# Xharlie/pointnerf

Measured on AMD Instinct MI355X. Metric: rays/sec (render+bwd) NeRF-synth lego 800^2, K=8, 128 samp/ray, higher is better.
Workload: dtype f32 in / out / accumulate; forward GEMM operands as 2 x f16 planes (22-bit) on the f16 MFMA, 3 products per multiply-add; input-gradient GEMMs: f16 leading product + e4m3 cross terms (csrc/mixq.h), 2 product equivalents; weight-gradient GEMM operands as one f16 plane each

## Files before the change

include/pnerf.h:

```cpp
#ifndef PNERF_H
#define PNERF_H
#include <stddef.h>
#include <stdint.h>

#ifdef __cplusplus
extern "C" {
#endif

#define PNERF_E_INVAL   (-1)
#define PNERF_E_WS      (-2)
#define PNERF_E_LAUNCH  (-3)
#define PNERF_E_UNSUP   (-4)

#define PNERF_MAX_K 16

typedef struct pnerf_grid_params {
    float ranges[6];
    float vsize[3];
    int32_t vdim[3];
    int32_t kernel_size[3];
    int32_t query_size[3];
    int32_t P;
    int32_t max_o;
    float radius;
} pnerf_grid_params;

enum { PNERF_GI_N_IN_GRID = 0, PNERF_GI_N_OCC = 1, PNERF_GI_MAX_CNT = 2, PNERF_GI_CELL0 = 3,
       PNERF_GI_FIRST_IDX = 4, PNERF_GI_OSTART_OFF = 5 , PNERF_GI_LEN = 8 };

int pnerf_version(void);
const char *pnerf_arch(void);

size_t pnerf_grid_workspace_bytes(const pnerf_grid_params *gp, int n_points);
int pnerf_grid_build(const pnerf_grid_params *gp, const float *d_xyz, int n_points,
                     void *d_grid_ws, size_t ws_bytes, void *stream);
int pnerf_grid_info(const void *d_grid_ws, int32_t *host_info, void *stream);
int pnerf_points_minmax(const float *d_xyz, int64_t n_points, float *d_out6, void *stream);

size_t pnerf_query_workspace_bytes(int R, int SR);
int pnerf_query(const pnerf_grid_params *gp, const void *d_grid_ws,
                const float *d_raypos,
                const float *campos3_host, const float *d_raydir, const float *d_mid,
                float near_depth, float far_depth, float jitter, uint64_t seed,
                int R, int D, int SR, int K,
                float *d_sample_loc, int32_t *d_sample_pidx, int32_t *d_sample_nn,
                int32_t *d_ray_hit, int32_t *d_valid_list, int32_t *d_counters,
                void *d_query_ws, size_t ws_bytes, void *stream);

int pnerf_gather_rows(const float *d_src, int n_src, int width, const int32_t *d_idx, int64_t n_idx,
                      float *d_dst, void *stream);
int pnerf_scatter_add_rows(const float *d_grad_rows, const int32_t *d_idx, int64_t n_idx, int width,
                           float *d_grad_src, int n_src, void *stream);

int pnerf_zero_one_blocks(int64_t n_idx);
int pnerf_zero_one_forward(const float *d_conf, int n_points, const int32_t *d_idx, int64_t n_idx, float eps,
                           float *d_partial, void *stream);
int pnerf_zero_one_backward(const float *d_conf, int n_points, const int32_t *d_idx, int64_t n_idx, float eps,
                            const float *d_gscale, float *d_grad_conf, void *stream);
int pnerf_zero_one_forward_rays(const float *d_conf, int n_points, const int32_t *d_idx, const int32_t *d_ray_hit, int R, int slots_per_ray, float eps,
                                float *d_partial, void *stream);
int pnerf_zero_one_backward_rays(const float *d_conf, int n_points, const int32_t *d_idx, const int32_t *d_ray_hit, int R, int slots_per_ray, float eps,
                                 const float *d_gscale, float *d_grad_conf, void *stream);
int pnerf_color_loss_blocks(int R);
int pnerf_color_loss_forward_rays(const float *d_ray_color, const float *d_gt, const int32_t *d_ray_hit, int R, float *d_partial, void *stream);
int pnerf_color_loss_backward_rays(const float *d_ray_color, const float *d_gt, const int32_t *d_ray_hit, int R, const float *d_gscale,
                                   float *d_grad_ray_color, void *stream);

int pnerf_geometry_loss_forward_rays(const float *d_depth_sum, const float *d_acc, const float *d_bg_trans, const int32_t *d_ray_hit,
                                     const float *d_gt_depth, const float *d_gt_mask, int R, float *d_partial, void *stream);
int pnerf_geometry_loss_backward_rays(const float *d_depth_sum, const float *d_acc, const float *d_bg_trans, const int32_t *d_ray_hit,
                                      const float *d_gt_depth, const float *d_gt_mask, int R, const float *d_gscale2, float *d_grad_geom, void *stream);


#define PNERF_MLP_NTENSORS 18
int pnerf_mlp_layout(int feat_dim, int64_t *offsets );
size_t pnerf_mlp_packed_bytes(void);
int pnerf_mlp_pack(const float *d_params, void *d_packed, void *stream);

typedef struct pnerf_camera {
    float campos[3];
    float camrot[9];
    float rw2c[9];
    float vsize_z;
    int32_t raydist_mode_unit;
    float bg[3];
    int32_t has_bg;
} pnerf_camera;

typedef struct pnerf_points {
    const float *xyz;
    const float *embedding;
    const float *conf;
    const float *dir;
    const float *color;
    int32_t n, feat_dim;
    const float *frames;
} pnerf_points;

typedef struct pnerf_point_grads {
    float *embedding, *conf, *dir, *color;
    void *ready_event;
    const float *zero_one_gscale;
    float zero_one_eps;
    float *xyz;
} pnerf_point_grads;

typedef struct pnerf_step {
    const float *raydir;
    const float *sample_loc;
    const int32_t *sample_pidx;
    const int32_t *sample_nn;
    const int32_t *valid_list;
    const int32_t *counters;
    const float *xyz_pers;
    const float *loc_pers;
    const float *params;
    const void *packed_mlp;
    int32_t R, SR, K;
    int64_t n_valid_max;
} pnerf_step;

size_t pnerf_agg_saved_bytes(int64_t n_valid_samples, int K);
size_t pnerf_agg_workspace_bytes(int64_t n_valid_max, int K);
size_t pnerf_render_backward_workspace_bytes(int R, int SR);

int pnerf_render_forward(const pnerf_camera *cam, const pnerf_points *pts, const pnerf_step *step,
                         float *d_decoded, float *d_weight, float *d_ray_color, float *d_opacity,
                         float *d_bg_trans, float *d_blend_w,
                         void *d_saved, void *d_ws, size_t ws_bytes, void *stream);

size_t pnerf_render_cut_workspace_bytes(int R, int SR);
int pnerf_render_forward_cut(const pnerf_camera *cam, const pnerf_points *pts, const pnerf_step *step, float cutoff, int stage_samples,
                             float *d_decoded, float *d_weight, float *d_ray_color, float *d_opacity, float *d_bg_trans, float *d_blend_w,
                             int32_t *d_cut_counters, void *d_ws, size_t ws_bytes, void *d_cut_ws, size_t cut_ws_bytes, void *stream);
int pnerf_cut_stage(const pnerf_camera *cam, const float *d_sample_loc, const int32_t *d_sample_nn, const int32_t *d_ray_hit,
                    const float *d_decoded, int R, int SR, float cutoff, int stage_samples, int stage,
                    float *d_trans, float *d_depth_max, int32_t *d_alive, int32_t *d_flags, int32_t *d_list, int32_t *d_counters,
                    void *d_ws, size_t ws_bytes, void *stream);

int pnerf_set_inference_products(int n);

int pnerf_set_wgrad_planes(int n);
int pnerf_set_cross_terms(int bits);
int pnerf_set_cross_terms_where(int mask);
int pnerf_get_arithmetic(int32_t out[4]);
int pnerf_debug_set_tile_grid(int max_workgroups);

int pnerf_render_backward(const pnerf_camera *cam, const pnerf_points *pts, const pnerf_step *step,
                          const float *d_decoded, const float *d_weight, const float *d_grad_ray_color,
                          void *d_saved, float *d_grad_params, const pnerf_point_grads *pg,
                          void *d_ws, size_t ws_bytes, void *stream);
int pnerf_render_backward_geom(const pnerf_camera *cam, const pnerf_points *pts, const pnerf_step *step,
                               const float *d_decoded, const float *d_weight, const float *d_grad_ray_color, const float *d_grad_geom,
                               void *d_saved, float *d_grad_params, const pnerf_point_grads *pg,
                               void *d_ws, size_t ws_bytes, void *stream);


size_t pnerf_compact_workspace_bytes(int64_t n);
int pnerf_touched_flags(const int32_t *d_pidx, int64_t n, int32_t n_points, int32_t *d_flags, void *stream);
int pnerf_compact_valid(const int32_t *d_nn, int64_t n, int32_t *d_list, int32_t *d_counters, void *d_ws, size_t ws_bytes, void *stream);

int pnerf_agg_forward(const pnerf_camera *cam, const pnerf_points *pts, const pnerf_step *step, float *d_decoded, float *d_weight,
                      void *d_saved, void *d_ws, size_t ws_bytes, void *stream);
int pnerf_agg_backward(const pnerf_camera *cam, const pnerf_points *pts, const pnerf_step *step,
                       const float *d_decoded, const float *d_weight, const float *d_grad_decoded,
                       void *d_saved, float *d_grad_params, const pnerf_point_grads *pg, void *d_ws, size_t ws_bytes, void *stream);

int pnerf_raymarch_forward(const float *d_ray_dist, const uint8_t *d_ray_valid, const float *d_features, const float *bg3_host,
                           int R, int SR, float *d_ray_color, float *d_opacity, float *d_acc_trans, float *d_blend_w,
                           float *d_bg_trans, void *stream);
int pnerf_raymarch_backward(const float *d_ray_dist, const uint8_t *d_ray_valid, const float *d_features, const float *bg3_host,
                            int R, int SR, const float *d_grad_ray_color, float *d_grad_features, void *stream);
int pnerf_raymarch_backward_geom(const float *d_ray_dist, const uint8_t *d_ray_valid, const float *d_features, const float *d_z, const float *bg3_host,
                                 int R, int SR, const float *d_grad_ray_color, const float *d_grad_geom, float *d_grad_features, void *stream);

int pnerf_adam_step(float *d_param, const float *d_grad, float *d_exp_avg, float *d_exp_avg_sq, int64_t n,
                    double lr, double beta1, double beta2, double eps, int64_t step, void *stream);
typedef struct pnerf_adam_tensor {
    float *param; const float *grad; float *exp_avg; float *exp_avg_sq;
    int64_t n; double lr; int64_t step;
} pnerf_adam_tensor;
int pnerf_adam_step_multi(const pnerf_adam_tensor *tensors, int count, double beta1, double beta2, double eps, void *stream);

size_t pnerf_voxel_downsample_workspace_bytes(int64_t n_points, int rx, int ry, int rz);
int pnerf_voxel_downsample(const float *d_xyz, int64_t n_points, const float *space_min3_host, const float *vox_size3_host,
                           int rx, int ry, int rz, float *d_centroid, int32_t *d_grid_idx, int64_t *d_min_idx, int32_t *d_counts,
                           void *d_ws, size_t ws_bytes, void *stream);

#define PNERF_EX2D_MAX_VIEWS 8
#define PNERF_EX2D_MAX_MAPS 32
typedef struct pnerf_view_desc {
    float c2w[16];
    float w2c[16];
    float intrinsic[9];
    int32_t has_w2c;
} pnerf_view_desc;
typedef struct pnerf_map_desc {
    const float *d_map;
    int32_t view;
    int32_t C, H, W;
    int32_t out_col;
    int32_t is_color;
    int32_t first_of_view;
} pnerf_map_desc;
size_t pnerf_extract_2d_workspace_bytes(int64_t n_points, int n_views, int HD, int WD, int depth_occ);
int pnerf_extract_2d(const float *d_cam_xyz, int64_t n_points, const pnerf_view_desc *views, int n_views, const pnerf_map_desc *maps,
                     int n_maps, int HD, int WD, int depth_occ, float tolerate, float *d_feats, int feat_cols, float *d_colors,
                     int color_cols, uint8_t *d_mask, void *d_ws, size_t ws_bytes, void *stream);
int pnerf_point_dirs(const float *d_cam_xyz, int64_t n_points, const float *cam_pos_cam_host, int n_views, const float *rot1_host9,
                     const float *rot2_host9, float *d_dirs, void *stream);

#define PNERF_DF_PAIR_FLOATS 32
int pnerf_depth_consistency(const float *d_depth, const int32_t *view_hw_host, int V, const float *d_pairs, int32_t *d_geo_mask_sum,
                            float *d_depth_avg, void *stream);
size_t pnerf_depth_fuse_select_workspace_bytes(int V, int H, int W);
int pnerf_depth_fuse_select(const int32_t *d_geo_mask_sum, const float *d_depth_avg, const float *d_cam_xyz, const float *d_confidence,
                            const uint8_t *d_points_mask, const float *d_inv_ext, int V, int H, int W, float depth_conf_thresh,
                            int geo_cnsst_num, const float *conf_factor10_host, const float *ranges6_host, float *d_xyz_cam,
                            float *d_xyz_world, float *d_conf_out, int32_t *d_view_id, int32_t *d_count, void *d_ws, size_t ws_bytes,
                            void *stream);
int pnerf_alpha_hull(const float *d_points, int64_t n_points, const float *d_alphas, const float *d_w2c, const float *d_intrinsics, int V,
                     int H, int W, int use_range_mask, const float *near_far2_host, uint8_t *d_mask, void *stream);

int pnerf_nearest_view(const float *d_xyz, int64_t n, const float *d_campos, const float *d_camdir, int M, int32_t *d_cam_ind, void *stream);
size_t pnerf_occupancy_merge_workspace_bytes(int64_t nb, int res);
int pnerf_occupancy_merge(const float *d_a_xyz, int64_t na, const float *d_b_xyz, int64_t nb, const float *space_min3_host,
                          const float *vox_size_a3_host, const float *vox_size_b3_host, int res, float *d_kept_xyz, int32_t *d_count,
                          uint8_t *d_mask, void *d_ws, size_t ws_bytes, void *stream);
size_t pnerf_crop_ranges_workspace_bytes(int64_t n);
int pnerf_crop_ranges(const float *d_xyz, int64_t n, const float *ranges6_host, float *d_kept_xyz, int32_t *d_count, uint8_t *d_mask, void *d_ws,
                      size_t ws_bytes, void *stream);
size_t pnerf_group_by_view_workspace_bytes(int64_t n, int M);
int pnerf_group_by_view(const int32_t *d_cam_ind, int64_t n, int M, int64_t *d_order, int64_t *d_offsets, void *d_ws, size_t ws_bytes,
                        void *stream);

size_t pnerf_mvs_cost_volume_workspace_bytes(int n_feat_sets, int V, int h, int w);
int pnerf_mvs_cost_volume(const float *d_feats, int n_feat_sets, const float *d_proj, const float *d_depth_values, int B, int V, int C, int D,
                          int h, int w, int align_corners, float *d_volume, void *d_ws, size_t ws_bytes, void *stream);
int pnerf_mvs_depth_regress(const float *d_cost_reg, const float *d_depth_values, int B, int D, int h, int w, float *d_depth,
                            float *d_confidence, float *d_prob_volume, void *stream);
int pnerf_depth_to_cam_points(const float *d_depth_lr, const float *d_conf_lr, int h, int w, int H, int W, float near, float far,
                              const float *inv_kt9_host, float *d_cam_xyz, float *d_confidence, uint8_t *d_mask, void *stream);

size_t pnerf_image_metrics_workspace_bytes(int H, int W, int win);
int pnerf_image_metrics(const float *d_img, const float *d_gt, int H, int W, int win, double data_range, int quantize8, double *d_out4,
                        void *d_ws, size_t ws_bytes, void *stream);

int pnerf_probe_rays(const pnerf_points *pts, const float *d_opacity, const float *d_weight, const float *d_sample_loc,
                     const int32_t *d_sample_pidx, const int32_t *d_ray_hit, int R, int SR, int K, float *d_max_opacity, float *d_loc3,
                     float *d_far_dist, float *d_avg_color3, float *d_avg_dir3, float *d_avg_conf, float *d_avg_emb32, void *stream);
int pnerf_probe_hole_mask(const int8_t *d_ray_mask, const float *d_max_opacity, const float *d_far_dist, const float *d_raycolor,
                          const float *d_gt, const uint8_t *d_edge, const float *bg3_host, int H, int W, float opacity_thresh,
                          float far_thresh, int32_t *d_flags, void *stream);

int pnerf_ray_geometry(const pnerf_camera *cam, const float *d_sample_loc, const int32_t *d_sample_nn, const int32_t *d_ray_hit,
                       const float *d_opacity, const float *d_blend_w, int R, int SR, float *d_acc, float *d_depth_sum, float *d_depth,
                       float *d_median_depth, int32_t *d_median_slot, void *stream);
int pnerf_geometry_canvas(const int32_t *d_pixel_idx, const int8_t *d_ray_mask, const float *d_depth, const float *d_median_depth,
                          const float *d_acc, int n_rays, int H, int W, float *d_depth_canvas, float *d_median_canvas, float *d_acc_canvas,
                          int32_t *d_flag, void *stream);

int pnerf_ray_attributes(const float *d_attr, int32_t n_points, int C,
        const float *d_blend_w, const float *d_weight, const int32_t *d_sample_pidx, const int32_t *d_ray_hit,
        int R, int SR, int K,
        float *d_attr_sum , int32_t *d_top_point, int32_t *d_top_flat, float *d_top_contrib ,
        void *stream);
int pnerf_lift_to_points(const float *d_values , int C, const float *d_ray_factor ,
        const float *d_blend_w, const float *d_weight, const int32_t *d_sample_pidx, const int32_t *d_ray_hit,
        int R, int SR, int K, int32_t n_points,
        float *d_point_sum , float *d_point_mass , void *stream);

int pnerf_debug_mfma_f16(const void *d_a, const void *d_b, float *d_out, void *stream);
int pnerf_debug_mix_gemm(const float *d_w, int K, const float *d_x, void *d_img, float *d_out, void *stream);
int pnerf_debug_mfma_rate(int mode, int iters, float *d_scratch, double *flop_out, void *stream);
int pnerf_debug_uniform(uint64_t seed, uint64_t first, int64_t n, float *d_out, void *stream);
int pnerf_debug_split(const float *d_x, int64_t n, void *d_h, void *d_m, int sat, void *stream);
int pnerf_debug_pe(const float *d_x, int64_t n, int nfreq, float *d_out, void *stream);

int pnerf_prof_enable(int on);
int pnerf_prof_kernel_count(void);
const char *pnerf_prof_kernel_name(int id);
int pnerf_prof_collect(double *total_ms, int64_t *launches);

#ifdef __cplusplus
}
#endif
#endif
```

pointnerf_amd/_lib.py:

```python
import ctypes
import os

import torch

_HERE = os.path.dirname(os.path.abspath(__file__))
LIB_PATH = os.path.join(_HERE, "libpnerf_hip.so")

c_int, c_i64, c_f32, c_void_p, c_size_t = ctypes.c_int, ctypes.c_int64, ctypes.c_float, ctypes.c_void_p, ctypes.c_size_t

ABI_VERSION = 1009
PNERF_MAX_K = 16
DF_PAIR_FLOATS = 32
GI_N_IN_GRID, GI_N_OCC, GI_MAX_CNT, GI_CELL0, GI_FIRST_IDX, GI_LEN = 0, 1, 2, 3, 4, 8
MLP_NTENSORS = 18

ERRORS = {-1: "PNERF_E_INVAL (bad argument)", -2: "PNERF_E_WS (workspace too small)",
          -3: "PNERF_E_LAUNCH (HIP launch/runtime error)", -4: "PNERF_E_UNSUP (unsupported configuration)"}


class GridParams(ctypes.Structure):
    _fields_ = [("ranges", c_f32 * 6), ("vsize", c_f32 * 3), ("vdim", ctypes.c_int32 * 3),
                ("kernel_size", ctypes.c_int32 * 3), ("query_size", ctypes.c_int32 * 3),
                ("P", ctypes.c_int32), ("max_o", ctypes.c_int32), ("radius", c_f32)]


class Camera(ctypes.Structure):
    _fields_ = [("campos", c_f32 * 3), ("camrot", c_f32 * 9), ("rw2c", c_f32 * 9), ("vsize_z", c_f32),
                ("raydist_mode_unit", ctypes.c_int32), ("bg", c_f32 * 3), ("has_bg", ctypes.c_int32)]


class Points(ctypes.Structure):
    _fields_ = [("xyz", c_void_p), ("embedding", c_void_p), ("conf", c_void_p), ("dir", c_void_p),
                ("color", c_void_p), ("n", ctypes.c_int32), ("feat_dim", ctypes.c_int32), ("frames", c_void_p)]


class AdamTensor(ctypes.Structure):
    _fields_ = [("param", c_void_p), ("grad", c_void_p), ("exp_avg", c_void_p), ("exp_avg_sq", c_void_p),
                ("n", ctypes.c_int64), ("lr", ctypes.c_double), ("step", ctypes.c_int64)]


class ViewDesc(ctypes.Structure):
    _fields_ = [("c2w", c_f32 * 16), ("w2c", c_f32 * 16), ("intrinsic", c_f32 * 9), ("has_w2c", ctypes.c_int32)]


class MapDesc(ctypes.Structure):
    _fields_ = [("d_map", c_void_p), ("view", ctypes.c_int32), ("C", ctypes.c_int32), ("H", ctypes.c_int32), ("W", ctypes.c_int32),
                ("out_col", ctypes.c_int32), ("is_color", ctypes.c_int32), ("first_of_view", ctypes.c_int32)]


class PointGrads(ctypes.Structure):
    _fields_ = [("embedding", c_void_p), ("conf", c_void_p), ("dir", c_void_p), ("color", c_void_p), ("ready_event", c_void_p),
                ("zero_one_gscale", c_void_p), ("zero_one_eps", c_f32), ("xyz", c_void_p)]


class Step(ctypes.Structure):
    _fields_ = [("raydir", c_void_p), ("sample_loc", c_void_p), ("sample_pidx", c_void_p), ("sample_nn", c_void_p), ("valid_list", c_void_p),
                ("counters", c_void_p), ("xyz_pers", c_void_p), ("loc_pers", c_void_p), ("params", c_void_p), ("packed_mlp", c_void_p),
                ("R", ctypes.c_int32), ("SR", ctypes.c_int32), ("K", ctypes.c_int32), ("n_valid_max", ctypes.c_int64)]


_STEP_ARGS = [ctypes.POINTER(Camera), ctypes.POINTER(Points), ctypes.POINTER(Step)]
PROTOTYPES = {
    "pnerf_version": (c_int, []),
    "pnerf_arch": (ctypes.c_char_p, []),
    "pnerf_grid_workspace_bytes": (c_size_t, [ctypes.POINTER(GridParams), c_int]),
    "pnerf_grid_build": (c_int, [ctypes.POINTER(GridParams), c_void_p, c_int, c_void_p, c_size_t, c_void_p]),
    "pnerf_grid_info": (c_int, [c_void_p, ctypes.POINTER(ctypes.c_int32), c_void_p]),
    "pnerf_points_minmax": (c_int, [c_void_p, c_i64, c_void_p, c_void_p]),
    "pnerf_query_workspace_bytes": (c_size_t, [c_int, c_int]),
    "pnerf_query": (c_int, [ctypes.POINTER(GridParams), c_void_p, c_void_p, ctypes.POINTER(c_f32), c_void_p, c_void_p,
                            c_f32, c_f32, c_f32, ctypes.c_uint64, c_int, c_int, c_int, c_int,
                            c_void_p, c_void_p, c_void_p, c_void_p, c_void_p, c_void_p, c_void_p, c_size_t, c_void_p]),
    "pnerf_gather_rows": (c_int, [c_void_p, c_int, c_int, c_void_p, c_i64, c_void_p, c_void_p]),
    "pnerf_scatter_add_rows": (c_int, [c_void_p, c_void_p, c_i64, c_int, c_void_p, c_int, c_void_p]),
    "pnerf_zero_one_blocks": (c_int, [c_i64]),
    "pnerf_zero_one_forward": (c_int, [c_void_p, c_int, c_void_p, c_i64, c_f32, c_void_p, c_void_p]),
    "pnerf_zero_one_backward": (c_int, [c_void_p, c_int, c_void_p, c_i64, c_f32, c_void_p, c_void_p, c_void_p]),
    "pnerf_color_loss_blocks": (c_int, [c_int]),
    "pnerf_color_loss_forward_rays": (c_int, [c_void_p, c_void_p, c_void_p, c_int, c_void_p, c_void_p]),
    "pnerf_color_loss_backward_rays": (c_int, [c_void_p, c_void_p, c_void_p, c_int, c_void_p, c_void_p, c_void_p]),
    "pnerf_zero_one_forward_rays": (c_int, [c_void_p, c_int, c_void_p, c_void_p, c_int, c_int, c_f32, c_void_p, c_void_p]),
    "pnerf_zero_one_backward_rays": (c_int, [c_void_p, c_int, c_void_p, c_void_p, c_int, c_int, c_f32, c_void_p, c_void_p, c_void_p]),
    "pnerf_voxel_downsample_workspace_bytes": (c_size_t, [c_i64, c_int, c_int, c_int]),
    "pnerf_voxel_downsample": (c_int, [c_void_p, c_i64, c_void_p, c_void_p, c_int, c_int, c_int, c_void_p, c_void_p, c_void_p, c_void_p, c_void_p, c_size_t, c_void_p]),
    "pnerf_extract_2d_workspace_bytes": (c_size_t, [c_i64, c_int, c_int, c_int, c_int]),
    "pnerf_extract_2d": (c_int, [c_void_p, c_i64, ctypes.POINTER(ViewDesc), c_int, ctypes.POINTER(MapDesc), c_int, c_int, c_int, c_int, c_f32,
                                 c_void_p, c_int, c_void_p, c_int, c_void_p, c_void_p, c_size_t, c_void_p]),
    "pnerf_point_dirs": (c_int, [c_void_p, c_i64, ctypes.POINTER(c_f32), c_int, ctypes.POINTER(c_f32), ctypes.POINTER(c_f32), c_void_p, c_void_p]),
    "pnerf_depth_consistency": (c_int, [c_void_p, ctypes.POINTER(ctypes.c_int32), c_int, c_void_p, c_void_p, c_void_p, c_void_p]),
    "pnerf_depth_fuse_select_workspace_bytes": (c_size_t, [c_int, c_int, c_int]),
    "pnerf_depth_fuse_select": (c_int, [c_void_p, c_void_p, c_void_p, c_void_p, c_void_p, c_void_p, c_int, c_int, c_int, c_f32, c_int,
                                        ctypes.POINTER(c_f32), ctypes.POINTER(c_f32), c_void_p, c_void_p, c_void_p, c_void_p, c_void_p,
                                        c_void_p, c_size_t, c_void_p]),
    "pnerf_alpha_hull": (c_int, [c_void_p, c_i64, c_void_p, c_void_p, c_void_p, c_int, c_int, c_int, c_int, ctypes.POINTER(c_f32), c_void_p, c_void_p]),
    "pnerf_nearest_view": (c_int, [c_void_p, c_i64, c_void_p, c_void_p, c_int, c_void_p, c_void_p]),
    "pnerf_occupancy_merge_workspace_bytes": (c_size_t, [c_i64, c_int]),
    "pnerf_occupancy_merge": (c_int, [c_void_p, c_i64, c_void_p, c_i64, ctypes.POINTER(c_f32), ctypes.POINTER(c_f32), ctypes.POINTER(c_f32), c_int,
                                      c_void_p, c_void_p, c_void_p, c_void_p, c_size_t, c_void_p]),
    "pnerf_crop_ranges_workspace_bytes": (c_size_t, [c_i64]),
    "pnerf_crop_ranges": (c_int, [c_void_p, c_i64, ctypes.POINTER(c_f32), c_void_p, c_void_p, c_void_p, c_void_p, c_size_t, c_void_p]),
    "pnerf_group_by_view_workspace_bytes": (c_size_t, [c_i64, c_int]),
    "pnerf_group_by_view": (c_int, [c_void_p, c_i64, c_int, c_void_p, c_void_p, c_void_p, c_size_t, c_void_p]),
    "pnerf_mvs_cost_volume_workspace_bytes": (c_size_t, [c_int, c_int, c_int, c_int]),
    "pnerf_mvs_cost_volume": (c_int, [c_void_p, c_int, c_void_p, c_void_p, c_int, c_int, c_int, c_int, c_int, c_int, c_int, c_void_p, c_void_p,
                                      c_size_t, c_void_p]),
    "pnerf_mvs_depth_regress": (c_int, [c_void_p, c_void_p, c_int, c_int, c_int, c_int, c_void_p, c_void_p, c_void_p, c_void_p]),
    "pnerf_depth_to_cam_points": (c_int, [c_void_p, c_void_p, c_int, c_int, c_int, c_int, c_f32, c_f32, ctypes.POINTER(c_f32), c_void_p, c_void_p,
                                          c_void_p, c_void_p]),
    "pnerf_adam_step": (c_int, [c_void_p, c_void_p, c_void_p, c_void_p, c_i64, ctypes.c_double, ctypes.c_double, ctypes.c_double, ctypes.c_double, c_i64, c_void_p]),
    "pnerf_adam_step_multi": (c_int, [ctypes.POINTER(AdamTensor), c_int, ctypes.c_double, ctypes.c_double, ctypes.c_double, c_void_p]),
    "pnerf_mlp_layout": (c_int, [c_int, ctypes.POINTER(c_i64)]),
    "pnerf_mlp_packed_bytes": (c_size_t, []),
    "pnerf_mlp_pack": (c_int, [c_void_p, c_void_p, c_void_p]),
    "pnerf_agg_saved_bytes": (c_size_t, [c_i64, c_int]),
    "pnerf_agg_workspace_bytes": (c_size_t, [c_i64, c_int]),
    "pnerf_render_backward_workspace_bytes": (c_size_t, [c_int, c_int]),
    "pnerf_render_forward": (c_int, _STEP_ARGS + [c_void_p, c_void_p, c_void_p, c_void_p, c_void_p, c_void_p, c_void_p, c_void_p, c_size_t, c_void_p]),
    "pnerf_render_cut_workspace_bytes": (c_size_t, [c_int, c_int]),
    "pnerf_render_forward_cut": (c_int, _STEP_ARGS + [c_f32, c_int, c_void_p, c_void_p, c_void_p, c_void_p, c_void_p, c_void_p, c_void_p,
                                                      c_void_p, c_size_t, c_void_p, c_size_t, c_void_p]),
    "pnerf_cut_stage": (c_int, [ctypes.POINTER(Camera), c_void_p, c_void_p, c_void_p, c_void_p, c_int, c_int, c_f32, c_int, c_int,
                                c_void_p, c_void_p, c_void_p, c_void_p, c_void_p, c_void_p, c_void_p, c_size_t, c_void_p]),
    "pnerf_set_inference_products": (c_int, [c_int]),
    "pnerf_set_wgrad_planes": (c_int, [c_int]),
    "pnerf_set_cross_terms": (c_int, [c_int]),
    "pnerf_set_cross_terms_where": (c_int, [c_int]),
    "pnerf_get_arithmetic": (c_int, [ctypes.POINTER(ctypes.c_int32)]),
    "pnerf_debug_set_tile_grid": (c_int, [c_int]),
    "pnerf_compact_workspace_bytes": (c_size_t, [c_i64]),
    "pnerf_touched_flags": (c_int, [c_void_p, c_i64, c_int, c_void_p, c_void_p]),
    "pnerf_compact_valid": (c_int, [c_void_p, c_i64, c_void_p, c_void_p, c_void_p, c_size_t, c_void_p]),
    "pnerf_agg_forward": (c_int, _STEP_ARGS + [c_void_p, c_void_p, c_void_p, c_void_p, c_size_t, c_void_p]),
    "pnerf_agg_backward": (c_int, _STEP_ARGS + [c_void_p, c_void_p, c_void_p, c_void_p, c_void_p, ctypes.POINTER(PointGrads), c_void_p, c_size_t, c_void_p]),
    "pnerf_raymarch_forward": (c_int, [c_void_p, c_void_p, c_void_p, ctypes.POINTER(c_f32), c_int, c_int,
                                       c_void_p, c_void_p, c_void_p, c_void_p, c_void_p, c_void_p]),
    "pnerf_raymarch_backward": (c_int, [c_void_p, c_void_p, c_void_p, ctypes.POINTER(c_f32), c_int, c_int,
                                        c_void_p, c_void_p, c_void_p]),
    "pnerf_image_metrics_workspace_bytes": (c_size_t, [c_int, c_int, c_int]),
    "pnerf_image_metrics": (c_int, [c_void_p, c_void_p, c_int, c_int, c_int, ctypes.c_double, c_int, c_void_p, c_void_p, c_size_t, c_void_p]),
    "pnerf_probe_rays": (c_int, [ctypes.POINTER(Points), c_void_p, c_void_p, c_void_p, c_void_p, c_void_p, c_int, c_int, c_int,
                                 c_void_p, c_void_p, c_void_p, c_void_p, c_void_p, c_void_p, c_void_p, c_void_p]),
    "pnerf_probe_hole_mask": (c_int, [c_void_p, c_void_p, c_void_p, c_void_p, c_void_p, c_void_p, ctypes.POINTER(c_f32), c_int, c_int,
                                      c_f32, c_f32, c_void_p, c_void_p]),
    "pnerf_ray_geometry": (c_int, [ctypes.POINTER(Camera), c_void_p, c_void_p, c_void_p, c_void_p, c_void_p, c_int, c_int,
                                   c_void_p, c_void_p, c_void_p, c_void_p, c_void_p, c_void_p]),
    "pnerf_geometry_canvas": (c_int, [c_void_p, c_void_p, c_void_p, c_void_p, c_void_p, c_int, c_int, c_int,
                                      c_void_p, c_void_p, c_void_p, c_void_p, c_void_p]),
    "pnerf_ray_attributes": (c_int, [c_void_p, ctypes.c_int32, c_int, c_void_p, c_void_p, c_void_p, c_void_p, c_int, c_int, c_int,
                                     c_void_p, c_void_p, c_void_p, c_void_p, c_void_p]),
    "pnerf_lift_to_points": (c_int, [c_void_p, c_int, c_void_p, c_void_p, c_void_p, c_void_p, c_void_p, c_int, c_int, c_int, ctypes.c_int32,
                                     c_void_p, c_void_p, c_void_p]),
    "pnerf_debug_mfma_f16": (c_int, [c_void_p, c_void_p, c_void_p, c_void_p]),
    "pnerf_debug_mix_gemm": (c_int, [c_void_p, c_int, c_void_p, c_void_p, c_void_p, c_void_p]),
    "pnerf_debug_mfma_rate": (c_int, [c_int, c_int, c_void_p, ctypes.POINTER(ctypes.c_double), c_void_p]),
    "pnerf_debug_uniform": (c_int, [ctypes.c_uint64, ctypes.c_uint64, c_i64, c_void_p, c_void_p]),
    "pnerf_debug_split": (c_int, [c_void_p, c_i64, c_void_p, c_void_p, c_int, c_void_p]),
    "pnerf_debug_pe": (c_int, [c_void_p, c_i64, c_int, c_void_p, c_void_p]),
    "pnerf_prof_enable": (c_int, [c_int]),
    "pnerf_prof_kernel_count": (c_int, []),
    "pnerf_prof_kernel_name": (ctypes.c_char_p, [c_int]),
    "pnerf_prof_collect": (c_int, [ctypes.POINTER(ctypes.c_double), ctypes.POINTER(c_i64)]),
    "pnerf_render_backward": (c_int, _STEP_ARGS + [c_void_p, c_void_p, c_void_p, c_void_p, c_void_p, ctypes.POINTER(PointGrads), c_void_p, c_size_t, c_void_p]),
    "pnerf_render_backward_geom": (c_int, _STEP_ARGS + [c_void_p, c_void_p, c_void_p, c_void_p, c_void_p, c_void_p, ctypes.POINTER(PointGrads), c_void_p, c_size_t,
                                                        c_void_p]),
    "pnerf_raymarch_backward_geom": (c_int, [c_void_p, c_void_p, c_void_p, c_void_p, ctypes.POINTER(c_f32), c_int, c_int, c_void_p, c_void_p, c_void_p, c_void_p]),
    "pnerf_geometry_loss_forward_rays": (c_int, [c_void_p, c_void_p, c_void_p, c_void_p, c_void_p, c_void_p, c_int, c_void_p, c_void_p]),
    "pnerf_geometry_loss_backward_rays": (c_int, [c_void_p, c_void_p, c_void_p, c_void_p, c_void_p, c_void_p, c_int, c_void_p, c_void_p, c_void_p]),
}

_lib = None


def bind(handle, path):
    for name, (res, args) in PROTOTYPES.items():
        try:
            fn = getattr(handle, name)
        except AttributeError as e:
            raise RuntimeError("pointnerf_amd: %s lacks symbol %s (stale build?)" % (os.path.basename(path), name)) from e
        fn.restype, fn.argtypes = res, args
    got = handle.pnerf_version()
    if got != ABI_VERSION:
        raise RuntimeError("pointnerf_amd: %s reports pnerf_version() %d, this binding is written for %d (stale build?)"
                           % (os.path.basename(path), got, ABI_VERSION))
    return handle


def lib():
    global _lib
    if _lib is None:
        if not os.path.exists(LIB_PATH):
            raise RuntimeError(
                "pointnerf_amd: %s not found. Build it with `python -c 'import __graft_entry__ as g; g.build()'` "
                "(hipcc --offload-arch=gfx950). There is no CPU/PyTorch fallback for this path." % LIB_PATH)
        _lib = bind(ctypes.CDLL(LIB_PATH), LIB_PATH)
    return _lib


def check(rc, what):
    if rc != 0:
        raise RuntimeError("pointnerf_amd: %s failed: %s" % (what, ERRORS.get(rc, rc)))
```

pointnerf_amd/csrc/aggregate.hip:

```cpp
#include "mixq.h"
#include <stdlib.h>

extern "C" int pnerf_mlp_layout(int feat_dim, int64_t *offsets) {
    if (feat_dim != PN_F || !offsets) return PNERF_E_UNSUP;
    const int64_t o[PNERF_MLP_NTENSORS + 1] = {PO_W1, PO_B1, PO_W2, PO_B2, PO_W3, PO_B3, PO_W4, PO_B4, PO_W5, PO_B5,
                                               PO_WC1, PO_BC1, PO_WC2, PO_BC2, PO_WC3, PO_BC3, PO_WC4, PO_BC4, PO_TOTAL};
    for (int i = 0; i <= PNERF_MLP_NTENSORS; ++i) offsets[i] = o[i];
    return 0;
}
extern "C" size_t pnerf_mlp_packed_bytes(void) { return (size_t)PKC_END; }

namespace {
struct PackHDesc { int src, ld, trans, Mreal, Kreal, NCH, MB, dst, cm1, ck1; };
__device__ __forceinline__ float pn_pack_scale(const char *packed, int cm1, int ck1, int m, int k) {
    float f = 1.f;
    if (cm1 && m < (cm1 - 1 < PN_CS_C1 ? PN_H : PN_HC)) f = pn_col_scale(packed, cm1 - 1)[m];
    if (ck1) f *= pn_col_scale_inv(packed, ck1 - 1)[k];
    return f;
}
struct ColScaleDesc { int first, units, n_cons; struct { int src, ld, rows; } cons[2]; };
struct ColScaleTable { ColScaleDesc d[7]; };
__global__ __launch_bounds__(256) void k_pack_colscale(ColScaleTable t, const float *__restrict__ params, char *__restrict__ packed) {
    __shared__ unsigned red[256];
    const ColScaleDesc d = t.d[blockIdx.x];
// ... 163 lines not shown
        {PO_W3, PN_IN3, 0, PN_H, PN_IN3, 1, 8, PKM_F3},
        {PO_W4, PN_H, 0, PN_H, PN_H, 0, 8, PKM_F4},
        {PO_W4, PN_H, 1, PN_H, PN_H, 0, 8, PKM_D4, PN_CS_L3 + 1, PN_CS_L4 + 1},
        {PO_W3, PN_IN3, 1, PN_IN3, PN_H, 0, 9, PKM_D3, PN_CS_L2 + 1, PN_CS_L3 + 1},
        {PO_W2, PN_H, 1, PN_H, PN_H, 0, 8, PKM_D2, PN_CS_L1 + 1, PN_CS_L2 + 1},
        {PO_W1, PN_IN1, 1, 32 * PN_MB_D1, PN_H, 0, PN_MB_D1, PKM_D1, 0, PN_CS_L1 + 1},
        {PO_W1 + 32 * PN_MB_D1, PN_IN1, 1, PN_IN1 - 32 * PN_MB_D1, PN_H, 0, 2, PKM_D1T, 0, PN_CS_L1 + 1},
    }};
    hipLaunchKernelGGL(k_pack_mix, dim3(12, 9), dim3(256), 0, (hipStream_t)stream, tm, d_params, (char *)d_packed);
    PN_CHECK_LAUNCH();
    return 0;
}

namespace {
template <int NT>
__global__ __launch_bounds__(256) void k_debug_mix_gemm(const float *__restrict__ x, const char *__restrict__ img, float *__restrict__ out) {
    extern __shared__ __attribute__((aligned(16))) char smem_d[];
    pn_mode_saturate();
    constexpr int K = 256 + 16 * NT;
    char *X = smem_d;
    const int tid = threadIdx.x, lane = tid & 63, wave = __builtin_amdgcn_readfirstlane(tid >> 6);
    for (int e = tid; e < PN_TILE * (K / 4); e += 256) {
        const int row = e / (K / 4), col = 4 * (e % (K / 4));
        const float4 v = *reinterpret_cast<const float4 *>(x + row * K + col);
        if (col < 256) pn_xq_store4(X, row, col, v.x, v.y, v.z, v.w);
        else pn_xt_store4(X, row, col, v.x, v.y, v.z, v.w);
    }
    __syncthreads();
    f32x16 acc[2][2];
    pn_acc_zero(acc);
    pn_gemm_mix<PN_MIX_NS, NT, 8, 2>(X, img, 2 * wave, lane, acc);
#pragma unroll
    for (int fb = 0; fb < 2; ++fb)
#pragma unroll
        for (int rb = 0; rb < 2; ++rb)
#pragma unroll
            for (int g = 0; g < 4; ++g)
#pragma unroll
                for (int i = 0; i < 4; ++i) out[(32 * rb + (lane & 31)) * PN_H + pn_d_feat(2 * wave + fb, g, lane) + i] = acc[fb][rb][4 * g + i];
}
}

extern "C" int pnerf_debug_mix_gemm(const float *d_w, int K, const float *d_x, void *d_img, float *d_out, void *stream) {
    if (!d_w || !d_x || !d_img || !d_out || (K != 256 && K != 272 && K != 288)) return PNERF_E_INVAL;
    hipStream_t s = (hipStream_t)stream;
    const int NT = (K - 256) / 16;
    PackMTable tm = {{{0, K, 0, PN_H, K, NT, 8, 0}}};
    hipLaunchKernelGGL(k_pack_mix, dim3(12, 1), dim3(256), 0, s, tm, d_w, (char *)d_img);
    const void *fn = NT == 0 ? (const void *)k_debug_mix_gemm<0> : NT == 1 ? (const void *)k_debug_mix_gemm<1> : (const void *)k_debug_mix_gemm<2>;
    if (hipFuncSetAttribute(fn, hipFuncAttributeMaxDynamicSharedMemorySize, PN_XBYTES) != hipSuccess) return PNERF_E_LAUNCH;
    if (NT == 0) hipLaunchKernelGGL(k_debug_mix_gemm<0>, dim3(1), dim3(256), PN_XBYTES, s, d_x, (const char *)d_img, d_out);
    else if (NT == 1) hipLaunchKernelGGL(k_debug_mix_gemm<1>, dim3(1), dim3(256), PN_XBYTES, s, d_x, (const char *)d_img, d_out);
    else hipLaunchKernelGGL(k_debug_mix_gemm<2>, dim3(1), dim3(256), PN_XBYTES, s, d_x, (const char *)d_img, d_out);
    PN_CHECK_LAUNCH();
    return 0;
}

namespace {
__global__ __launch_bounds__(64) void k_debug_mfma_f16(const uint4 *__restrict__ a, const uint4 *__restrict__ b, float *__restrict__ d) {
    f32x16 acc;
#pragma unroll
    for (int r = 0; r < 16; ++r) acc[r] = 0.f;
    acc = __builtin_amdgcn_mfma_f32_32x32x16_f16(__builtin_bit_cast(pn_h8, a[threadIdx.x]), __builtin_bit_cast(pn_h8, b[threadIdx.x]), acc, 0, 0, 0);
#pragma unroll
    for (int r = 0; r < 16; ++r) d[threadIdx.x * 16 + r] = acc[r];
}
}
namespace {
__global__ __launch_bounds__(256) void k_debug_split(const float *__restrict__ x, long long n, unsigned *__restrict__ h, unsigned *__restrict__ m, int sat) {
    for (long long i = (long long)blockIdx.x * 256 + threadIdx.x; 2 * i < n; i += (long long)gridDim.x * 256) {
        unsigned hh, mm;
        if (sat) pn_split2_sat(x[2 * i], x[2 * i + 1], hh, mm);
        else pn_split2(x[2 * i], x[2 * i + 1], hh, mm);
        h[i] = hh; m[i] = mm;
    }
}
}
extern "C" int pnerf_debug_split(const float *d_x, int64_t n, void *d_h, void *d_m, int sat, void *stream) {
    if (!d_x || !d_h || !d_m || n < 0 || (n & 1)) return PNERF_E_INVAL;
    if (n == 0) return 0;
    hipLaunchKernelGGL(k_debug_split, dim3(64), dim3(256), 0, (hipStream_t)stream, d_x, (long long)n, (unsigned *)d_h, (unsigned *)d_m, sat);
    PN_CHECK_LAUNCH();
    return 0;
}

namespace {
template <int NF> __global__ __launch_bounds__(256) void k_debug_pe(const float *__restrict__ x, long long n, float *__restrict__ out) {
    for (long long i = (long long)blockIdx.x * 256 + threadIdx.x; i < n; i += (long long)gridDim.x * 256) {
        float s[NF], c[NF];
        pn_pe_octaves<NF>(x[i], s, c);
#pragma unroll
        for (int f = 0; f < NF; ++f) { out[(i * NF + f) * 2] = s[f]; out[(i * NF + f) * 2 + 1] = c[f]; }
    }
}
}
extern "C" int pnerf_debug_pe(const float *d_x, int64_t n, int nfreq, float *d_out, void *stream) {
    if (!d_x || !d_out || n < 0 || nfreq < 1 || nfreq > 5) return PNERF_E_INVAL;
    if (n == 0) return 0;
    hipStream_t s = (hipStream_t)stream;
    switch (nfreq) {
        case 1: hipLaunchKernelGGL(k_debug_pe<1>, dim3(64), dim3(256), 0, s, d_x, (long long)n, d_out); break;
        case 2: hipLaunchKernelGGL(k_debug_pe<2>, dim3(64), dim3(256), 0, s, d_x, (long long)n, d_out); break;
        case 3: hipLaunchKernelGGL(k_debug_pe<3>, dim3(64), dim3(256), 0, s, d_x, (long long)n, d_out); break;
        case 4: hipLaunchKernelGGL(k_debug_pe<4>, dim3(64), dim3(256), 0, s, d_x, (long long)n, d_out); break;
        default: hipLaunchKernelGGL(k_debug_pe<5>, dim3(64), dim3(256), 0, s, d_x, (long long)n, d_out); break;
    }
    PN_CHECK_LAUNCH();
    return 0;
}

extern "C" int pnerf_debug_mfma_f16(const void *d_a, const void *d_b, float *d_out, void *stream) {
    if (!d_a || !d_b || !d_out) return PNERF_E_INVAL;
    hipLaunchKernelGGL(k_debug_mfma_f16, dim3(1), dim3(64), 0, (hipStream_t)stream, (const uint4 *)d_a, (const uint4 *)d_b, d_out);
    PN_CHECK_LAUNCH();
    return 0;
}

size_t pn_saved_walk(void *base, long long n_valid, int K, PnSaved &s) {
    const int TS = pn_tile_samples(K);
    const long long tiles = (n_valid + TS - 1) / TS + 2 * PN_NCLS + 1;
    s.rows = tiles * PN_TILE;
    s.samples = ((tiles * TS + PN_CTILE - 1) / PN_CTILE + 1) * PN_CTILE;
    PnCarver cv(base);
    const size_t rg = (size_t)s.rows / 8, rgc = (size_t)s.samples / 8;
    auto planes = [&](uint4 *&x0, uint4 *&h2, uint4 *&h1, uint4 *&h3, uint4 *&dy1, uint4 *&dy2, uint4 *&dy3, uint4 *&dy4) {
        x0 = cv.take<uint4>(rg * PN_NF1); h2 = cv.take<uint4>(rg * PN_NF1);
        h1 = cv.take<uint4>(rg * PN_H); h3 = cv.take<uint4>(rg * PN_H);
        dy1 = cv.take<uint4>(rg * PN_H); dy2 = cv.take<uint4>(rg * PN_H);
        dy3 = cv.take<uint4>(rg * PN_H); dy4 = cv.take<uint4>(rg * PN_H);
    };
    auto cplanes = [&](uint4 *&xc, uint4 *&c1, uint4 *&c2, uint4 *&dc1, uint4 *&dc2, uint4 *&dc3) {
        xc = cv.take<uint4>(rgc * PN_NF1); c1 = cv.take<uint4>(rgc * PN_HC); c2 = cv.take<uint4>(rgc * PN_HC);
        dc1 = cv.take<uint4>(rgc * PN_HC); dc2 = cv.take<uint4>(rgc * PN_HC); dc3 = cv.take<uint4>(rgc * PN_HC);
    };
    planes(s.x0k, s.h2k, s.h1k, s.h3k, s.dy1k, s.dy2k, s.dy3k, s.dy4k);
    s.h4r = cv.take<uint4>((size_t)s.rows * 32 * 2);
    s.arow = cv.take<float>((size_t)s.rows); s.rmeta = cv.take<int4>((size_t)s.rows);
    s.lmask = cv.take<unsigned>((size_t)tiles * 3 * 512);
    s.gscale = cv.take<unsigned>(PN_GS_WORDS);
    s.fs = cv.take<float>((size_t)s.samples * PN_H); s.dfs = cv.take<float>((size_t)s.samples * PN_H);
    s.c3 = cv.take<float>((size_t)s.samples * PN_HC);
    cplanes(s.xck, s.c1k, s.c2k, s.dc1k, s.dc2k, s.dc3k);
    s.cmask = cv.take<unsigned>((size_t)s.samples / PN_CTILE * 2 * 256);
    s.wg2 = pn_arith().wgrad_planes == 2 ? 1 : 0;
    s.x0m = s.h1m = s.h2m = s.h3m = s.dy1m = s.dy2m = s.dy3m = s.dy4m = nullptr;
    s.xcm = s.c1m = s.c2m = s.dc1m = s.dc2m = s.dc3m = nullptr;
    if (s.wg2) {
        planes(s.x0m, s.h2m, s.h1m, s.h3m, s.dy1m, s.dy2m, s.dy3m, s.dy4m);
        cplanes(s.xcm, s.c1m, s.c2m, s.dc1m, s.dc2m, s.dc3m);
    }
    pn_cls_walk(cv, s);
    return cv.off;
}
void pn_cls_walk(PnCarver &cv, PnSaved &s) {
    s.cls_list = cv.take<int>((size_t)s.samples);
    s.cls_info = cv.take<int>(PN_CI_WORDS);
    s.cls_tmp = cv.take<int>((size_t)2 * s.samples + pn_scan_scratch_ints(s.samples) + 8);
}
size_t pn_saved_bytes(long long n_valid, int K) { PnSaved s; return pn_saved_walk(nullptr, n_valid, K, s); }
PnSaved pn_saved_carve(void *base, long long n_valid, int K) { PnSaved s; pn_saved_walk(base, n_valid, K, s); return s; }

extern "C" size_t pnerf_agg_saved_bytes(int64_t n_valid_samples, int K) {
    if (K <= 0 || K > PNERF_MAX_K || n_valid_samples < 0) return 0;
    return pn_saved_bytes(n_valid_samples, K);
}

namespace {
struct FwdArgs {
    pnerf_camera cam;
    const float *xyz, *emb, *conf, *dir, *color;
    const float *params;
    const float4 *packed;
    const float *raydir, *sample_loc;
    const float *xyz_pers, *loc_pers;
    const int *pidx, *valid_list, *counters;
    const int *cls_list, *cls_info;
    int cls, Kstride;
    int save_x0;
    int R, SR, K, TS;
    long long cap_samples;
    float *decoded, *weight;
    PnSaved sv;
};
struct FwdArgsF : FwdArgs { const float *frames; };
template <bool FRAMES> struct FwdArgsOf { using type = FwdArgs; };
template <> struct FwdArgsOf<true> { using type = FwdArgsF; };

namespace {
struct ClsArgs { const int *valid_list, *counters, *pidx; int K, n, ncls; int kc[PN_NCLS], ts[PN_NCLS]; };

__global__ void k_cls_flags(ClsArgs c, int which, int *__restrict__ flags) {
    const int vs = blockIdx.x * blockDim.x + threadIdx.x;
    if (vs >= c.n) return;
    const int Ns = c.counters[0] < c.n ? c.counters[0] : c.n;
    int f = 0;
    if (vs < Ns) {
        const long long si = c.valid_list[vs];
        int hv = 0;
        for (int k = 0; k < c.K; ++k)
            if (c.pidx[si * c.K + k] >= 0) hv = k + 1;
        int cl = 0;
        for (int j = 1; j < c.ncls; ++j)
            if (hv <= c.kc[j]) cl = j;
        f = cl == which;
    }
    flags[vs] = f;
}

__global__ void k_cls_gather(ClsArgs c, int which, const int *__restrict__ pos, const int *__restrict__ count, int *__restrict__ cls_list,
                             int *__restrict__ info) {
    const int n = *count, base = info[PN_CI_VBASE + which];
    for (int i = blockIdx.x * blockDim.x + threadIdx.x; i < n; i += gridDim.x * blockDim.x) cls_list[base + i] = c.valid_list[pos[i]];
    if (blockIdx.x == 0 && threadIdx.x == 0) {
        const int tiles = (n + c.ts[which] - 1) / c.ts[which], tb = info[PN_CI_TBASE + which];
        info[PN_CI_COUNT + which] = n;
        if (which + 1 < PN_NCLS) { info[PN_CI_VBASE + which + 1] = base + n; info[PN_CI_TBASE + which + 1] = tb + tiles + 1; }
        info[PN_CI_TILES] = tb + tiles + 1;
    }
}

__global__ void k_cls_zero_gaps(PnSaved sv, int ncls, int save_x0) {
    const int c = blockIdx.y;
    if (c >= ncls) return;
    if ((blockIdx.x == 0 && !save_x0) || (blockIdx.x == 8 && save_x0)) return;
    const long long gap = (c + 1 < PN_NCLS ? sv.cls_info[PN_CI_TBASE + c + 1] : sv.cls_info[PN_CI_TILES]) - 1;
    uint4 *arrs[9] = {sv.x0k, sv.h2k, sv.h1k, sv.h3k, sv.dy1k, sv.dy2k, sv.dy3k, sv.dy4k, sv.x0k};
    uint4 *arrm[9] = {sv.x0m, sv.h2m, sv.h1m, sv.h3m, sv.dy1m, sv.dy2m, sv.dy3m, sv.dy4m, nullptr};
    const int which = blockIdx.x;
    const int nf = which == 8 ? 64 : which < 2 ? PN_NF1 : PN_H;
    uint4 *p = arrs[which] + gap * 8 * nf;
    for (int i = threadIdx.x; i < 8 * nf; i += blockDim.x) p[i] = make_uint4(0u, 0u, 0u, 0u);
    if (sv.wg2 && arrm[which]) {
        uint4 *pm = arrm[which] + gap * 8 * nf;
        for (int i = threadIdx.x; i < 8 * nf; i += blockDim.x) pm[i] = make_uint4(0u, 0u, 0u, 0u);
    }
}
}

}

int pn_class_slots(int K, int kc[PN_NCLS]) {
    if (K % 4 == 0) { kc[0] = K; kc[1] = K / 2; kc[2] = K / 4; return 3; }
    kc[0] = K; kc[1] = kc[2] = 0;
    return 1;
}

int pn_classify(const PnSaved &sv, const int32_t *d_valid_list, const int32_t *d_counters, const int32_t *d_pidx, int K, long long n_valid,
                bool train, bool save_x0, hipStream_t s) {
    ClsArgs c;
    c.valid_list = d_valid_list; c.counters = d_counters; c.pidx = d_pidx; c.K = K; c.n = (int)n_valid;
    c.ncls = pn_class_slots(K, c.kc);
    for (int j = 0; j < PN_NCLS; ++j) c.ts[j] = c.kc[j] > 0 ? pn_tile_samples(c.kc[j]) : 1;
    if (hipMemsetAsync(sv.cls_info, 0, PN_CI_WORDS * sizeof(int), s) != hipSuccess) return PNERF_E_LAUNCH;
    if (n_valid <= 0) return 0;
    int *flags = sv.cls_tmp, *pos = flags + n_valid, *cnt = pos + n_valid, *scratch = cnt + 8;
    PnProfScope prof(PNK_COMPACT, s);
    for (int j = 0; j < c.ncls; ++j) {
        hipLaunchKernelGGL(k_cls_flags, dim3(pn_cdiv(n_valid, 256)), dim3(256), 0, s, c, j, flags);
        int rc = pn_compact_gt0_i32(flags, n_valid, pos, cnt, scratch, s);
        if (rc) return rc;
        hipLaunchKernelGGL(k_cls_gather, dim3(256), dim3(256), 0, s, c, j, pos, cnt, sv.cls_list, sv.cls_info);
    }
    if (train) hipLaunchKernelGGL(k_cls_zero_gaps, dim3(9, c.ncls), dim3(256), 0, s, sv, c.ncls, save_x0 ? 1 : 0);
    PN_CHECK_LAUNCH();
    return 0;
}


namespace {

constexpr int FL_EX = PN_XBYTES, FL_W5 = FL_EX + PN_TILE * 8 * 4, FL_ROW = FL_W5 + PN_H * 4, FL_CLAIM = FL_ROW + 4 * PN_TILE * 4 , FL_BYTES = FL_CLAIM + 16;
static_assert(2 * FL_BYTES <= 160 * 1024, "two forward workgroups must fit the 160 KB LDS");

struct FGather {
    float4 e0, e1;
    float px, py, pz, lx, ly, lz, cf;
    float ppx, ppy, ppz, lpx, lpy, lpz;
    float dxv, dyv, dzv, cx, cy, cz, rx, ry, rz;
    float fx, fy, fz, gx, gy, gz;
};

__device__ __forceinline__ int f_sample_of(const FwdArgs &a, long long tile, int row, int Ns, unsigned kinv) {
    const int ls = pn_row_div(row, kinv);
    const long long vs = tile * a.TS + ls;
    return (ls < a.TS && vs < Ns) ? a.valid_list[vs] : -1;
}

template <bool PERS, bool FRAMES = false>
__device__ __forceinline__ void f_gather(const FwdArgs &a, FGather &G, int si_, int p_, int q, const float *frames = nullptr) {
    const int p = p_ > 0 ? p_ : 0, si = si_ > 0 ? si_ : 0;
    const float *ep = a.emb + (long long)p * PN_F + PN_EPT * q;
    G.e0 = *reinterpret_cast<const float4 *>(ep); G.e1 = *reinterpret_cast<const float4 *>(ep + 4);
    G.px = a.xyz[3 * p]; G.py = a.xyz[3 * p + 1]; G.pz = a.xyz[3 * p + 2];
    G.lx = a.sample_loc[(long long)si * 3]; G.ly = a.sample_loc[(long long)si * 3 + 1]; G.lz = a.sample_loc[(long long)si * 3 + 2];
    if (PERS) {
        G.ppx = a.xyz_pers[3 * p]; G.ppy = a.xyz_pers[3 * p + 1]; G.ppz = a.xyz_pers[3 * p + 2];
        G.lpx = a.loc_pers[(long long)si * 3]; G.lpy = a.loc_pers[(long long)si * 3 + 1]; G.lpz = a.loc_pers[(long long)si * 3 + 2];
    }
    G.cf = a.conf[p];
    if (FRAMES) {
        const int r = si / a.SR, fr = q < 3 ? q : 2;
        const int ps_ = a.pidx[(long long)si * a.Kstride], ps = ps_ > 0 ? ps_ : 0;
        const float *fp = frames + (long long)p * 9 + 3 * fr, *gp = frames + (long long)ps * 9 + 3 * fr;
        G.fx = fp[0]; G.fy = fp[1]; G.fz = fp[2];
        G.gx = gp[0]; G.gy = gp[1]; G.gz = gp[2];
        G.dxv = a.dir[3 * p]; G.dyv = a.dir[3 * p + 1]; G.dzv = a.dir[3 * p + 2];
        G.rx = a.raydir[3 * r]; G.ry = a.raydir[3 * r + 1]; G.rz = a.raydir[3 * r + 2];
        if (q == 0) { G.cx = a.color[3 * p]; G.cy = a.color[3 * p + 1]; G.cz = a.color[3 * p + 2]; }
    } else if (q == 0) {
        const int r = si / a.SR;
        G.dxv = a.dir[3 * p]; G.dyv = a.dir[3 * p + 1]; G.dzv = a.dir[3 * p + 2];
        G.cx = a.color[3 * p]; G.cy = a.color[3 * p + 1]; G.cz = a.color[3 * p + 2];
        G.rx = a.raydir[3 * r]; G.ry = a.raydir[3 * r + 1]; G.rz = a.raydir[3 * r + 2];
    }
}

template <bool PERS, bool MIX = false, bool FRAMES = false>
__device__ __forceinline__ void f_build(const FwdArgs &a, const FGather &G, char *X, float *exb, float *wraw, int *sidx, int si, int p, int row, int q) {
    const float dwx = G.px - G.lx, dwy = G.py - G.ly, dwz = G.pz - G.lz;
    float ppx, ppy, pcz, spx, spy, scz;
    if (PERS) {
        ppx = G.ppx; ppy = G.ppy; pcz = G.ppz; spx = G.lpx; spy = G.lpy; scz = G.lpz;
    } else {
        float pcx, pcy, scx, scy;
        if (FRAMES) {
            const float *M = a.cam.camrot;
            const float x = G.px - a.cam.campos[0], y = G.py - a.cam.campos[1], z = G.pz - a.cam.campos[2];
            const float u = G.lx - a.cam.campos[0], v = G.ly - a.cam.campos[1], w = G.lz - a.cam.campos[2];
            pcx = __builtin_fmaf(z, M[6], __builtin_fmaf(y, M[3], x * M[0]));
            pcy = __builtin_fmaf(z, M[7], __builtin_fmaf(y, M[4], x * M[1]));
            pcz = __builtin_fmaf(z, M[8], __builtin_fmaf(y, M[5], x * M[2]));
            scx = __builtin_fmaf(w, M[6], __builtin_fmaf(u, M[0], v * M[3]));
            scy = __builtin_fmaf(w, M[7], __builtin_fmaf(u, M[1], v * M[4]));
            scz = __builtin_fmaf(w, M[8], __builtin_fmaf(u, M[2], v * M[5]));
        } else {
        rot3(a.cam.camrot, G.px - a.cam.campos[0], G.py - a.cam.campos[1], G.pz - a.cam.campos[2], false, pcx, pcy, pcz);
        rot3(a.cam.camrot, G.lx - a.cam.campos[0], G.ly - a.cam.campos[1], G.lz - a.cam.campos[2], false, scx, scy, scz);
        }
        ppx = pcx / pcz; ppy = pcy / pcz; spx = scx / scz; spy = scy / scz;
    }
    float d0, d1, d2;
    if (FRAMES) d0 = d1 = d2 = dwx * G.fx + dwy * G.fy + dwz * G.fz;
    else rot3(a.cam.rw2c, dwx, dwy, dwz, true, d0, d1, d2);
    const float d3 = ppx * pcz - spx * scz, d4 = ppy * pcz - spy * scz, d5 = pcz - scz;
    const float da = q == 0 ? d0 : q == 1 ? d1 : q == 2 ? d2 : d3;
    const float db = q == 0 ? d4 : d5;
    const float e[8] = {G.e0.x, G.e0.y, G.e0.z, G.e0.w, G.e1.x, G.e1.y, G.e1.z, G.e1.w};
    if (MIX) {
        pn_xq_store4(X, row, PN_EPT * q, e[0], e[1], e[2], e[3]);
        pn_xq_store4(X, row, PN_EPT * q + 4, e[4], e[5], e[6], e[7]);
#pragma unroll
        for (int i = 0; i < 8; i += 2) {
            const int col = PN_F + (PN_EPT * q + i) * 6;
            float s0[3], c0[3], s1[3], c1[3];
            pn_pe_octaves<3>(e[i], s0, c0);
            pn_pe_octaves<3>(e[i + 1], s1, c1);
            pn_xq_store4(X, row, col, s0[0], c0[0], s0[1], c0[1]);
            pn_xq_store4(X, row, col + 4, s0[2], c0[2], s1[0], c1[0]);
            pn_xq_store4(X, row, col + 8, s1[1], c1[1], s1[2], c1[2]);
        }
    } else {
    pn_xt_store4(X, row, PN_EPT * q, e[0], e[1], e[2], e[3]); pn_xt_store4(X, row, PN_EPT * q + 4, e[4], e[5], e[6], e[7]);
#pragma unroll
    for (int i = 0; i < 8; ++i) {
        const int dd = PN_EPT * q + i;
        float s[3], c[3];
        pn_pe_octaves<3>(e[i], s, c);
        pn_xt_store2(X, row, PN_F + dd * 6, s[0], c[0]);
        pn_xt_store2(X, row, PN_F + dd * 6 + 2, s[1], c[1]);
        pn_xt_store2(X, row, PN_F + dd * 6 + 4, s[2], c[2]);
    }
    }
#pragma unroll
    for (int j = 0; j < 2; ++j) {
        const int comp = q + 4 * j;
        if (comp < 6) {
            float s[5], c[5];
            pn_pe_octaves<5>(j == 0 ? da : db, s, c);
#pragma unroll
            for (int f = 0; f < 5; ++f) {
                if (MIX) pn_xa_store2(X, row, PN_F * 7 + (comp * 5 + f) * 2, s[f], c[f]);
                else pn_xt_store2(X, row, PN_F * 7 + (comp * 5 + f) * 2, s[f], c[f]);
            }
        }
    }
    if (q == 3) pn_xt_store4(X, row, PN_ONES1, 1.f, 0.f, 0.f, 0.f);
    float fvx = 0.f, fvy = 0.f, fvz = 0.f, fqx = 0.f, fqy = 0.f, fqz = 0.f;
    if (FRAMES) {
        fvx = G.rx * G.gx + G.ry * G.gy + G.rz * G.gz;
        fqx = G.dxv * G.fx + G.dyv * G.fy + G.dzv * G.fz;
        fvy = __shfl_down(fvx, 1, 64); fvz = __shfl_down(fvx, 2, 64);
        fqy = __shfl_down(fqx, 1, 64); fqz = __shfl_down(fqx, 2, 64);
    }
    if (q == 0) {
        float vx, vy, vz, qx, qy, qz;
        if (FRAMES) { vx = fvx; vy = fvy; vz = fvz; qx = fqx; qy = fqy; qz = fqz; }
        else {
        rot3(a.cam.rw2c, G.rx, G.ry, G.rz, true, vx, vy, vz);
        rot3(a.cam.rw2c, G.dxv, G.dyv, G.dzv, true, qx, qy, qz);
        }
        float *ex = exb + row * 8;
        *reinterpret_cast<float4 *>(ex) = make_float4(G.cx, G.cy, G.cz, qx - vx);
        if (FRAMES) {
            *reinterpret_cast<float4 *>(ex + 4) = make_float4(qy - vy, qz - vz, __builtin_fmaf(qz, vz, __builtin_fmaf(qx, vx, qy * vy)), 1.f);
            wraw[row] = p >= 0 ? 1.0f / fmaxf(sqrtf(__builtin_fmaf(dwz, dwz, __builtin_fmaf(dwx, dwx, dwy * dwy))), 1e-6f) : 0.f;
        } else {
        *reinterpret_cast<float4 *>(ex + 4) = make_float4(qy - vy, qz - vz, qx * vx + qy * vy + qz * vz, 1.f);
        wraw[row] = p >= 0 ? 1.0f / fmaxf(sqrtf(dwx * dwx + dwy * dwy + dwz * dwz), 1e-6f) : 0.f;
        }
        sidx[row] = si;
    }
}

__device__ __forceinline__ void f_acc_bias(const float *__restrict__ bias, int wave, int lane, f32x16 (&acc)[PN_NFB][2]) {
#pragma unroll
    for (int fb = 0; fb < PN_NFB; ++fb)
#pragma unroll
        for (int g = 0; g < 4; ++g) {
// ... 147 lines not shown
    }

    f32x16 acc[PN_NFB][2];
    PN_TR_ITER_DECL;
    for (bool first = true; t0 < tile_last; first = false) {
        PN_TR_ITER_NEXT;
        tile = t0;
        int tid = threadIdx.x;
        asm volatile("" : "+v"(tid));
        const int lane = tid & 63, wave = __builtin_amdgcn_readfirstlane(tid >> 6);
        const int row = tid / PN_TPR, q = tid % PN_TPR, k = row - pn_row_div(row, kinv) * K;
        const long long gtile = tb + tile;
        PN_LDS_BARRIER();
        PN_TR(pn_trace_fwd, 0); PN_TR_HWID(pn_trace_fwd); PN_TR_SPAN(pn_span_fwd, a.cls, 0);
        f_build<PERS, MIX, FRAMES>(a, G, X, exb, wraw, sidx, si0, p0, row, q);
        f_acc_bias(P + PO_B1, wave, lane, acc);
        PnTileW<MIX, 2, 8, NP> W1;
        W1.prefetch(img, PKH_F1, PKM_F1, PN_NFB * wave, lane);
        PN_LDS_BARRIER();
        if (q == 0) {
            const int ls = pn_row_div(row, kinv);
            float wn = 0.f, w = 0.f;
            if (si0 >= 0) {
                float sum = 0.f;
                for (int kk = 0; kk < K; ++kk) sum += wraw[ls * K + kk];
                wn = wraw[row] / fmaxf(sum, 1e-8f);
                w = wn * fminf(fmaxf(G.cf, 1e-4f), 1.0f);
                a.weight[(long long)si0 * a.Kstride + k] = wn;
            }
            wnrm[row] = wn; wrow[row] = w;
            if (TRAIN) a.sv.rmeta[gtile * PN_TILE + row] = make_int4(si0, si0 >= 0 ? p0 : -1, __float_as_int(wn), __float_as_int(w));
        }
        unsigned mask[PN_NFB];
        PN_TR(pn_trace_fwd, 1);
        PN_TR(pn_trace_fwd, 2);
        W1.run(X, lane, acc);
        if (TRAIN) {
            if (HC) {
                if (a.save_x0) pn_copy_out_kmajor_h<PN_NF1>(X, a.sv.x0k, gtile * 8, tid);
                else pn_copy_out_kmajor_cols64_h<224>(X, a.sv.x0k, gtile * 8, tid);
            } else if (WG2) pn_copy_out_kmajor<PN_NF1, true>(X, a.sv.x0k, gtile * 8, tid, a.sv.x0m);
            else if (a.save_x0) pn_copy_out_kmajor<PN_NF1, false>(X, a.sv.x0k, gtile * 8, tid);
            else pn_copy_out_kmajor_cols64<224>(X, a.sv.x0k, gtile * 8, tid);
        }
        PN_LDS_BARRIER();
        PN_TR(pn_trace_fwd, 3);
        f_epilogue<TRAIN, MIX, HR>(acc, X, wave, lane, mask);
        if (TRAIN) f_store_masks(a.sv.lmask, gtile, 0, wave, lane, mask);
        f_acc_bias(P + PO_B2, wave, lane, acc);
        PnTileW<MIX, 0, 8, NP> W2;
        W2.prefetch(img, PKH_F2, PKM_F2, PN_NFB * wave, lane);
        PN_LDS_BARRIER();
        PN_TR(pn_trace_fwd, 4);
        PN_TR(pn_trace_fwd, 5);
        W2.run(X, lane, acc);
        if (TRAIN) {
            if (HC) pn_copy_out_kmajor_h<PN_H>(X, a.sv.h1k, gtile * 8, tid);
            else pn_copy_out_kmajor<PN_H, WG2>(X, a.sv.h1k, gtile * 8, tid, a.sv.h1m);
        }
        PN_LDS_BARRIER();
        PN_TR(pn_trace_fwd, 6);
        f_epilogue<TRAIN, MIX, HR>(acc, X, wave, lane, mask);
        if (TRAIN) f_store_masks(a.sv.lmask, gtile, 1, wave, lane, mask);
        if (tid < PN_TILE) {
            const float4 u = *reinterpret_cast<const float4 *>(exb + tid * 8), v = *reinterpret_cast<const float4 *>(exb + tid * 8 + 4);
            pn_xt_store4(X, tid, PN_H, u.x, u.y, u.z, u.w);
            pn_xt_store4(X, tid, PN_H + 4, v.x, v.y, v.z, v.w);
            pn_xt_store4(X, tid, PN_H + 8, 0.f, 0.f, 0.f, 0.f);
            pn_xt_store4(X, tid, PN_H + 12, 0.f, 0.f, 0.f, 0.f);
        }
        f_acc_bias(P + PO_B3, wave, lane, acc);
        PnTileW<MIX, 1, 8, NP> W3;
        W3.prefetch(img, PKH_F3, PKM_F3, PN_NFB * wave, lane);
        PN_LDS_BARRIER();
        PN_TR(pn_trace_fwd, 7);
        PN_TR(pn_trace_fwd, 8);
        W3.run(X, lane, acc);
        if (TRAIN) {
            if (HC) pn_copy_out_kmajor_h<PN_NF1>(X, a.sv.h2k, gtile * 8, tid);
            else pn_copy_out_kmajor<PN_NF1, WG2>(X, a.sv.h2k, gtile * 8, tid, a.sv.h2m);
        }
        PN_LDS_BARRIER();
        PN_TR(pn_trace_fwd, 9);
        f_epilogue<TRAIN, MIX, HR>(acc, X, wave, lane, mask);
        if (TRAIN) f_store_masks(a.sv.lmask, gtile, 2, wave, lane, mask);
        f_acc_bias(P + PO_B4, wave, lane, acc);
        PnTileW<MIX, 0, 8, NP> W4;
        W4.prefetch(img, PKH_F4, PKM_F4, PN_NFB * wave, lane);
        PN_LDS_BARRIER();
        PN_TR(pn_trace_fwd, 10);
        PN_TR(pn_trace_fwd, 11);
        W4.run(X, lane, acc);
        if (TRAIN) {
            if (HC) pn_copy_out_kmajor_h<PN_H>(X, a.sv.h3k, gtile * 8, tid);
            else pn_copy_out_kmajor<PN_H, WG2>(X, a.sv.h3k, gtile * 8, tid, a.sv.h3m);
        }
        PN_TR(pn_trace_fwd, 12);
        const int t3 = first ? t2 + grid : pn_claim_tile(PN_CLAIM_STATIC_FWD, grid, __builtin_amdgcn_readfirstlane(*claim_w), nclaim - 1);
        const bool claims = nclaim % PN_CLAIM_TILES == 0;
        int claimed = 0;
        if (tid == 0 && claims) claimed = atomicAdd(claim_ctr, 1);
        const int si_next = si1, p_next = p1;
        if (t1 < tile_last) f_gather<PERS, FRAMES>(a, G, si1, p1, q, frames);
        const int p2 = si2 >= 0 ? a.pidx[(long long)si2 * a.Kstride + k] : -1;
        const int si3 = t3 < tile_last ? f_sample_of(a, t3, row, Ns, kinv) : -1;
        PN_LDS_BARRIER();
        PN_TR(pn_trace_fwd, 13);
        f_epilogue<false>(acc, X, wave, lane, mask);
        PN_LDS_BARRIER();
        PN_TR(pn_trace_fwd, 14);
        if (K == 8 || K == 4 || K == 2 || K == 1) {
            if (K == 8) f_tail<8, TRAIN>(a, X, w5s, wrow, sidx, b5, tile, gtile, tid);
            else if (K == 4) f_tail<4, TRAIN>(a, X, w5s, wrow, sidx, b5, tile, gtile, tid);
            else if (K == 2) f_tail<2, TRAIN>(a, X, w5s, wrow, sidx, b5, tile, gtile, tid);
            else f_tail<1, TRAIN>(a, X, w5s, wrow, sidx, b5, tile, gtile, tid);
            PN_TR(pn_trace_fwd, 15);
        } else {
        f_tail<0, TRAIN>(a, X, w5s, wrow, sidx, b5, tile, gtile, tid, wraw);
        PN_LDS_BARRIER();
        PN_TR(pn_trace_fwd, 15);
        for (int e = tid; e < TS * 32; e += PN_NTHR) {
            const int ls = e >> 5, cg = e & 31;
            float4 f0 = make_float4(0.f, 0.f, 0.f, 0.f), f1 = f0;
            for (int kk = 0; kk < K; ++kk) {
                const int r = ls * K + kk;
                const uint4 h = *reinterpret_cast<const uint4 *>(X + r * PN_XRS + cg * 16);
                const uint4 m = *reinterpret_cast<const uint4 *>(X + PN_XPLANE + r * PN_XRS + cg * 16);
                const float w = wrow[r];
                f0.x = pn_fma2_lo(h.x, m.x, w, f0.x); f0.y = pn_fma2_hi(h.x, m.x, w, f0.y); f0.z = pn_fma2_lo(h.y, m.y, w, f0.z); f0.w = pn_fma2_hi(h.y, m.y, w, f0.w);
                f1.x = pn_fma2_lo(h.z, m.z, w, f1.x); f1.y = pn_fma2_hi(h.z, m.z, w, f1.y); f1.z = pn_fma2_lo(h.w, m.w, w, f1.z); f1.w = pn_fma2_hi(h.w, m.w, w, f1.w);
            }
            const long long vs = tile * TS + ls;
            if (vs < a.cap_samples) {
                *reinterpret_cast<float4 *>(a.sv.fs + vs * PN_H + 8 * cg) = f0;
                *reinterpret_cast<float4 *>(a.sv.fs + vs * PN_H + 8 * cg + 4) = f1;
            }
        }
        if (tid < TS) {
            const int si = sidx[tid * K];
            if (si >= 0) {
                float sg = 0.f;
                for (int kk = 0; kk < K; ++kk) sg += wraw[tid * K + kk];
                a.decoded[(long long)si * 4] = sg;
            }
        }
        }
        si0 = si_next; p0 = p_next; si1 = si2; p1 = p2; si2 = si3;
        if (tid == 0 && claims) *claim_w = claimed;
        t0 = t1; t1 = t2; t2 = t3; ++nclaim;
        PN_TR(pn_trace_fwd, 16); PN_TR_SPAN(pn_span_fwd, a.cls, 1);
    }
}

constexpr int CL_W4 = PN_XBYTES, CL_BYTES = CL_W4 + 3 * PN_HC * 4;
static_assert(2 * CL_BYTES <= 160 * 1024, "two colour workgroups must fit the 160 KB LDS");

__device__ __forceinline__ void c_load_bias(const float *__restrict__ bias, int wave, int lane, float4 (&b)[4]) {
#pragma unroll
    for (int g = 0; g < 4; ++g) {
        const float *p = bias + pn_d_feat(wave, g, lane);
        b[g] = make_float4(p[0], p[1], p[2], p[3]);
    }
}
template <bool TRAIN, bool SAVE32>
__device__ __forceinline__ unsigned c_epilogue(const f32x16 (&acc)[2][2], const float4 (&bias)[4], char *X, int wave, int lane, float *__restrict__ save, long long grow0) {
    unsigned mw = 0u;
#pragma unroll
    for (int rb = 0; rb < 2; ++rb)
#pragma unroll
        for (int g = 0; g < 4; ++g) {
            const int f0 = pn_d_feat(wave, g, lane), row = 32 * rb + (lane & 31);
            const float4 b = bias[g];
            float v[4] = {acc[0][rb][4 * g] + b.x, acc[0][rb][4 * g + 1] + b.y, acc[0][rb][4 * g + 2] + b.z, acc[0][rb][4 * g + 3] + b.w};
            if (TRAIN && !SAVE32) {
#pragma unroll
                for (int i = 0; i < 4; ++i) mw = __builtin_amdgcn_alignbit(mw, __float_as_uint(v[i]), 31);
            }
#pragma unroll
            for (int i = 0; i < 4; ++i) v[i] = fmaxf(v[i], 0.01f * v[i]);
            if (TRAIN && SAVE32) {
                pn_f4 t = {v[0], v[1], v[2], v[3]};
                PN_REG_STORE(t, reinterpret_cast<pn_f4 *>(save + (grow0 + row) * PN_HC + f0));
            }
            pn_x_store4<false>(X, row, f0, v[0], v[1], v[2], v[3]);
        }
    return mw;
}

template <bool TRAIN, int NP, bool WG2 = false, bool FRAMES = false>
__global__ __launch_bounds__(256, 2) void k_color_forward(typename FwdArgsOf<FRAMES>::type a) {
    extern __shared__ __attribute__((aligned(16))) char smem_c[];
    char *X = smem_c;
    float *w4s = reinterpret_cast<float *>(smem_c + CL_W4);
    const int Ns = a.counters[0] < a.cap_samples ? a.counters[0] : (int)a.cap_samples;
    const float *P = a.params;
    const char *img = reinterpret_cast<const char *>(a.packed);
    for (int i = threadIdx.x; i < 3 * PN_HC; i += 256) w4s[i] = P[PO_WC4 + i];
    const float b40 = P[PO_BC4], b41 = P[PO_BC4 + 1], b42 = P[PO_BC4 + 2];

    f32x16 acc[2][2];
    for (long long tile = blockIdx.x; tile * PN_CTILE < Ns; tile += gridDim.x) {
        int tid = threadIdx.x;
        asm volatile("" : "+v"(tid));
        const int lane = tid & 63, wave = __builtin_amdgcn_readfirstlane(tid >> 6), row = tid >> 2, q = tid & 3;
        const long long grow0 = tile * PN_CTILE, vs = grow0 + row;
        const int si = vs < Ns ? a.valid_list[vs] : -1;
        PnGemmW<18, 4, 1, 7, NP> WC1;
        WC1.prefetch(reinterpret_cast<const uint4 *>(img + PKH_FC1), wave, lane);
        PN_LDS_BARRIER();
        if (si >= 0) {
            const float4 *f = reinterpret_cast<const float4 *>(a.sv.fs + vs * PN_H);
            float4 fv[16];
#pragma unroll
            for (int c = 0; c < 16; ++c) fv[c] = f[4 * c + q];
#pragma unroll
            for (int c = 0; c < 16; ++c) pn_x_store4<false>(X, row, 16 * c + 4 * q, fv[c].x, fv[c].y, fv[c].z, fv[c].w);
            {
                const int r = si / a.SR;
                float v[3], sn[4], cs[4];
                if constexpr (FRAMES) {
                    const int ps_ = a.pidx[(long long)si * a.Kstride], ps = ps_ > 0 ? ps_ : 0;
                    const float *fp = a.frames + (long long)ps * 9;
                    const float fm[9] = {fp[0], fp[1], fp[2], fp[3], fp[4], fp[5], fp[6], fp[7], fp[8]};
                    rot3(fm, a.raydir[3 * r], a.raydir[3 * r + 1], a.raydir[3 * r + 2], true, v[0], v[1], v[2]);
                } else
                rot3(a.cam.rw2c, a.raydir[3 * r], a.raydir[3 * r + 1], a.raydir[3 * r + 2], true, v[0], v[1], v[2]);
                const float vq = q == 0 ? v[0] : (q == 1 ? v[1] : v[2]);
                pn_pe_octaves<4>(vq, sn, cs);
                if (q < 3) {
                    pn_x_store4<false>(X, row, PN_H + 4 * q, sn[0], sn[1], sn[2], sn[3]);
                    pn_x_store4<false>(X, row, PN_H + 12 + 4 * q, cs[0], cs[1], cs[2], cs[3]);
                } else {
                    pn_x_store4<false>(X, row, PN_H + 24, 0.f, 0.f, 0.f, 0.f);
                    pn_x_store4<false>(X, row, PN_H + 28, 0.f, 0.f, 0.f, 0.f);
                }
            }
        } else {
#pragma unroll
            for (int c = 0; c < 18; ++c) pn_x_store4<false>(X, row, 16 * c + 4 * q, 0.f, 0.f, 0.f, 0.f);
        }
        PN_LDS_BARRIER();
        float4 bias[4];
        if (TRAIN) pn_copy_out_kmajor<PN_NF1, WG2>(X, a.sv.xck, tile * 8, tid, a.sv.xcm);
        pn_acc_zero(acc);
        pn_gemm_f16x3_run<18, 4, 1, 7, NP>(X, WC1, lane, acc);
        c_load_bias(P + PO_BC1, wave, lane, bias);
        PN_LDS_BARRIER();
        unsigned mw = c_epilogue<TRAIN, false>(acc, bias, X, wave, lane, nullptr, grow0);
        if (TRAIN) a.sv.cmask[(tile * 2 + 0) * 256 + tid] = mw;
        PnGemmW<8, 4, 1, 7, NP> WC2;
        WC2.prefetch(reinterpret_cast<const uint4 *>(img + PKH_FC2), wave, lane);
        PN_LDS_BARRIER();
        if (TRAIN) pn_copy_out_kmajor<PN_HC, WG2>(X, a.sv.c1k, tile * 8, tid, a.sv.c1m);
        pn_acc_zero(acc);
        pn_gemm_f16x3_run<8, 4, 1, 7, NP>(X, WC2, lane, acc);
        c_load_bias(P + PO_BC2, wave, lane, bias);
        PN_LDS_BARRIER();
        mw = c_epilogue<TRAIN, false>(acc, bias, X, wave, lane, nullptr, grow0);
        if (TRAIN) a.sv.cmask[(tile * 2 + 1) * 256 + tid] = mw;
        PnGemmW<8, 4, 1, 7, NP> WC3;
        WC3.prefetch(reinterpret_cast<const uint4 *>(img + PKH_FC3), wave, lane);
        PN_LDS_BARRIER();
        if (TRAIN) pn_copy_out_kmajor<PN_HC, WG2>(X, a.sv.c2k, tile * 8, tid, a.sv.c2m);
        pn_acc_zero(acc);
        pn_gemm_f16x3_run<8, 4, 1, 7, NP>(X, WC3, lane, acc);
        c_load_bias(P + PO_BC3, wave, lane, bias);
        PN_LDS_BARRIER();
        c_epilogue<TRAIN, true>(acc, bias, X, wave, lane, a.sv.c3, grow0);
        PN_LDS_BARRIER();
        {
            float o0 = 0.f, o1 = 0.f, o2 = 0.f;
#pragma unroll
            for (int j = 0; j < 4; ++j) {
                const int c0 = q * 32 + 8 * j;
                o0 = pn_x_dot8(X, row, c0, *reinterpret_cast<const float4 *>(w4s + c0), *reinterpret_cast<const float4 *>(w4s + c0 + 4), o0);
                o1 = pn_x_dot8(X, row, c0, *reinterpret_cast<const float4 *>(w4s + PN_HC + c0), *reinterpret_cast<const float4 *>(w4s + PN_HC + c0 + 4), o1);
                o2 = pn_x_dot8(X, row, c0, *reinterpret_cast<const float4 *>(w4s + 2 * PN_HC + c0), *reinterpret_cast<const float4 *>(w4s + 2 * PN_HC + c0 + 4), o2);
            }
            o0 = group_sum<4>(o0); o1 = group_sum<4>(o1); o2 = group_sum<4>(o2);
            if (q == 0 && si >= 0) {
                float *o = a.decoded + (long long)si * 4;
                o[1] = 1.0f / (1.0f + expf(-(o0 + b40))) * 1.002f - 0.001f;
                o[2] = 1.0f / (1.0f + expf(-(o1 + b41))) * 1.002f - 0.001f;
                o[3] = 1.0f / (1.0f + expf(-(o2 + b42))) * 1.002f - 0.001f;
            }
        }
    }
}
}

#ifndef PN_MIX_DEFAULT_MASK
#define PN_MIX_DEFAULT_MASK 4
#endif
static PnArith &pn_arith_record() {
    static PnArith a = [] {
        const char *e = getenv("PNERF_MIX_MASK");
        return PnArith{3, 1, 8, e ? atoi(e) & 7 : PN_MIX_DEFAULT_MASK};
    }();
    return a;
}
PnArith pn_arith() { return pn_arith_record(); }
static int pn_arith_set(int PnArith::*field, int v, bool valid) {
    if (!valid) return PNERF_E_INVAL;
    const int old = pn_arith_record().*field;
    pn_arith_record().*field = v;
    return old;
}
extern "C" int pnerf_set_inference_products(int n) { return pn_arith_set(&PnArith::products, n, n == 2 || n == 3); }
extern "C" int pnerf_set_wgrad_planes(int n) { return pn_arith_set(&PnArith::wgrad_planes, n, n == 1 || n == 2); }
extern "C" int pnerf_set_cross_terms(int bits) { return pn_arith_set(&PnArith::cross_terms, bits, bits == 8 || bits == 16); }
extern "C" int pnerf_set_cross_terms_where(int mask) { return pn_arith_set(&PnArith::mix_where, mask, mask >= 0 && mask <= 7); }
static int pn_tile_grid_cap = 0;
int pn_tile_grid(long long tiles, long long dflt) { return pn_capped_grid(tiles, pn_tile_grid_cap > 0 && pn_tile_grid_cap < dflt ? pn_tile_grid_cap : dflt); }
extern "C" int pnerf_debug_set_tile_grid(int max_workgroups) {
    if (max_workgroups < 0) return PNERF_E_INVAL;
    const int old = pn_tile_grid_cap;
    pn_tile_grid_cap = max_workgroups;
    return old;
}
extern "C" int pnerf_get_arithmetic(int32_t out[4]) {
    if (!out) return PNERF_E_INVAL;
    const PnArith a = pn_arith();
    out[0] = a.products; out[1] = a.wgrad_planes; out[2] = a.cross_terms; out[3] = a.mix_where;
    return 0;
}

int pn_agg_forward_launch(const pnerf_camera *cam, const pnerf_points *pts, const pnerf_step &st, float *d_decoded, float *d_weight,
                          const PnSaved &sv, bool train, bool save_x0, hipStream_t s) {
    const int K = st.K;
    const long long cap_samples = st.n_valid_max;
    const PnArith ar = pn_arith();
    FwdArgs a;
    const bool wg2 = train && sv.wg2;
    if (wg2) save_x0 = true;
    a.save_x0 = save_x0 ? 1 : 0;
    a.cam = *cam;
    a.xyz = pts->xyz; a.emb = pts->embedding; a.conf = pts->conf; a.dir = pts->dir; a.color = pts->color;
    a.params = st.params; a.packed = (const float4 *)st.packed_mlp;
    a.raydir = st.raydir; a.sample_loc = st.sample_loc; a.xyz_pers = st.xyz_pers; a.loc_pers = st.loc_pers; a.pidx = st.sample_pidx; a.valid_list = st.valid_list; a.counters = st.counters;
    a.R = st.R; a.SR = st.SR; a.K = K; a.TS = pn_tile_samples(K);
    a.cap_samples = cap_samples;
    a.decoded = d_decoded; a.weight = d_weight; a.sv = sv;
    const bool frames = pts->frames != nullptr;
    if (frames && train) return PNERF_E_INVAL;
    const int ncu = pn_cu_count();
    if (!ncu) return PNERF_E_LAUNCH;
    const int grid_c = pn_tile_grid((cap_samples + PN_CTILE - 1) / PN_CTILE, 2LL * ncu);
    const size_t lds_a = FL_BYTES, lds_c = CL_BYTES;
    const bool pers = st.xyz_pers != nullptr;
    const bool np2 = !train && ar.products == 2;
    const bool mix = !wg2 && !np2 && (ar.mix_mask() & (train ? 2 : 1));
    if (frames && (np2 || mix)) return PNERF_E_UNSUP;
    using FwdKernel = void (*)(FwdArgs);
    using FwdKernelF = void (*)(FwdArgsF);
    const FwdKernelF kfnf = pers ? k_agg_forward<false, true, 3, false, true> : k_agg_forward<false, false, 3, false, true>;
    const FwdKernelF cfnf = k_color_forward<false, 3, false, true>;
    const FwdKernel kfn = wg2   ? (pers ? k_agg_forward<true, true, 3, true> : k_agg_forward<true, false, 3, true>)
                        : mix   ? (train ? (pers ? k_agg_forward<true, true, 4> : k_agg_forward<true, false, 4>)
                                         : (pers ? k_agg_forward<false, true, 4> : k_agg_forward<false, false, 4>))
                        : train ? (pers ? k_agg_forward<true, true, 3> : k_agg_forward<true, false, 3>)
                        : np2   ? (pers ? k_agg_forward<false, true, 2> : k_agg_forward<false, false, 2>)
                                : (pers ? k_agg_forward<false, true, 3> : k_agg_forward<false, false, 3>);
    const FwdKernel cfn = wg2 ? k_color_forward<true, 3, true> : train ? k_color_forward<true, 3> : np2 ? k_color_forward<false, 2> : k_color_forward<false, 3>;
    if (hipFuncSetAttribute(frames ? reinterpret_cast<const void *>(kfnf) : reinterpret_cast<const void *>(kfn), hipFuncAttributeMaxDynamicSharedMemorySize, (int)lds_a) != hipSuccess) return PNERF_E_LAUNCH;
    if (hipFuncSetAttribute(frames ? reinterpret_cast<const void *>(cfnf) : reinterpret_cast<const void *>(cfn), hipFuncAttributeMaxDynamicSharedMemorySize, (int)lds_c) != hipSuccess) return PNERF_E_LAUNCH;
    int rc = pn_classify(sv, st.valid_list, st.counters, st.sample_pidx, K, cap_samples, train, save_x0, s);
    if (rc) return rc;
    a.cls_list = sv.cls_list; a.cls_info = sv.cls_info; a.Kstride = K;
    int kc[PN_NCLS];
    const int ncls = pn_class_slots(K, kc);
    {
        PnProfScope prof(PNK_AGG_FWD, s);
        for (int j = 0; j < ncls; ++j) {
            a.cls = j; a.K = kc[j]; a.TS = pn_tile_samples(kc[j]);
            const int grid_a = pn_tile_grid((cap_samples + a.TS - 1) / a.TS, 2LL * ncu);
            if (frames) { FwdArgsF af; static_cast<FwdArgs &>(af) = a; af.frames = pts->frames; hipLaunchKernelGGL(kfnf, dim3(grid_a), dim3(PN_NTHR), lds_a, s, af); }
            else hipLaunchKernelGGL(kfn, dim3(grid_a), dim3(PN_NTHR), lds_a, s, a);
        }
    }
    a.K = K; a.TS = pn_tile_samples(K); a.valid_list = sv.cls_list;
    {
        PnProfScope prof(PNK_COLOR_FWD, s);
        if (frames) { FwdArgsF af; static_cast<FwdArgs &>(af) = a; af.frames = pts->frames; hipLaunchKernelGGL(cfnf, dim3(grid_c), dim3(256), lds_c, s, af); }
        else hipLaunchKernelGGL(cfn, dim3(grid_c), dim3(256), lds_c, s, a);
    }
    PN_CHECK_LAUNCH();
    return 0;
}

#ifdef PN_PHASE_TRACE
extern "C" int pnerf_debug_trace_fwd(void *host, size_t bytes) {
    return hipMemcpyFromSymbol(host, HIP_SYMBOL(pn_trace_fwd), bytes < sizeof(pn_trace_fwd) ? bytes : sizeof(pn_trace_fwd)) == hipSuccess ? 0 : -1;
}
extern "C" int pnerf_debug_span_fwd(void *host, size_t bytes) {
    return hipMemcpyFromSymbol(host, HIP_SYMBOL(pn_span_fwd), bytes < sizeof(pn_span_fwd) ? bytes : sizeof(pn_span_fwd)) == hipSuccess ? 0 : -1;
}
#endif
```

pointnerf_amd/csrc/backward.hip:

```cpp
#include "mixq.h"

namespace {
constexpr int WG_CHUNKS = 256;
constexpr size_t PARTIAL_FLOATS = (size_t)WG_CHUNKS * PN_H * PN_IN1P;

struct BwdArgs {
    pnerf_camera cam;
    const float *params;
    const float4 *packed;
    const float *raydir;
    const int *pidx, *valid_list, *counters;
    const int *cls_list, *cls_info;
    int cls;
    int SR, K, TS;
    long long cap_samples;
    const float *decoded, *weight, *grad_decoded;
    PnSaved sv;
    const float *emb;
    float *gparams;
    float *g_emb, *g_conf, *g_dir, *g_color;
    const float *conf, *zo_gs;
    float zo_eps;
};
struct BwdXArgs : BwdArgs {
    const float *xyz, *sample_loc;
    float *g_xyz;
};
template <bool XYZG> struct BwdArgsOf { using T = BwdArgs; };
template <> struct BwdArgsOf<true> { using T = BwdXArgs; };

__global__ __launch_bounds__(256) void k_grad_max(const int *__restrict__ list, const int *__restrict__ counters, long long cap, const float *__restrict__ gd,
                                                  unsigned *__restrict__ gscale) {
    __shared__ unsigned red[4];
    const long long Ns = counters[0] < cap ? counters[0] : cap;
    float m = 0.f;
    for (long long vs = (long long)blockIdx.x * 256 + threadIdx.x; vs < Ns; vs += (long long)gridDim.x * 256) {
        const float4 g = *reinterpret_cast<const float4 *>(gd + (long long)list[vs] * 4);
        m = fmaxf(m, fmaxf(fmaxf(fabsf(g.x), fabsf(g.y)), fmaxf(fabsf(g.z), fabsf(g.w))));
    }
#pragma unroll
    for (int off = 32; off > 0; off >>= 1) m = fmaxf(m, __shfl_xor(m, off, 64));
    if ((threadIdx.x & 63) == 0) red[threadIdx.x >> 6] = __float_as_uint(m);
    __syncthreads();
    if (threadIdx.x == 0) {
        unsigned r = red[0];
        for (int i = 1; i < 4; ++i) r = red[i] > r ? red[i] : r;
        if (r != 0u && r < 0x7f800000u) atomicMax(gscale, r);
    }
}
__device__ __forceinline__ void pn_scale_from_bits(unsigned mb, float &S, float &invS) {
    const int e = (int)((mb >> 23) & 0xffu);
    int se = (e == 0 || e == 255) ? 127 : 127 + 4 - (e - 127);
    se = se < 2 ? 2 : (se > 252 ? 252 : se);
    S = __uint_as_float((unsigned)se << 23);
    invS = __uint_as_float((unsigned)(254 - se) << 23);
}
static_assert(PN_CTILE == PN_TILE, "one row-scale record layout for both tile kernels");
constexpr int PN_RSC_BYTES = PN_TILE * 16 + PN_TILE * 2;
__device__ __forceinline__ void pn_sample_scale(const float4 g, float S, float invS, float &Si, float &invSi) {
    const unsigned mb = __float_as_uint(fmaxf(fmaxf(fabsf(g.x), fabsf(g.y)), fmaxf(fabsf(g.z), fabsf(g.w))));
    Si = S; invSi = invS;
    if (mb >= 0x00800000u && mb < 0x7f800000u) {
        pn_scale_from_bits(mb, Si, invSi);
        if (Si < S) { Si = S; invSi = invS; }
    }
}
struct PnRowScale {
    float *p;
    __device__ __forceinline__ void set(int r, float Si, float invSi, float S, float w = 0.f) const {
        const float f = S * invSi;
        *reinterpret_cast<float4 *>(p + 4 * r) = make_float4(Si, invSi, f, w * Si);
        reinterpret_cast<_Float16 *>(p + 4 * PN_TILE)[r] = (_Float16)f;
    }
    __device__ __forceinline__ float S(int r) const { return p[4 * r]; }
    __device__ __forceinline__ float inv(int r) const { return p[4 * r + 1]; }
    __device__ __forceinline__ float to_call(int r) const { return p[4 * r + 2]; }
    __device__ __forceinline__ float wS(int r) const { return p[4 * r + 3]; }
    __device__ __forceinline__ const char *h8(int rg) const { return reinterpret_cast<const char *>(p + 4 * PN_TILE) + rg * 16; }
};
template <int NF, int XRS = PN_XRS>
__device__ __forceinline__ void pn_copy_out_kmajor_hs(const char *X, const PnRowScale &rs, uint4 *__restrict__ dst, long long rg0, int tid) {
    const int lane = tid & 63, wave = tid >> 6;
    const int blk = ((lane >> 2) & 3) * XRS + ((lane >> 4) * 16 + (lane & 3) * 4) * 2;
#pragma unroll
    for (int i = 0; i < 2; ++i) {
        const int rg = wave * 2 + i;
        const char *src = X + rg * 8 * XRS + blk;
        uint4 *d = dst + (rg0 + rg) * NF;
        const uint4 fq = *reinterpret_cast<const uint4 *>(rs.h8(rg));
        const pn_h4 flo = __builtin_bit_cast(pn_h4, make_uint2(fq.x, fq.y)), fhi = __builtin_bit_cast(pn_h4, make_uint2(fq.z, fq.w));
        uint2 lo[(NF + 63) / 64], hi[(NF + 63) / 64];
#pragma unroll
        for (int j = 0; j < (NF + 63) / 64; ++j) { lo[j] = pn_lds_read_tr16(src + j * 128); hi[j] = pn_lds_read_tr16(src + 4 * XRS + j * 128); }
#pragma unroll
        for (int j = 0; j < (NF + 63) / 64; ++j) {
            const int f = lane + 64 * j;
            if (f < NF) {
                const uint2 a = __builtin_bit_cast(uint2, __builtin_bit_cast(pn_h4, lo[j]) * flo), b = __builtin_bit_cast(uint2, __builtin_bit_cast(pn_h4, hi[j]) * fhi);
                pn_f4 t = {__uint_as_float(a.x), __uint_as_float(a.y), __uint_as_float(b.x), __uint_as_float(b.y)};
                PN_STREAM_STORE(t, reinterpret_cast<pn_f4 *>(d + f));
            }
        }
    }
}

constexpr int CB_XRS = 2 * PN_HC + 16, CB_XPL = PN_CTILE * CB_XRS, CB_XBYTES = 2 * CB_XPL;
constexpr int CB_GSUMS = 6 * PN_HC;
constexpr int CB_DRAW = CB_XBYTES, CB_GACC = CB_DRAW + PN_CTILE * 4 * 4, CB_W4 = CB_GACC + 4 * CB_GSUMS * 4, CB_RSC = CB_W4 + 3 * PN_HC * 4, CB_BYTES = CB_RSC + PN_RSC_BYTES;
static_assert(3 * CB_BYTES <= 160 * 1024, "three colour workgroups must fit the 160 KB LDS");

__device__ __forceinline__ void cb_epilogue(const f32x16 (&acc)[2][2], unsigned mw, char *X, int wave, int lane) {
#pragma unroll
    for (int rb = 0; rb < 2; ++rb)
#pragma unroll
        for (int g = 0; g < 4; ++g) {
            const int f0 = pn_d_feat(wave, g, lane), row = 32 * rb + (lane & 31), e = rb * 16 + g * 4;
            float v[4];
#pragma unroll
            for (int i = 0; i < 4; ++i) v[i] = acc[0][rb][4 * g + i] * ((int)(mw << (e + i)) < 0 ? 0.01f : 1.f);
            pn_x_store4<true, CB_XRS, CB_XPL>(X, row, f0, v[0], v[1], v[2], v[3]);
        }
}
__device__ __forceinline__ void cb_bias_sums(const char *X, const PnRowScale &rs, int tid, float *__restrict__ gsum) {
    const int cp = tid & 63, r0 = 16 * (tid >> 6);
    float g0 = 0.f, g1 = 0.f;
#pragma unroll
    for (int rr = 0; rr < 16; ++rr) {
        const unsigned h = *reinterpret_cast<const unsigned *>(X + (r0 + rr) * CB_XRS + cp * 4);
        const unsigned m = *reinterpret_cast<const unsigned *>(X + CB_XPL + (r0 + rr) * CB_XRS + cp * 4);
        const float f = rs.to_call(r0 + rr);
        g0 = pn_fma2_lo(h, m, f, g0); g1 = pn_fma2_hi(h, m, f, g1);
    }
    float2 *d = reinterpret_cast<float2 *>(gsum) + cp;
    const float2 t = *d;
    *d = make_float2(t.x + g0, t.y + g1);
}

__device__ __forceinline__ void cb_add4(float *__restrict__ d, const float (&v)[4]) {
    float4 *p = reinterpret_cast<float4 *>(d);
    const float4 t = *p;
    *p = make_float4(t.x + v[0], t.y + v[1], t.z + v[2], t.w + v[3]);
}

template <bool WG2>
__global__ __launch_bounds__(256, 3) void k_color_backward(BwdArgs a) {
    extern __shared__ __attribute__((aligned(16))) char smem_cb[];
    char *X = smem_cb;
    float *draw = reinterpret_cast<float *>(smem_cb + CB_DRAW);
    const PnRowScale rs{reinterpret_cast<float *>(smem_cb + CB_RSC)};
    const int Ns = a.counters[0] < a.cap_samples ? a.counters[0] : (int)a.cap_samples;
    const float *P = a.params;
    const char *img = reinterpret_cast<const char *>(a.packed);
    float S, invS;
    pn_scale_from_bits(a.sv.gscale[0], S, invS);
    if (blockIdx.x == 0 && threadIdx.x == 0) a.sv.cls_info[PN_CI_CTILES] = (Ns + PN_CTILE - 1) / PN_CTILE;
    float *gacc = reinterpret_cast<float *>(smem_cb + CB_GACC);
    for (int i = threadIdx.x; i < 4 * CB_GSUMS; i += 256) gacc[i] = 0.f;
    float *gaccw = gacc + (threadIdx.x >> 6) * CB_GSUMS;
    float gb4x = 0.f, gb4y = 0.f, gb4z = 0.f;
    auto row_sample = [&](long long t) -> long long {
        const long long vs = t * PN_CTILE + threadIdx.x;
        return (threadIdx.x < PN_CTILE && vs < Ns) ? (long long)a.valid_list[vs] : -1;
    };
    float po[3] = {0.f, 0.f, 0.f}, pg[3] = {0.f, 0.f, 0.f}, pgs = 0.f;
    auto row_values = [&](long long si) {
        if (si >= 0) {
            const float *o = a.decoded + si * 4, *g = a.grad_decoded + si * 4;
            po[0] = o[1]; po[1] = o[2]; po[2] = o[3]; pgs = g[0]; pg[0] = g[1]; pg[1] = g[2]; pg[2] = g[3];
        }
    };
    long long si_cur = row_sample(blockIdx.x);
    row_values(si_cur);
    float *w4s = reinterpret_cast<float *>(smem_cb + CB_W4);
    for (int i = threadIdx.x; i < 3 * PN_HC; i += 256) w4s[i] = P[PO_WC4 + i] * pn_col_scale(a.packed, PN_CS_C3)[i & (PN_HC - 1)];

    f32x16 acc[2][2];
    for (long long tile = blockIdx.x; tile * PN_CTILE < Ns; tile += gridDim.x) {
        int tid = threadIdx.x;
        asm volatile("" : "+v"(tid));
        const int lane = tid & 63, wave = __builtin_amdgcn_readfirstlane(tid >> 6);
        const long long grow0 = tile * PN_CTILE;
        float4 c3v[8];
#pragma unroll
        for (int rr = 0; rr < 8; ++rr) c3v[rr] = *reinterpret_cast<const float4 *>(a.sv.c3 + (grow0 + 8 * (tid >> 5) + rr) * PN_HC + 4 * (tid & 31));
        const unsigned mw2 = a.sv.cmask[(tile * 2 + 1) * 256 + tid], mw1 = a.sv.cmask[(tile * 2 + 0) * 256 + tid];
        PN_LDS_BARRIER();
        if (tid < PN_CTILE) {
            float d0 = 0.f, d1 = 0.f, d2 = 0.f, Si = S, invSi = invS;
            if (si_cur >= 0) {
                pn_sample_scale(make_float4(pgs, pg[0], pg[1], pg[2]), S, invS, Si, invSi);
                const float s0 = (po[0] + 0.001f) / 1.002f, s1 = (po[1] + 0.001f) / 1.002f, s2 = (po[2] + 0.001f) / 1.002f;
                d0 = pg[0] * 1.002f * s0 * (1.f - s0); d1 = pg[1] * 1.002f * s1 * (1.f - s1); d2 = pg[2] * 1.002f * s2 * (1.f - s2);
            }
            *reinterpret_cast<float4 *>(draw + tid * 4) = make_float4(d0, d1, d2, Si);
            rs.set(tid, Si, invSi, S);
            gb4x += d0; gb4y += d1; gb4z += d2;
        }
        const long long si_next = row_sample(tile + gridDim.x);
        PN_LDS_BARRIER();
        {
            const int c4 = tid & 31, rg = tid >> 5;
            float w4[3][4], gw4[3][4], gb3[4] = {0.f, 0.f, 0.f, 0.f};
#pragma unroll
            for (int k = 0; k < 3; ++k) {
                const float4 w = *reinterpret_cast<const float4 *>(w4s + k * PN_HC + 4 * c4);
                w4[k][0] = w.x; w4[k][1] = w.y; w4[k][2] = w.z; w4[k][3] = w.w;
#pragma unroll
                for (int i = 0; i < 4; ++i) gw4[k][i] = 0.f;
            }
#pragma unroll
            for (int rr = 0; rr < 8; ++rr) {
                const int row = 8 * rg + rr;
                const float4 d = *reinterpret_cast<const float4 *>(draw + row * 4);
                const float c[4] = {c3v[rr].x, c3v[rr].y, c3v[rr].z, c3v[rr].w};
                float u[4];
#pragma unroll
                for (int i = 0; i < 4; ++i) {
                    u[i] = (d.x * w4[0][i] + d.y * w4[1][i] + d.z * w4[2][i]) * pn_lrelu_grad(c[i]);
                    gw4[0][i] += d.x * c[i]; gw4[1][i] += d.y * c[i]; gw4[2][i] += d.z * c[i];
                    gb3[i] += u[i];
                }
                pn_x_store4<true, CB_XRS, CB_XPL>(X, row, 4 * c4, u[0] * d.w, u[1] * d.w, u[2] * d.w, u[3] * d.w);
            }
#pragma unroll
            for (int i = 0; i < 4; ++i) {
#pragma unroll
                for (int k = 0; k < 3; ++k) gw4[k][i] += __shfl_xor(gw4[k][i], 32, 64);
                gb3[i] += __shfl_xor(gb3[i], 32, 64);
            }
            if (lane < 32) {
#pragma unroll
                for (int k = 0; k < 3; ++k) cb_add4(gaccw + k * PN_HC + 4 * c4, gw4[k]);
                cb_add4(gaccw + 3 * PN_HC + 4 * c4, gb3);
            }
        }
        PnGemmW<8, 4, 1, 4, 3> WD3;
        WD3.prefetch(reinterpret_cast<const uint4 *>(img + PKH_DC3), wave, lane);
        PN_LDS_BARRIER();
        pn_copy_out_kmajor_hs<PN_HC, CB_XRS>(X, rs, a.sv.dc3k, tile * 8, tid);
        if (WG2) pn_copy_out_kmajor_hs<PN_HC, CB_XRS>(X + CB_XPL, rs, a.sv.dc3m, tile * 8, tid);
        pn_acc_zero(acc);
        pn_gemm_f16x3_run<8, 4, 1, 4, 3, CB_XRS, CB_XPL>(X, WD3, lane, acc);
        row_values(si_next);
        si_cur = si_next;
        PN_LDS_BARRIER();
        cb_epilogue(acc, mw2, X, wave, lane);
        PnGemmW<8, 4, 1, 4, 3> WD2;
        WD2.prefetch(reinterpret_cast<const uint4 *>(img + PKH_DC2), wave, lane);
        PN_LDS_BARRIER();
        cb_bias_sums(X, rs, tid, gaccw + 4 * PN_HC);
        pn_copy_out_kmajor_hs<PN_HC, CB_XRS>(X, rs, a.sv.dc2k, tile * 8, tid);
        if (WG2) pn_copy_out_kmajor_hs<PN_HC, CB_XRS>(X + CB_XPL, rs, a.sv.dc2m, tile * 8, tid);
        pn_acc_zero(acc);
        pn_gemm_f16x3_run<8, 4, 1, 4, 3, CB_XRS, CB_XPL>(X, WD2, lane, acc);
        PN_LDS_BARRIER();
        cb_epilogue(acc, mw1, X, wave, lane);
        PnGemmW<8, 8, 2, 1, 3> WD1;
        WD1.prefetch(reinterpret_cast<const uint4 *>(img + PKH_DC1), 2 * wave, lane);
        PN_LDS_BARRIER();
        cb_bias_sums(X, rs, tid, gaccw + 5 * PN_HC);
        pn_copy_out_kmajor_hs<PN_HC, CB_XRS>(X, rs, a.sv.dc1k, tile * 8, tid);
        if (WG2) pn_copy_out_kmajor_hs<PN_HC, CB_XRS>(X + CB_XPL, rs, a.sv.dc1m, tile * 8, tid);
        pn_acc_zero(acc);
        pn_gemm_f16x3_run<8, 8, 2, 1, 3, CB_XRS, CB_XPL>(X, WD1, lane, acc);
#pragma unroll
        for (int fb = 0; fb < 2; ++fb)
#pragma unroll
            for (int rb = 0; rb < 2; ++rb) {
                const float ri = rs.inv(32 * rb + (lane & 31));
#pragma unroll
                for (int g = 0; g < 4; ++g) {
                    pn_f4 t = {acc[fb][rb][4 * g] * ri, acc[fb][rb][4 * g + 1] * ri, acc[fb][rb][4 * g + 2] * ri, acc[fb][rb][4 * g + 3] * ri};
                    PN_REG_STORE(t, reinterpret_cast<pn_f4 *>(a.sv.dfs + (grow0 + 32 * rb + (lane & 31)) * PN_H + pn_d_feat(2 * wave + fb, g, lane)));
                }
            }
    }
    PN_LDS_BARRIER();
    {
        const int tid = threadIdx.x;
        auto total = [&](int i) { return (gacc[i] + gacc[CB_GSUMS + i]) + (gacc[2 * CB_GSUMS + i] + gacc[3 * CB_GSUMS + i]); };
        for (int i = tid; i < 3 * PN_HC; i += 256) atomicAdd(&a.gparams[PO_WC4 + i], total(i));
        if (tid < PN_HC) {
            atomicAdd(&a.gparams[PO_BC3 + tid], total(3 * PN_HC + tid) * pn_col_scale_inv(a.packed, PN_CS_C3)[tid]);
            atomicAdd(&a.gparams[PO_BC2 + tid], total(4 * PN_HC + tid) * invS * pn_col_scale_inv(a.packed, PN_CS_C2)[tid]);
            atomicAdd(&a.gparams[PO_BC1 + tid], total(5 * PN_HC + tid) * invS * pn_col_scale_inv(a.packed, PN_CS_C1)[tid]);
        }
        if (tid < PN_CTILE) {
#pragma unroll
            for (int off = 32; off > 0; off >>= 1) { gb4x += __shfl_xor(gb4x, off, 64); gb4y += __shfl_xor(gb4y, off, 64); gb4z += __shfl_xor(gb4z, off, 64); }
            if (tid == 0) { atomicAdd(&a.gparams[PO_BC4], gb4x); atomicAdd(&a.gparams[PO_BC4 + 1], gb4y); atomicAdd(&a.gparams[PO_BC4 + 2], gb4z); }
        }
    }
}

constexpr int BL_ROW = PN_XBYTES, BL_RSC = BL_ROW + 10 * PN_TILE * 4, BL_W5 = BL_RSC + PN_RSC_BYTES, BL_CLAIM = BL_W5 + PN_H * 4 ,
              BL_C4 = BL_CLAIM + 16 , BL_BYTES = BL_C4 + PN_H * 4;
constexpr int LDDX = 228;
static_assert(2 * BL_BYTES <= 160 * 1024, "two backward workgroups must fit the 160 KB LDS");
static_assert(PN_TILE * LDDX * 4 <= PN_XBYTES, "d X0 tile");
constexpr int LDDX_X = 292, BL_GW = BL_BYTES, BL_BYTES_X = BL_GW + PN_TILE * 4;
static_assert(2 * BL_BYTES_X <= 160 * 1024, "two xyz_grad backward workgroups must fit the 160 KB LDS");
static_assert(PN_TILE * LDDX_X * 4 <= PN_XBYTES, "d X0 tile (xyz_grad)");

template <bool MIX = false>
__device__ __forceinline__ void b_epilogue(const f32x16 (&acc)[PN_NFB][2], const unsigned (&mask)[PN_NFB], char *X, int wave, int lane) {
#pragma unroll
    for (int fb = 0; fb < PN_NFB; ++fb) {
        const unsigned mw = mask[fb];
#pragma unroll
        for (int rb = 0; rb < 2; ++rb)
#pragma unroll
            for (int g = 0; g < 4; ++g) {
                float v[4];
#pragma unroll
                for (int i = 0; i < 4; ++i) {
                    const int e = (rb * 4 + g) * 4 + i;
                    v[i] = acc[fb][rb][4 * g + i] * ((int)(mw << e) < 0 ? 0.01f : 1.f);
                }
                if (MIX) pn_xq_store4(X, 32 * rb + (lane & 31), pn_d_feat(PN_NFB * wave + fb, g, lane), v[0], v[1], v[2], v[3]);
                else pn_x_store4<true>(X, 32 * rb + (lane & 31), pn_d_feat(PN_NFB * wave + fb, g, lane), v[0], v[1], v[2], v[3]);
            }
    }
}

#ifdef PN_EMU
#define PN_WAVE_LDS_SYNC() __syncthreads()
#else
#define PN_WAVE_LDS_SYNC() asm volatile("s_waitcnt lgkmcnt(0)" ::: "memory")
#endif

template <int KC, bool MIX = false, bool XG = false>
__device__ __forceinline__ void b_front(const BwdArgs &a, char *X, const float *w5s, const float *c4is, const float *wrow, const float *wnrm, const float *dsg, const float *xrow,
                                        float *draw, const int *sidx, const int *prow, const float4 (&dfr)[4], const float *dfb0, const PnRowScale &rs, int tid,
                                        float (&gw5)[8], float &gb5t, unsigned kinv = 0u, float *gwf = nullptr) {
    const int lane = tid & 63, cg = tid & 31, r0 = 8 * (tid >> 5);
    const int j0 = KC == 0 ? pn_row_div(r0, kinv) : 0;
    float zo_conf = 0.f;
    if (a.zo_gs && (lane & 3) == 0) {
        const int rz = prow[r0 + ((lane >> 4) & 1) * 4 + ((lane >> 3) & 1) * 2 + ((lane >> 2) & 1)];
        if (rz >= 0) zo_conf = a.conf[rz];
    }
    auto df_of = [&](int j, float4 &ga, float4 &gb) {
        if (KC >= 4) { ga = dfr[2 * j]; gb = dfr[2 * j + 1]; }
        else { ga = *reinterpret_cast<const float4 *>(dfb0 + j * PN_H); gb = *reinterpret_cast<const float4 *>(dfb0 + j * PN_H + 4); }
    };
    const float4 cia = *reinterpret_cast<const float4 *>(c4is + 8 * cg), cib = *reinterpret_cast<const float4 *>(c4is + 8 * cg + 4);
    float pd[8];
#pragma unroll
    for (int i = 0; i < 8; ++i) {
        const int r = r0 + i, j = KC == 0 ? pn_row_div(r, kinv) - j0 : i / (KC == 0 ? 1 : KC);
        const uint4 h = *reinterpret_cast<const uint4 *>(X + r * PN_XRS + cg * 16);
        const uint4 m = *reinterpret_cast<const uint4 *>(X + PN_XPLANE + r * PN_XRS + cg * 16);
        float4 ga, gb;
        df_of(j, ga, gb);
        ga.x *= cia.x; ga.y *= cia.y; ga.z *= cia.z; ga.w *= cia.w; gb.x *= cib.x; gb.y *= cib.y; gb.z *= cib.z; gb.w *= cib.w;
        float s = 0.f;
        s = pn_fma2_lo(h.x, m.x, ga.x, s); s = pn_fma2_hi(h.x, m.x, ga.y, s); s = pn_fma2_lo(h.y, m.y, ga.z, s); s = pn_fma2_hi(h.y, m.y, ga.w, s);
        s = pn_fma2_lo(h.z, m.z, gb.x, s); s = pn_fma2_hi(h.z, m.z, gb.y, s); s = pn_fma2_lo(h.w, m.w, gb.z, s); s = pn_fma2_hi(h.w, m.w, gb.w, s);
        pd[i] = s;
    }
    {
        const bool b4 = lane & 16, b3 = lane & 8, b2 = lane & 4;
#pragma unroll
        for (int j = 0; j < 4; ++j) { const float send = b4 ? pd[j] : pd[j + 4], keep = b4 ? pd[j + 4] : pd[j]; pd[j] = keep + __shfl_xor(send, 16, 64); }
#pragma unroll
        for (int j = 0; j < 2; ++j) { const float send = b3 ? pd[j] : pd[j + 2], keep = b3 ? pd[j + 2] : pd[j]; pd[j] = keep + __shfl_xor(send, 8, 64); }
        { const float send = b2 ? pd[0] : pd[1], keep = b2 ? pd[1] : pd[0]; pd[0] = keep + __shfl_xor(send, 4, 64); }
        pd[0] += __shfl_xor(pd[0], 2, 64);
        pd[0] += __shfl_xor(pd[0], 1, 64);
        const int r = r0 + ((lane >> 4) & 1) * 4 + ((lane >> 3) & 1) * 2 + ((lane >> 2) & 1);
        if ((lane & 3) == 0) {
            float dr = 0.f, gw = 0.f;
            if (sidx[r] >= 0) {
                const float x = xrow[r], dotf = pd[0] * rs.S(r);
                const float alpha = pn_softplus(x), sg = pn_sigmoid(x);
                const int rp = prow[r];
                float zo_eps = a.zo_eps;
                asm volatile("" : "+s"(zo_eps));
                if (rp >= 0) atomicAdd(&a.g_conf[rp], (dsg[r] * alpha + dotf) * wnrm[r] * rs.inv(r) + (a.zo_gs ? PnZeroOne(zo_conf, zo_eps).grad(a.zo_gs[0]) : 0.f));
                if (XG && rp >= 0) gw = dsg[r] * alpha + dotf;
                dr = dsg[r] * wrow[r] * sg;
            }
            draw[r] = dr;
            if (XG) gwf[r] = gw;
        }
    }
    PN_WAVE_LDS_SYNC();
    const float4 wa = *reinterpret_cast<const float4 *>(w5s + 8 * cg), wb = *reinterpret_cast<const float4 *>(w5s + 8 * cg + 4);
    const float w5[8] = {wa.x, wa.y, wa.z, wa.w, wb.x, wb.y, wb.z, wb.w};
    float drsum = 0.f;
#pragma unroll
    for (int i = 0; i < 8; ++i) {
        const int r = r0 + i, j = KC == 0 ? pn_row_div(r, kinv) - j0 : i / (KC == 0 ? 1 : KC);
        const uint4 h = *reinterpret_cast<const uint4 *>(X + r * PN_XRS + cg * 16);
        const uint4 m = *reinterpret_cast<const uint4 *>(X + PN_XPLANE + r * PN_XRS + cg * 16);
        const bool live = sidx[r] >= 0;
        const float dr = draw[r], w = rs.wS(r), drc = dr * rs.to_call(r);
        drsum += drc;
        const float hv[8] = {pn_h_lo(h.x) + pn_h_lo(m.x), pn_h_hi(h.x) + pn_h_hi(m.x), pn_h_lo(h.y) + pn_h_lo(m.y), pn_h_hi(h.y) + pn_h_hi(m.y),
                             pn_h_lo(h.z) + pn_h_lo(m.z), pn_h_hi(h.z) + pn_h_hi(m.z), pn_h_lo(h.w) + pn_h_lo(m.w), pn_h_hi(h.w) + pn_h_hi(m.w)};
        float4 ga, gb;
        df_of(j, ga, gb);
        const float g[8] = {ga.x, ga.y, ga.z, ga.w, gb.x, gb.y, gb.z, gb.w};
        float o[8];
#pragma unroll
        for (int c = 0; c < 8; ++c) {
            o[c] = live ? (w * g[c] + dr * w5[c]) * pn_lrelu_grad(hv[c]) : 0.f;
            gw5[c] += drc * hv[c];
        }
        unsigned oh[4], om[4];
#pragma unroll
        for (int c = 0; c < 4; ++c) pn_split2_sat(o[2 * c], o[2 * c + 1], oh[c], om[c]);
        *reinterpret_cast<uint4 *>(X + r * PN_XRS + cg * 16) = make_uint4(oh[0], oh[1], oh[2], oh[3]);
        if (MIX) *reinterpret_cast<uint4 *>(X + PN_XPLANE + r * PN_XRS + cg * 16) =
                     make_uint4(pn_q8x4(oh[0], oh[1], 1.0f), pn_q8x4(oh[2], oh[3], 1.0f), pn_q8x4(om[0], om[1], PN_MIX_MSC), pn_q8x4(om[2], om[3], PN_MIX_MSC));
        else *reinterpret_cast<uint4 *>(X + PN_XPLANE + r * PN_XRS + cg * 16) = make_uint4(om[0], om[1], om[2], om[3]);
    }
    if (cg == 0) gb5t += drsum;
}

__device__ __forceinline__ void b_xyz_row(const BwdXArgs &a, const float *dxr, const float *gwf, const float *wrow, const float *wnrm, const int *sidx,
                                          int rp, int row, int q, int K, unsigned kinv, float invS) {
    float u[6] = {0.f, 0.f, 0.f, 0.f, 0.f, 0.f}, t = 0.f;
    float dwx = 0.f, dwy = 0.f, dwz = 0.f;
    if (rp >= 0) {
        const long long si = sidx[row];
        const float px = a.xyz[3 * rp], py = a.xyz[3 * rp + 1], pz = a.xyz[3 * rp + 2];
        const float lx = a.sample_loc[si * 3], ly = a.sample_loc[si * 3 + 1], lz = a.sample_loc[si * 3 + 2];
// ... 735 lines not shown
                const uint4 *fa = smem_x + ra * WX_AU + (2 * kk + (lane >> 5)) * MF + (lane & 31);
                const uint4 *fb = smem_x + WX_OFF_B + (s & 1) * WX_BU + (2 * kk + (lane >> 5)) * WX_NB + (lane & 31);
                const uint4 *ft = smem_x + WX_OFF_T + ra * WX_TU + (2 * kk + (lane >> 5)) * 64 + (lane & 31);
                pn_h8 ah[MTW], bh[2];
#pragma unroll
                for (int i = 0; i < MTW; ++i) ah[i] = __builtin_bit_cast(pn_h8, fa[(MTW * wm + i) * 32]);
                const pn_h8 tah = __builtin_bit_cast(pn_h8, fa[(MTW * wm + wn) * 32]);
                bh[0] = __builtin_bit_cast(pn_h8, fb[(2 * wn) * 32]);
                bh[1] = __builtin_bit_cast(pn_h8, wn < 3 ? fb[(2 * wn + 1) * 32] : ft[0]);
#pragma unroll
                for (int i = 0; i < MTW; ++i)
#pragma unroll
                    for (int j = 0; j < 2; ++j)
                        acc[i][j] = __builtin_amdgcn_mfma_f32_32x32x16_f16(ah[i], bh[j], acc[i][j], 0, 0, 0);
                acct = __builtin_amdgcn_mfma_f32_32x32x16_f16(tah, __builtin_bit_cast(pn_h8, ft[32]), acct, 0, 0, 0);
            }
            build_into(lds + (size_t)(WX_OFF_B + ((s + 1) & 1) * WX_BU) * 16, lds + (size_t)(WX_OFF_G + rgs * WX_GU) * 16);
            if (wave >= 1 && wave <= WX_RG && s + 1 + WX_GD < nst) {
                const int p = reinterpret_cast<const int4 *>(smem_x + WX_OFF_RM + rrm * WX_RS)[8 * (wave - 1) + (lane & 7)].y;
                p_gather = p < 0 ? 0 : (p >= g.n_points ? g.n_points - 1 : p);
            }
            bump(ia, WX_NST); bump(ig, WX_G_SLOTS); bump(irm, WX_RM_SLOTS); bump(ra, WX_NST); bump(rgs, WX_G_SLOTS); bump(rrm, WX_RM_SLOTS);
        }
    }
    float *out = partial + (size_t)blockIdx.x * 256 * 288;
#pragma unroll
    for (int i = 0; i < MTW; ++i)
#pragma unroll
        for (int j = 0; j < 2; ++j)
#pragma unroll
            for (int r = 0; r < 16; ++r) {
                const int m = (MTW * wm + i) * 32 + (r & 3) + 8 * (r >> 2) + 4 * (lane >> 5);
                out[(size_t)m * 288 + (2 * wn + j) * 32 + (lane & 31)] = acc[i][j][r];
            }
#pragma unroll
    for (int r = 0; r < 16; ++r) {
        const int m = (MTW * wm + wn) * 32 + (r & 3) + 8 * (r >> 2) + 4 * (lane >> 5);
        out[(size_t)m * 288 + 256 + (lane & 31)] = acct[r];
    }
}

int launch_wgrad_x0(const uint4 *A, const WgX0Args &g, const int *d_tiles, long long rows_max, float *partial, const unsigned *gscale, const float *cinv,
                    float *grad, hipStream_t s) {
    int chunks = WG_CHUNKS;
    const long long tiles = rows_max / PN_TILE;
    if (tiles < chunks) chunks = (int)(tiles > 0 ? tiles : 1);
    if ((size_t)chunks * 256 * 288 > PARTIAL_FLOATS) return PNERF_E_WS;
    constexpr size_t lds = (size_t)WX_UNITS * 16;
    if (hipFuncSetAttribute((const void *)k_wgrad_x0, hipFuncAttributeMaxDynamicSharedMemorySize, (int)lds) != hipSuccess) return PNERF_E_LAUNCH;
    { PnProfScope prof(PNK_WGRAD, s);
    hipLaunchKernelGGL(k_wgrad_x0, dim3(chunks), dim3(512), lds, s, A, g, d_tiles, partial); }
    PnProfScope prof(PNK_WGRAD_REDUCE, s);
    hipLaunchKernelGGL(k_wgrad_reduce_f16, dim3(pn_cdiv((long long)PN_H * 288, 64)), dim3(256), 0, s, partial, chunks, PN_H, PN_IN1, PN_ONES1, gscale, cinv, grad, (int)PO_W1, (int)PN_IN1, (int)PO_B1);
    PN_CHECK_LAUNCH();
    return 0;
}
}

size_t pn_wgrad_partials_bytes() { return pn_align(PARTIAL_FLOATS * sizeof(float)); }

namespace {
__global__ void k_zero_one_empty(const float *__restrict__ conf, const int *__restrict__ counters, long long slots_per_ray, const float *__restrict__ gs, float eps,
                                 float *__restrict__ g_conf) {
    const long long n_empty = (long long)counters[1] * slots_per_ray - (long long)counters[3];
    if (n_empty <= 0) return;
    const float g = PnZeroOne(conf[0], eps).grad(gs[0]);
    if (g != 0.f) atomicAdd(&g_conf[0], g * (float)n_empty);
}
}

int pn_agg_backward_launch(const pnerf_camera *cam, const pnerf_points *pts, const pnerf_step &st, const float *d_decoded, const float *d_weight,
                           const float *d_grad_decoded, const PnSaved &sv, float *d_grad_params, const pnerf_point_grads *pg,
                           float *d_partials, bool x0_saved, hipStream_t s) {
    const int K = st.K;
    const long long n_valid = st.n_valid_max;
    const PnArith ar = pn_arith();
    BwdArgs a;
    a.cam = *cam; a.params = st.params; a.packed = (const float4 *)st.packed_mlp; a.raydir = st.raydir;
    a.pidx = st.sample_pidx; a.valid_list = st.valid_list; a.counters = st.counters;
    a.SR = st.SR; a.K = K; a.TS = pn_tile_samples(K); a.cap_samples = n_valid;
    a.decoded = d_decoded; a.weight = d_weight; a.grad_decoded = d_grad_decoded; a.sv = sv;
    a.emb = pts->embedding;
    a.gparams = d_grad_params; a.g_emb = pg->embedding; a.g_conf = pg->conf; a.g_dir = pg->dir; a.g_color = pg->color;
    a.conf = pts->conf; a.zo_gs = x0_saved ? nullptr : pg->zero_one_gscale; a.zo_eps = pg->zero_one_eps;
    if (a.zo_gs && !a.conf) return PNERF_E_INVAL;
    if (!a.g_emb || !a.g_conf || !a.g_dir || !a.g_color) return PNERF_E_INVAL;
    BwdXArgs ax;
    ax.xyz = pts->xyz; ax.sample_loc = st.sample_loc; ax.g_xyz = pg->xyz;
    const bool xg = ax.g_xyz != nullptr;
    if (xg && x0_saved) return PNERF_E_UNSUP;
    if (xg && (!ax.xyz || !ax.sample_loc)) return PNERF_E_INVAL;
    const int ncu = pn_cu_count();
    if (!ncu) return PNERF_E_LAUNCH;
    const int grid_c = pn_tile_grid((n_valid + PN_CTILE - 1) / PN_CTILE, 3LL * ncu);
    const size_t lds_c = CB_BYTES, lds_a = xg ? BL_BYTES_X : BL_BYTES;
    const bool wg2 = sv.wg2 != 0;
    if (wg2) x0_saved = true;
    const bool mix = !wg2 && (ar.mix_mask() & 4);
    void (*const kcb)(BwdArgs) = wg2 ? k_color_backward<true> : k_color_backward<false>;
    void (*const kab)(BwdArgs) = wg2 ? k_agg_backward<true> : mix ? k_agg_backward<false, true> : k_agg_backward<false>;
    void (*const kax)(BwdXArgs) = wg2 ? k_agg_backward<true, false, true> : mix ? k_agg_backward<false, true, true> : k_agg_backward<false, false, true>;
    if (hipFuncSetAttribute(reinterpret_cast<const void *>(kcb), hipFuncAttributeMaxDynamicSharedMemorySize, (int)lds_c) != hipSuccess) return PNERF_E_LAUNCH;
    if (hipFuncSetAttribute(xg ? reinterpret_cast<const void *>(kax) : reinterpret_cast<const void *>(kab), hipFuncAttributeMaxDynamicSharedMemorySize, (int)lds_a) != hipSuccess) return PNERF_E_LAUNCH;
    a.cls_list = sv.cls_list; a.cls_info = sv.cls_info; a.valid_list = sv.cls_list;
    if (hipMemsetAsync(sv.gscale, 0, PN_GS_WORDS * sizeof(unsigned), s) != hipSuccess) return PNERF_E_LAUNCH;
    hipLaunchKernelGGL(k_grad_max, dim3(pn_capped_grid((n_valid + 255) / 256, 1024)), dim3(256), 0, s, sv.cls_list, st.counters, n_valid, d_grad_decoded, sv.gscale);
    if (a.zo_gs) hipLaunchKernelGGL(k_zero_one_empty, dim3(1), dim3(1), 0, s, a.conf, st.counters, (long long)st.SR * K, a.zo_gs, a.zo_eps, a.g_conf);
    { PnProfScope prof(PNK_COLOR_BWD, s);
      hipLaunchKernelGGL(kcb, dim3(grid_c), dim3(256), lds_c, s, a); }
    int kc[PN_NCLS];
    const int ncls = pn_class_slots(K, kc);
    { PnProfScope prof(PNK_AGG_BWD, s);
      for (int j = 0; j < ncls; ++j) {
          a.cls = j; a.K = kc[j]; a.TS = pn_tile_samples(kc[j]);
          const int grid_a = pn_tile_grid((n_valid + a.TS - 1) / a.TS, 2LL * ncu);
          if (xg) { static_cast<BwdArgs &>(ax) = a; hipLaunchKernelGGL(kax, dim3(grid_a), dim3(PN_NTHR), lds_a, s, ax); }
          else hipLaunchKernelGGL(kab, dim3(grid_a), dim3(PN_NTHR), lds_a, s, a);
      } }
    PN_CHECK_LAUNCH();
    if (pg->ready_event && hipEventRecord((hipEvent_t)pg->ready_event, s) != hipSuccess) return PNERF_E_LAUNCH;
    const long long rows = sv.rows, smps = sv.samples;
    const int *dt = sv.cls_info + PN_CI_TILES, *ct = sv.cls_info + PN_CI_CTILES;
    const float *ci = reinterpret_cast<const float *>(reinterpret_cast<const char *>(st.packed_mlp) + PKC_SCALE) + PN_CS_UNITS;
    const WgLayer layers[7] = {
        {WG_288x256, sv.dy1k, sv.x0k, sv.dy1m, sv.x0m, dt, rows, PO_W1, PN_IN1, PN_IN1, PN_ONES1, PO_B1, ci + PN_CS_L1},
        {WG_256x256, sv.dy2k, sv.h1k, sv.dy2m, sv.h1m, dt, rows, PO_W2, PN_H, PN_H, PN_H, PO_B2, ci + PN_CS_L2},
        {WG_288x256, sv.dy3k, sv.h2k, sv.dy3m, sv.h2m, dt, rows, PO_W3, PN_IN3, PN_IN3, PN_ONES3, PO_B3, ci + PN_CS_L3},
        {WG_256x256, sv.dy4k, sv.h3k, sv.dy4m, sv.h3m, dt, rows, PO_W4, PN_H, PN_H, PN_H, PO_B4, ci + PN_CS_L4},
        {WG_288x128, sv.dc1k, sv.xck, sv.dc1m, sv.xcm, ct, smps, PO_WC1, PN_INC, PN_INC, -1, 0, ci + PN_CS_C1},
        {WG_128x128, sv.dc2k, sv.c1k, sv.dc2m, sv.c1m, ct, smps, PO_WC2, PN_HC, PN_HC, -1, 0, ci + PN_CS_C2},
        {WG_128x128, sv.dc3k, sv.c2k, sv.dc3m, sv.c2m, ct, smps, PO_WC3, PN_HC, PN_HC, -1, 0, ci + PN_CS_C3},
    };
    for (const WgLayer &L : layers) {
        int rc;
        if (&L == layers && !x0_saved) {
            WgX0Args wa;
            wa.rmeta = sv.rmeta; wa.emb = pts->embedding; wa.x0t = sv.x0k; wa.n_points = pts->n;
            rc = launch_wgrad_x0(L.dy, wa, dt, rows, d_partials, sv.gscale, L.cinv, d_grad_params, s);
        } else {
            rc = wg2 ? launch_wgrad_layer<true>(L, d_partials, sv.gscale, d_grad_params, s) : launch_wgrad_layer<false>(L, d_partials, sv.gscale, d_grad_params, s);
        }
        if (rc) return rc;
    }
    return 0;
}

#ifdef PN_PHASE_TRACE
extern "C" int pnerf_debug_trace_bwd(void *host, size_t bytes) {
    return hipMemcpyFromSymbol(host, HIP_SYMBOL(pn_trace_bwd), bytes < sizeof(pn_trace_bwd) ? bytes : sizeof(pn_trace_bwd)) == hipSuccess ? 0 : -1;
}
extern "C" int pnerf_debug_span_bwd(void *host, size_t bytes) {
    return hipMemcpyFromSymbol(host, HIP_SYMBOL(pn_span_bwd), bytes < sizeof(pn_span_bwd) ? bytes : sizeof(pn_span_bwd)) == hipSuccess ? 0 : -1;
}
#endif
```

pointnerf_amd/csrc/grid.hip:

```cpp
#include <limits.h>
#include "pn_ray.h"

PnGridLayout pn_grid_layout(const pnerf_grid_params *gp, int n) {
    PnGridLayout L;
    L.G = (long long)gp->vdim[0] * gp->vdim[1] * gp->vdim[2];
    L.NB = (long long)pn_cdiv(gp->vdim[0], 4) * pn_cdiv(gp->vdim[1], 4) * pn_cdiv(gp->vdim[2], 4);
    const size_t np = (size_t)(n > 0 ? n : 1);
    size_t off = 0;
    auto take = [&](size_t bytes) { size_t o = off; off += pn_align(bytes); return o; };
    L.info = take(PNERF_GI_LEN * sizeof(int));
    L.bricks = take((size_t)L.NB * sizeof(uint4));
    L.occ = take((size_t)((L.G + 31) / 32) * sizeof(uint32_t));
    L.pts = take(np * sizeof(float4));
    L.ostart = take((np + 2) * sizeof(int));
    L.keys = take(np * sizeof(int));
    L.cnt = take((size_t)L.NB * 64 * sizeof(int));
    L.tmp_idx = take(np * sizeof(int));
    L.ocell = take((np + 1) * sizeof(int));
    L.bocc = take((size_t)(L.NB + 1) * sizeof(int));
    L.bpts = take((size_t)(L.NB + 1) * sizeof(int));
    L.brank = take((size_t)(L.NB + 1) * sizeof(int));
    L.bbase = take((size_t)(L.NB + 1) * sizeof(int));
    L.scan = take(pn_scan_scratch_ints(L.NB) * sizeof(int));
    L.total = off;
// ... 91 lines not shown
    int pre = c;
#pragma unroll
    for (int d = 1; d < 64; d <<= 1) { const int v = __shfl_up(pre, d, 64); if (lane >= d) pre += v; }
    if (c > 0) {
        const int o = rank0 + __popcll(bits & ((1ull << lane) - 1ull));
        const int st = base0 + pre - c;
        ostart[o] = st;
        ocell[o] = key;
        cnt[key] = st;
    }
}

__global__ __launch_bounds__(TPB) void k_grid_scatter(const int *__restrict__ keys, int n, int *__restrict__ cursor, int *__restrict__ tmp_idx) {
    int i = blockIdx.x * TPB + threadIdx.x;
    if (i >= n) return;
    int key = keys[i];
    if (key < 0) return;
    tmp_idx[atomicAdd(&cursor[key], 1)] = i;
}

__global__ __launch_bounds__(TPB) void k_grid_finalize(GP g, int n, const float *__restrict__ xyz, const int *__restrict__ ostart,
                                                       const int *__restrict__ ocell, int *__restrict__ tmp_idx,
                                                       float4 *__restrict__ pts, uint32_t *__restrict__ occ, const int *info) {
    const int o = blockIdx.x * TPB + threadIdx.x;
    if (o >= n || o >= info[PNERF_GI_N_OCC]) return;
    const int s = ostart[o], m = ostart[o + 1] - s;
    for (int a = 1; a < m; ++a) {
        int v = tmp_idx[s + a];
        int b = a - 1;
        while (b >= 0 && tmp_idx[s + b] > v) { tmp_idx[s + b + 1] = tmp_idx[s + b]; --b; }
        tmp_idx[s + b + 1] = v;
    }
    for (int a = 0; a < m; ++a) {
        int idx = tmp_idx[s + a];
        pts[s + a] = make_float4(xyz[3 * idx], xyz[3 * idx + 1], xyz[3 * idx + 2], __int_as_float(idx));
    }
    const int key = ocell[o], brick = key >> 6, local = key & 63;
    const int bzi = brick % g.bz, byi = (brick / g.bz) % g.by, bxi = brick / (g.bz * g.by);
    const int cx = bxi * 4 + (local >> 4), cy = byi * 4 + ((local >> 2) & 3), cz = bzi * 4 + (local & 3);
    int x0 = max(0, cx - g.qx / 2), x1 = min(g.gx, cx + (g.qx + 1) / 2);
    int y0 = max(0, cy - g.qy / 2), y1 = min(g.gy, cy + (g.qy + 1) / 2);
    int z0 = max(0, cz - g.qz / 2), z1 = min(g.gz, cz + (g.qz + 1) / 2);
    for (int x = x0; x < x1; ++x)
        for (int y = y0; y < y1; ++y)
            for (int z = z0; z < z1; ++z) {
                long long lin = (long long)x * (g.gy * g.gz) + (long long)y * g.gz + z;
                atomicOr(&occ[lin >> 5], 1u << (lin & 31));
            }
}
}

extern "C" size_t pnerf_grid_workspace_bytes(const pnerf_grid_params *gp, int n_points) {
    if (!gp) return 0;
    return pn_grid_layout(gp, n_points).total;
}

extern "C" int pnerf_grid_build(const pnerf_grid_params *gp, const float *d_xyz, int n, void *ws, size_t ws_bytes,
                                void *stream) {
    if (!gp || !ws || (n > 0 && !d_xyz) || n < 0) return PNERF_E_INVAL;
    for (int a = 0; a < 3; ++a)
        if (gp->vdim[a] <= 0 || !(gp->vsize[a] > 0.f) || gp->query_size[a] <= 0 || gp->kernel_size[a] <= 0) return PNERF_E_INVAL;
    PnGridLayout L = pn_grid_layout(gp, n);
    if (L.G <= 0 || L.G >= (1LL << 31) - 64 || L.NB * 64 >= (1LL << 31) - 64) return PNERF_E_UNSUP;
    if (ws_bytes < L.total) return PNERF_E_WS;
    hipStream_t s = (hipStream_t)stream;
    char *b = (char *)ws;
    int *info = (int *)(b + L.info), *ostart = (int *)(b + L.ostart), *keys = (int *)(b + L.keys), *cnt = (int *)(b + L.cnt);
    int *tmp_idx = (int *)(b + L.tmp_idx), *ocell = (int *)(b + L.ocell), *scan = (int *)(b + L.scan);
    int *bocc = (int *)(b + L.bocc), *bpts = (int *)(b + L.bpts), *brank = (int *)(b + L.brank), *bbase = (int *)(b + L.bbase);
    uint4 *bricks = (uint4 *)(b + L.bricks);
    uint32_t *occ = (uint32_t *)(b + L.occ);
    float4 *pts = (float4 *)(b + L.pts);
    GP g = {gp->ranges[0], gp->ranges[1], gp->ranges[2], gp->vsize[0], gp->vsize[1], gp->vsize[2],
            gp->vdim[0], gp->vdim[1], gp->vdim[2], gp->query_size[0], gp->query_size[1], gp->query_size[2],
            pn_cdiv(gp->vdim[1], 4), pn_cdiv(gp->vdim[2], 4)};

    PnProfScope prof(PNK_GRID, s);
    hipLaunchKernelGGL(k_grid_init, dim3(1), dim3(TPB), 0, s, info, (int)(L.ostart / 256));
    if (hipMemsetAsync(cnt, 0, (size_t)L.NB * 64 * sizeof(int), s) != hipSuccess) return PNERF_E_LAUNCH;
    if (hipMemsetAsync(occ, 0, (size_t)((L.G + 31) / 32) * sizeof(uint32_t), s) != hipSuccess) return PNERF_E_LAUNCH;
    if (n > 0) hipLaunchKernelGGL(k_grid_count, dim3(pn_cdiv(n, TPB)), dim3(TPB), 0, s, g, d_xyz, n, keys, cnt, info);
    hipLaunchKernelGGL(k_grid_cell0, dim3(1), dim3(1), 0, s, keys, n, info);
    const int nbw = (int)pn_cdiv(L.NB, TPB / 64);
    hipLaunchKernelGGL(k_brick_bits, dim3(nbw), dim3(TPB), 0, s, L.NB, cnt, bocc, bpts, info);
    int rc = pn_exclusive_scan_i32(bocc, brank, L.NB, scan, s);
    if (rc) return rc;
    rc = pn_exclusive_scan_i32(bpts, bbase, L.NB, scan, s);
    if (rc) return rc;
    hipLaunchKernelGGL(k_brick_fill, dim3(nbw), dim3(TPB), 0, s, L.NB, cnt, brank, bbase, bricks, ostart, ocell, info);
    if (n > 0) {
        hipLaunchKernelGGL(k_grid_scatter, dim3(pn_cdiv(n, TPB)), dim3(TPB), 0, s, keys, n, cnt, tmp_idx);
        hipLaunchKernelGGL(k_grid_finalize, dim3(pn_cdiv(n, TPB)), dim3(TPB), 0, s, g, n, d_xyz, ostart, ocell, tmp_idx, pts, occ, info);
    }
    PN_CHECK_LAUNCH();
    return 0;
}

extern "C" int pnerf_grid_info(const void *ws, int32_t *host_info, void *stream) {
    if (!ws || !host_info) return PNERF_E_INVAL;
    hipStream_t s = (hipStream_t)stream;
    if (hipMemcpyAsync(host_info, ws, PNERF_GI_LEN * sizeof(int), hipMemcpyDeviceToHost, s) != hipSuccess) return PNERF_E_LAUNCH;
    if (hipStreamSynchronize(s) != hipSuccess) return PNERF_E_LAUNCH;
    return 0;
}

namespace {
__device__ __forceinline__ unsigned pn_fkey(float f) { const unsigned b = __float_as_uint(f); return (b & 0x80000000u) ? ~b : (b | 0x80000000u); }
__device__ __forceinline__ float pn_fkey_inv(unsigned k) { return __uint_as_float((k & 0x80000000u) ? (k & 0x7fffffffu) : ~k); }
__global__ void k_minmax_init(unsigned *__restrict__ key) { if (threadIdx.x < 6) key[threadIdx.x] = threadIdx.x < 3 ? 0xffffffffu : 0u; }
__global__ __launch_bounds__(256) void k_minmax(const float *__restrict__ xyz, long long n, unsigned *__restrict__ key) {
    unsigned mn[3] = {0xffffffffu, 0xffffffffu, 0xffffffffu}, mx[3] = {0u, 0u, 0u};
    for (long long i = (long long)blockIdx.x * 256 + threadIdx.x; i < n; i += (long long)gridDim.x * 256) {
#pragma unroll
        for (int c = 0; c < 3; ++c) {
            const unsigned k = pn_fkey(xyz[3 * i + c]);
            mn[c] = min(mn[c], k); mx[c] = max(mx[c], k);
        }
    }
#pragma unroll
    for (int c = 0; c < 3; ++c) {
#pragma unroll
        for (int off = 32; off > 0; off >>= 1) { mn[c] = min(mn[c], __shfl_xor(mn[c], off, 64)); mx[c] = max(mx[c], __shfl_xor(mx[c], off, 64)); }
    }
    __shared__ unsigned red[4][6];
    if ((threadIdx.x & 63) == 0) {
#pragma unroll
        for (int c = 0; c < 3; ++c) { red[threadIdx.x >> 6][c] = mn[c]; red[threadIdx.x >> 6][3 + c] = mx[c]; }
    }
    __syncthreads();
    if (threadIdx.x < 6) {
        unsigned v = red[0][threadIdx.x];
        for (int w = 1; w < 4; ++w) v = threadIdx.x < 3 ? min(v, red[w][threadIdx.x]) : max(v, red[w][threadIdx.x]);
        if (threadIdx.x < 3) atomicMin(&key[threadIdx.x], v); else atomicMax(&key[threadIdx.x], v);
    }
}
__global__ void k_minmax_decode(unsigned *__restrict__ key) {
    if (threadIdx.x < 6) { const float f = pn_fkey_inv(key[threadIdx.x]); key[threadIdx.x] = __float_as_uint(f); }
}
}

extern "C" int pnerf_points_minmax(const float *d_xyz, int64_t n, float *d_out6, void *stream) {
    if (!d_xyz || !d_out6 || n <= 0) return PNERF_E_INVAL;
    hipStream_t s = (hipStream_t)stream;
    unsigned *key = reinterpret_cast<unsigned *>(d_out6);
    PnProfScope prof(PNK_GRID, s);
    hipLaunchKernelGGL(k_minmax_init, dim3(1), dim3(64), 0, s, key);
    const int blocks = (int)(n / 256 < 512 ? (n + 255) / 256 : 512);
    hipLaunchKernelGGL(k_minmax, dim3(blocks), dim3(256), 0, s, d_xyz, (long long)n, key);
    hipLaunchKernelGGL(k_minmax_decode, dim3(1), dim3(64), 0, s, key);
    PN_CHECK_LAUNCH();
    return 0;
}

extern "C" int pnerf_version(void) { return 1009; }
extern "C" const char *pnerf_arch(void) { return "gfx950"; }
```

pointnerf_amd/csrc/mlp_common.h:

```cpp
#pragma once
#include "pn_common.h"
#include <type_traits>
#include <utility>

#define PN_F      32
#define PN_IN1    284
#define PN_IN1P   288
#define PN_H      256
#define PN_IN3    263
#define PN_INC    280
#define PN_HC     128
#define PN_TILE   64
#define PN_MT     (PN_TILE / 32)
#define PN_NTHR   256
#define PN_NW     4
#define PN_NFB    2
static_assert(PN_NTHR == 64 * PN_NW && PN_NW == 4 && PN_NW * PN_NFB == 8, "the tile kernels are written for 4 waves x 2 of the 8 feature blocks each");
#define PN_TPR    (PN_NTHR / PN_TILE)
#define PN_EPT    (PN_F / PN_TPR)
#define PN_CTILE  64

enum : int {
    PO_W1 = 0, PO_B1 = PO_W1 + PN_H * PN_IN1, PO_W2 = PO_B1 + PN_H, PO_B2 = PO_W2 + PN_H * PN_H,
    PO_W3 = PO_B2 + PN_H, PO_B3 = PO_W3 + PN_H * PN_IN3, PO_W4 = PO_B3 + PN_H, PO_B4 = PO_W4 + PN_H * PN_H,
    PO_W5 = PO_B4 + PN_H, PO_B5 = PO_W5 + PN_H, PO_WC1 = PO_B5 + 1, PO_BC1 = PO_WC1 + PN_HC * PN_INC,
    PO_WC2 = PO_BC1 + PN_HC, PO_BC2 = PO_WC2 + PN_HC * PN_HC, PO_WC3 = PO_BC2 + PN_HC, PO_BC3 = PO_WC3 + PN_HC * PN_HC,
    PO_WC4 = PO_BC3 + PN_HC, PO_BC4 = PO_WC4 + 3 * PN_HC, PO_TOTAL = PO_BC4 + 3
};
static_assert(PO_TOTAL == 341764, "parameter count of the lego-script aggregator");

typedef float f32x16 __attribute__((ext_vector_type(16)));

typedef float pn_f4 __attribute__((ext_vector_type(4)));
typedef float pn_f2 __attribute__((ext_vector_type(2)));

__device__ __forceinline__ float pn_lrelu_grad(float post) { return post > 0.f ? 1.f : 0.01f; }

template <int... I, class F> __device__ __forceinline__ void pn_static_for_impl(std::integer_sequence<int, I...>, F &&f) { (f(std::integral_constant<int, I>{}), ...); }
template <int N, class F> __device__ __forceinline__ void pn_static_for(F &&f) { pn_static_for_impl(std::make_integer_sequence<int, N>{}, f); }

__device__ __forceinline__ void rot3(const float *M, float x, float y, float z, bool transpose, float &ox, float &oy, float &oz) {
    if (!transpose) { ox = x * M[0] + y * M[3] + z * M[6]; oy = x * M[1] + y * M[4] + z * M[7]; oz = x * M[2] + y * M[5] + z * M[8]; }
    else { ox = x * M[0] + y * M[1] + z * M[2]; oy = x * M[3] + y * M[4] + z * M[5]; oz = x * M[6] + y * M[7] + z * M[8]; }
}
template <int N> __device__ __forceinline__ float group_sum(float v) {
#pragma unroll
    for (int off = 1; off < N; off <<= 1) v += __shfl_xor(v, off, 64);
    return v;
}
template <int AF> __device__ __forceinline__ void pn_acc_zero(f32x16 (&acc)[AF][2]) {
#pragma unroll
    for (int i = 0; i < AF; ++i)
#pragma unroll
        for (int j = 0; j < 2; ++j)
#pragma unroll
            for (int r = 0; r < 16; ++r) acc[i][j][r] = 0.f;
}
__device__ __forceinline__ float pn_softplus(float x) {
#ifdef PN_EMU
    return x > 20.f ? x : log1pf(expf(x));
#else
    return x > 20.f ? x : __logf(1.0f + __expf(x));
#endif
}
__device__ __forceinline__ float pn_sigmoid(float x) {
#ifdef PN_EMU
    return x > 20.f ? 1.f : 1.0f / (1.0f + expf(-x));
#else
    return x > 20.f ? 1.f : __builtin_amdgcn_rcpf(1.0f + __expf(-x));
#endif
}

struct PnSaved {
    uint4 *x0k, *h1k, *h2k, *h3k;
    uint4 *dy1k, *dy2k, *dy3k, *dy4k;
    uint4 *h4r;
    float *arow;
    int4 *rmeta;
    unsigned *lmask;
    unsigned *gscale;
    float *fs, *dfs, *c3;
    uint4 *xck, *c1k, *c2k;
    uint4 *dc1k, *dc2k, *dc3k;
    unsigned *cmask;
    uint4 *x0m, *h1m, *h2m, *h3m, *dy1m, *dy2m, *dy3m, *dy4m;
    uint4 *xcm, *c1m, *c2m, *dc1m, *dc2m, *dc3m;
    int wg2;
    int *cls_list;
    int *cls_info;
    int *cls_tmp;
    long long rows, samples;
};
enum : int { PN_NCLS = 3, PN_CI_COUNT = 0, PN_CI_VBASE = 4, PN_CI_TBASE = 8, PN_CI_TILES = 12, PN_CI_CTILES = 13 ,
              PN_CI_CLAIM = 16 , PN_CI_WORDS = 20 };
#ifndef PN_CLAIM_TILES
#define PN_CLAIM_TILES 1
#endif
enum : int { PN_CLAIM_STATIC_FWD = 4, PN_CLAIM_STATIC_BWD = 2, PN_GS_CLAIM = 4, PN_GS_WORDS = 8 };
__device__ __forceinline__ int pn_claim_tile(int nstatic, int grid, int v, int m) { return nstatic * grid + v * PN_CLAIM_TILES + m % PN_CLAIM_TILES; }
int pn_tile_grid(long long tiles, long long dflt);
int pn_class_slots(int K, int kc[3]);
int pn_classify(const PnSaved &sv, const int32_t *d_valid_list, const int32_t *d_counters, const int32_t *d_pidx, int K, long long n_valid, bool train, bool save_x0, hipStream_t s);
size_t pn_saved_walk(void *base, long long n_valid, int K, PnSaved &s);
void pn_cls_walk(PnCarver &cv, PnSaved &s);
size_t pn_saved_bytes(long long n_valid, int K);
PnSaved pn_saved_carve(void *base, long long n_valid, int K);
int pn_agg_forward_launch(const pnerf_camera *cam, const pnerf_points *pts, const pnerf_step &st, float *d_decoded, float *d_weight,
                          const PnSaved &sv, bool train, bool save_x0, hipStream_t s);
int pn_agg_backward_launch(const pnerf_camera *cam, const pnerf_points *pts, const pnerf_step &st, const float *d_decoded, const float *d_weight,
                           const float *d_grad_decoded, const PnSaved &sv, float *d_grad_params, const pnerf_point_grads *pg,
                           float *d_partials, bool x0_saved, hipStream_t s);
size_t pn_wgrad_partials_bytes();
struct PnArith {
    int products;
    int wgrad_planes;
    int cross_terms;
    int mix_where;
    int mix_mask() const { return cross_terms == 8 ? mix_where : 0; }
};
PnArith pn_arith();

__host__ __device__ inline int pn_tile_samples(int K) { return PN_TILE / K; }
__device__ __forceinline__ unsigned pn_kinv(int K) { return (65536u + (unsigned)K - 1u) / (unsigned)K; }
__device__ __forceinline__ int pn_row_div(int row, unsigned kinv) { return (int)(((unsigned)row * kinv) >> 16); }


#ifdef PN_PHASE_TRACE
#define PN_TR_WGS   512
#define PN_TR_IT0   20
#define PN_TR_ITERS 6
#define PN_TR_SLOTS 24
#define PN_TR_DECL(name) __device__ unsigned long long name[PN_TR_WGS * PN_TR_ITERS * PN_TR_SLOTS]
#define PN_TR(buf, ph)                                                                                              \
    do {                                                                                                            \
        if (tid == 0 && blockIdx.x < PN_TR_WGS && titer >= PN_TR_IT0 && titer < PN_TR_IT0 + PN_TR_ITERS)           \
            buf[((size_t)blockIdx.x * PN_TR_ITERS + (titer - PN_TR_IT0)) * PN_TR_SLOTS + (ph)] = wall_clock64();    \
    } while (0)
#define PN_TR_HWID(buf)                                                                                             \
    do {                                                                                                            \
        if (tid == 0 && blockIdx.x < PN_TR_WGS && titer >= PN_TR_IT0 && titer < PN_TR_IT0 + PN_TR_ITERS)           \
            buf[((size_t)blockIdx.x * PN_TR_ITERS + (titer - PN_TR_IT0)) * PN_TR_SLOTS + PN_TR_SLOTS - 1] =         \
                (unsigned long long)__builtin_amdgcn_s_getreg((31 << 11) | 4) |                                    \
                ((unsigned long long)__builtin_amdgcn_s_getreg((31 << 11) | 20) << 32);                             \
    } while (0)
#define PN_TR_ITER_DECL int titer = -1
#define PN_TR_ITER_NEXT ++titer
#define PN_TR_SPAN_DECL(name) __device__ unsigned long long name[PN_TR_WGS * 4]
#define PN_TR_SPAN(buf, cls, end)                                                                                   \
    do {                                                                                                            \
        if (tid == 0 && (cls) == 0 && blockIdx.x < PN_TR_WGS && ((end) || titer == 0)) {                            \
            buf[(size_t)blockIdx.x * 4 + (end)] = wall_clock64();                                                   \
            if (end) buf[(size_t)blockIdx.x * 4 + 2] = (unsigned long long)(titer + 1);                             \
        }                                                                                                           \
    } while (0)
#else
#define PN_TR(buf, ph)
#define PN_TR_HWID(buf)
#define PN_TR_ITER_DECL
#define PN_TR_ITER_NEXT
#define PN_TR_SPAN(buf, cls, end)
#endif
```

pointnerf_amd/ops.py:

```python
import ctypes
import math

import numpy as np
import torch

from . import _lib as L


def _stream():
    return ctypes.c_void_p(torch.cuda.current_stream().cuda_stream)


def _ptr(t):
    if t is None:
        return ctypes.c_void_p(0)
    assert t.is_cuda and t.is_contiguous(), "pointnerf_amd ops need contiguous device tensors"
    return ctypes.c_void_p(t.data_ptr())


def host_array(t):
    if not isinstance(t, torch.Tensor):
        return np.asarray(t)
    if not t.is_cuda:
        return t.detach().numpy()
# ... 453 lines not shown
        n_src = gs.numel() // w
        L.check(L.lib().pnerf_scatter_add_rows(_ptr(g2), _ptr(i2), i2.numel(), w, _ptr(gs), n_src, _stream()),
                "pnerf_scatter_add_rows")
        return gs, None


def gather_rows(src, idx):
    return GatherRows.apply(src, idx)


def zero_one_sum(conf_flat, pidx, ray_hit, eps):
    lib = L.lib()
    R = 0 if ray_hit is None else int(pidx.shape[0])
    part = torch.empty(lib.pnerf_zero_one_blocks(pidx.numel() if ray_hit is None else R * 256), dtype=torch.float32, device=conf_flat.device)
    if ray_hit is None:
        L.check(lib.pnerf_zero_one_forward(_ptr(conf_flat), conf_flat.numel(), _ptr(pidx), pidx.numel(), float(eps), _ptr(part), _stream()), "pnerf_zero_one_forward")
    else:
        L.check(lib.pnerf_zero_one_forward_rays(_ptr(conf_flat), conf_flat.numel(), _ptr(pidx), _ptr(ray_hit), R, int(pidx.numel() // max(R, 1)), float(eps),
                                                _ptr(part), _stream()), "pnerf_zero_one_forward_rays")
    return part.sum()


def zero_one_add_grad(conf_flat, pidx, ray_hit, eps, gscale, grad_conf_flat):
    if ray_hit is None:
        L.check(L.lib().pnerf_zero_one_backward(_ptr(conf_flat), conf_flat.numel(), _ptr(pidx), pidx.numel(), float(eps), _ptr(gscale), _ptr(grad_conf_flat),
                                                _stream()), "pnerf_zero_one_backward")
    else:
        R = int(pidx.shape[0])
        L.check(L.lib().pnerf_zero_one_backward_rays(_ptr(conf_flat), conf_flat.numel(), _ptr(pidx), _ptr(ray_hit), R, int(pidx.numel() // max(R, 1)), float(eps),
                                                     _ptr(gscale), _ptr(grad_conf_flat), _stream()), "pnerf_zero_one_backward_rays")


class ZeroOneConf(torch.autograd.Function):

    @staticmethod
    def forward(ctx, conf, pidx, ray_hit, eps):
        c = conf.detach().reshape(-1)
        _need_cuda(c, "points_conf")
        ctx.save_for_backward(c, pidx, ray_hit)
        ctx.eps, ctx.shape = float(eps), conf.shape
        return zero_one_sum(c, pidx, ray_hit, eps)

    @staticmethod
    def backward(ctx, g):
        c, pidx, ray_hit = ctx.saved_tensors
        grad = torch.zeros_like(c)
        zero_one_add_grad(c, pidx, ray_hit, ctx.eps, g.detach().reshape(1).to(torch.float32).contiguous(), grad)
        return grad.view(ctx.shape), None, None, None


def zero_one_conf_sum(conf, pidx, eps):
    return ZeroOneConf.apply(conf, pidx.contiguous().reshape(-1), None, eps)


def zero_one_conf_sum_rays(conf, pidx_dense, ray_hit, eps):
    return ZeroOneConf.apply(conf, pidx_dense.contiguous(), ray_hit.contiguous(), eps)


class ColorLossRays(torch.autograd.Function):

    @staticmethod
    def forward(ctx, ray_color, gt, ray_hit):
        _need_cuda(ray_color, "ray_color")
        lib = L.lib()
        c, g = ray_color.detach().reshape(-1, 3).contiguous().float(), gt.detach().reshape(-1, 3).contiguous().float()
        R = c.shape[0]
        part = torch.empty(lib.pnerf_color_loss_blocks(R), dtype=torch.float32, device=c.device)
        L.check(lib.pnerf_color_loss_forward_rays(_ptr(c), _ptr(g), _ptr(ray_hit), R, _ptr(part), _stream()), "pnerf_color_loss_forward_rays")
        ctx.save_for_backward(c, g, ray_hit)
        ctx.shape = ray_color.shape
        return part.sum()

    @staticmethod
    def backward(ctx, gout):
        c, g, ray_hit = ctx.saved_tensors
        grad = torch.empty_like(c)
        gs = gout.detach().reshape(1).to(torch.float32).contiguous()
        L.check(L.lib().pnerf_color_loss_backward_rays(_ptr(c), _ptr(g), _ptr(ray_hit), c.shape[0], _ptr(gs), _ptr(grad), _stream()),
                "pnerf_color_loss_backward_rays")
        return grad.view(ctx.shape), None, None


def color_loss_sum_rays(ray_color, gt, ray_hit):
    return ColorLossRays.apply(ray_color, gt, ray_hit.contiguous())


class GeometryLossRays(torch.autograd.Function):

    @staticmethod
    def forward(ctx, depth_sum, acc, bg_trans, ray_hit, gt_depth, gt_mask):
        _need_cuda(depth_sum, "depth_sum")
        lib = L.lib()
        R = int(ray_hit.numel())
        f32 = torch.float32
        flat = lambda t: t.detach().reshape(-1).contiguous().float()
        a = (flat(depth_sum), flat(acc), flat(bg_trans), ray_hit.reshape(-1).contiguous(), flat(gt_depth), flat(gt_mask))
        _dense_args("ray_hit", a[3], ("depth_sum", a[0], f32, R), ("acc", a[1], f32, R), ("bg_trans", a[2], f32, R), ("ray_hit", a[3], torch.int32, R),
                    ("gt_depth", a[4], f32, R), ("gt_mask", a[5], f32, R))
        nb = lib.pnerf_color_loss_blocks(R)
        part = torch.empty(2, nb, dtype=f32, device=a[0].device)
        L.check(lib.pnerf_geometry_loss_forward_rays(*[_ptr(t) for t in a], R, _ptr(part), _stream()), "pnerf_geometry_loss_forward_rays")
        ctx.save_for_backward(*a)
        ctx.shapes = (depth_sum.shape, acc.shape, bg_trans.shape)
        sums = part.sum(dim=1)
        return sums[0], sums[1]

    @staticmethod
    def backward(ctx, g_depth, g_bg):
        a = ctx.saved_tensors
        R = int(a[3].numel())
        dev = a[0].device
        gs = torch.stack([torch.zeros((), device=dev) if g is None else g.detach().reshape(()).to(torch.float32) for g in (g_depth, g_bg)]).contiguous()
        grad = torch.empty(R, 3, dtype=torch.float32, device=dev)
        L.check(L.lib().pnerf_geometry_loss_backward_rays(*[_ptr(t) for t in a], R, _ptr(gs), _ptr(grad), _stream()), "pnerf_geometry_loss_backward_rays")
        return grad[:, 0].reshape(ctx.shapes[0]), grad[:, 1].reshape(ctx.shapes[1]), grad[:, 2].reshape(ctx.shapes[2]), None, None, None


def geometry_loss_sums_rays(depth_sum, acc, bg_trans, ray_hit, gt_depth, gt_mask):
    return GeometryLossRays.apply(depth_sum, acc, bg_trans, ray_hit, gt_depth, gt_mask)


def set_inference_products(n):
    old = L.lib().pnerf_set_inference_products(int(n))
    if old < 0:
        raise ValueError("inference products must be 2 or 3")
    return old


def set_wgrad_planes(n):
    old = L.lib().pnerf_set_wgrad_planes(int(n))
    if old < 0:
        raise ValueError("weight-gradient planes must be 1 or 2")
    ARENA._cap_cache = {}
    return old


def set_cross_terms(bits, where=None):
    old = L.lib().pnerf_set_cross_terms(int(bits))
    if old < 0:
        raise ValueError("cross terms must be 8 or 16")
    oldw = L.lib().pnerf_set_cross_terms_where(int(where)) if where is not None else None
    if where is not None and oldw < 0:
        raise ValueError("cross-term mask must be 0..7")
    return old, oldw


def set_tile_grid(max_workgroups=0):
    old = L.lib().pnerf_debug_set_tile_grid(int(max_workgroups))
    if old < 0:
        raise ValueError("the grid cap must be >= 0")
    return old


def arithmetic():
    out = (ctypes.c_int32 * 4)()
    L.check(L.lib().pnerf_get_arithmetic(out), "pnerf_get_arithmetic")
    return tuple(int(v) for v in out)


def cross_terms_state():
    _, _, bits, mask = arithmetic()
    return bits, (mask if bits == 8 else 0)


def image_metrics_sums(img, gt, win=11, data_range=2.0, quantize8=True):
    for name, t in (("img", img), ("gt", gt)):
        _need_cuda(t, name)
        if t.dtype != torch.float32:
            raise TypeError("pointnerf_amd: image_metrics needs float32 images, %s is %s" % (name, t.dtype))
        if t.dim() != 3 or t.shape[2] != 3:
            raise ValueError("pointnerf_amd: image_metrics needs [H, W, 3] images, %s is %s" % (name, list(t.shape)))
        if not t.is_contiguous():
            raise ValueError("pointnerf_amd: image_metrics needs contiguous images, %s has strides %s" % (name, list(t.stride())))
    if img.shape != gt.shape or img.device != gt.device:
        raise ValueError("pointnerf_amd: image_metrics: img %s on %s and gt %s on %s differ" % (list(img.shape), img.device, list(gt.shape), gt.device))
    H, W = int(img.shape[0]), int(img.shape[1])
    lib = L.lib()
    nbytes = lib.pnerf_image_metrics_workspace_bytes(H, W, int(win))
    ws = torch.empty(max(nbytes, 8), dtype=torch.uint8, device=img.device)
    out4 = torch.empty(4, dtype=torch.float64, device=img.device)
    L.check(lib.pnerf_image_metrics(_ptr(img.detach()), _ptr(gt.detach()), H, W, int(win), float(data_range), 1 if quantize8 else 0,
                                    _ptr(out4), _ptr(ws), nbytes, _stream()), "pnerf_image_metrics")
    return out4


def image_metrics(img, gt, win=11, data_range=2.0, quantize8=True):
    out4 = image_metrics_sums(img, gt, win, data_range, quantize8)
    H, W = int(img.shape[0]), int(img.shape[1])
    n_win = (H - int(win) + 1) * (W - int(win) + 1)
    return torch.stack([out4[0] / float(H * W * 3), out4[1:].sum() / float(3 * n_win)])


def _f32(t, name, anchor=None):
    _need_cuda(t, name)
    if not t.is_floating_point():
        raise ValueError("pointnerf_amd: %s must be a floating-point tensor, got %s" % (name, t.dtype))
    if anchor is not None and t.device != anchor.device:
        raise ValueError("pointnerf_amd: %s is on %s, expected %s" % (name, t.device, anchor.device))
    return t.detach().float().contiguous()


def mvs_cost_volume(features, proj, depth_values, align_corners=False):
    f = _f32(features, "features")
    if f.dim() == 4:
        f = f[None]
    if f.dim() != 5:
        raise ValueError("pointnerf_amd: features must be [V,C,h,w] or [B,V,C,h,w], got %s" % list(features.shape))
    dv = _f32(depth_values, "depth_values", f)
    if dv.dim() != 2:
        raise ValueError("pointnerf_amd: depth_values must be [B,D], got %s" % list(depth_values.shape))
    B, D = dv.shape
    sets, V, C, h, w = f.shape
    _need_cuda(proj, "proj")
    if proj.dim() != 4 or proj.shape[0] != B or proj.shape[1] != V or proj.shape[2] not in (3, 4) or proj.shape[3] != 4:
        raise ValueError("pointnerf_amd: proj must be [%d,%d,3 or 4,4], got %s" % (B, V, list(proj.shape)))
    p = _f32(proj[:, :, :3, :], "proj", f)
    lib = L.lib()
    nws = lib.pnerf_mvs_cost_volume_workspace_bytes(sets, V, h, w)
    ws = torch.empty(max(nws, 8), dtype=torch.uint8, device=f.device)
    vol = torch.empty(B, C, D, h, w, dtype=torch.float32, device=f.device)
    L.check(lib.pnerf_mvs_cost_volume(_ptr(f), sets, _ptr(p), _ptr(dv), B, V, C, D, h, w, 1 if align_corners else 0, _ptr(vol), _ptr(ws), nws,
                                      _stream()), "pnerf_mvs_cost_volume")
    return vol


def mvs_depth_regress(cost_reg, depth_values, return_prob=False):
    c = _f32(cost_reg, "cost_reg")
    dv = _f32(depth_values, "depth_values", c)
    if c.dim() != 4 or dv.dim() != 2 or tuple(dv.shape) != tuple(c.shape[:2]):
        raise ValueError("pointnerf_amd: cost_reg [B,D,h,w] and depth_values [B,D] expected, got %s and %s" % (list(cost_reg.shape), list(depth_values.shape)))
    B, D, h, w = c.shape
    depth = torch.empty(B, h, w, dtype=torch.float32, device=c.device)
    conf = torch.empty(B, h, w, dtype=torch.float32, device=c.device)
    prob = torch.empty(B, D, h, w, dtype=torch.float32, device=c.device) if return_prob else None
    L.check(L.lib().pnerf_mvs_depth_regress(_ptr(c), _ptr(dv), B, D, h, w, _ptr(depth), _ptr(conf), _ptr(prob), _stream()), "pnerf_mvs_depth_regress")
    return (depth, conf, prob) if return_prob else (depth, conf)


def depth_to_cam_points(depth_lr, conf_lr, size, near_far, intrinsic):
    d = _f32(depth_lr, "depth_lr")
    c = _f32(conf_lr, "conf_lr", d)
    if d.dim() != 2 or c.shape != d.shape:
        raise ValueError("pointnerf_amd: depth_lr and conf_lr must be [h,w], got %s and %s" % (list(depth_lr.shape), list(conf_lr.shape)))
    h, w = d.shape
    H, W = int(size[0]), int(size[1])
    K = torch.tensor(np.asarray(host_array(intrinsic) if isinstance(intrinsic, torch.Tensor) else intrinsic), dtype=torch.float32).reshape(3, 3)
    M = (ctypes.c_float * 9)(*torch.inverse(K.t()).contiguous().reshape(-1).tolist())
    nf = [float(v) for v in (host_array(near_far) if isinstance(near_far, torch.Tensor) else np.asarray(near_far)).reshape(-1)[:2]]
    xyz = torch.empty(1, 1, 1, H, W, 3, dtype=torch.float32, device=d.device)
    conf = torch.empty(1, 1, H, W, dtype=torch.float32, device=d.device)
    mask = torch.empty(1, 1, H, W, dtype=torch.uint8, device=d.device)
    L.check(L.lib().pnerf_depth_to_cam_points(_ptr(d), _ptr(c), h, w, H, W, nf[0], nf[1], M, _ptr(xyz), _ptr(conf), _ptr(mask), _stream()),
            "pnerf_depth_to_cam_points")
    return xyz, conf, mask.bool()


PROBE_RAY_KEYS = (("ray_max_shading_opacity", 1), ("ray_max_sample_loc_w", 3), ("ray_max_far_dist", 1), ("shading_avg_color", 3),
                  ("shading_avg_dir", 3), ("shading_avg_conf", 1), ("shading_avg_embedding", 32))


def probe_rays(pts, opacity, weight, sample_loc, sample_pidx, ray_hit, R, SR, K):
    R, SR, K = int(R), int(SR), int(K)
    f32, i32 = torch.float32, torch.int32
    _dense_args(None, None, ("opacity", opacity, f32, R * SR), ("weight", weight, f32, R * SR * K), ("sample_loc", sample_loc, f32, R * SR * 3),
                ("sample_pidx", sample_pidx, i32, R * SR * K), ("ray_hit", ray_hit, i32, R))
    out = {k: torch.empty(R, c, dtype=f32, device=opacity.device) for k, c in PROBE_RAY_KEYS}
    L.check(L.lib().pnerf_probe_rays(ctypes.byref(pts), _ptr(opacity), _ptr(weight), _ptr(sample_loc), _ptr(sample_pidx), _ptr(ray_hit), R, SR, K,
                                     *[_ptr(out[k]) for k, _ in PROBE_RAY_KEYS], _stream()), "pnerf_probe_rays")
    return out


def probe_hole_flags(ray_mask, max_opacity, far_dist, raycolor, gt, edge, bg, opacity_thresh, far_thresh=-1.0):
    H, W = int(edge.shape[0]), int(edge.shape[1])
    n = H * W
    _need_cuda(edge, "edge")
    if edge.dtype != torch.bool or not edge.is_contiguous() or edge.dim() != 2:
        raise ValueError("pointnerf_amd: edge must be a contiguous [H, W] bool tensor")
    _dense_arg(ray_mask, "ray_mask", torch.int8, n); _dense_arg(max_opacity, "max_opacity", torch.float32, n); _dense_arg(far_dist, "far_dist", torch.float32, n)
    _dense_arg(raycolor, "raycolor", torch.float32, n * 3); _dense_arg(gt, "gt", torch.float32, n * 3)
    bg3 = (ctypes.c_float * 3)(*[float(x) for x in np.asarray(host_array(bg), dtype=np.float64).reshape(-1)[:3]])
    flags = torch.empty(H, W, dtype=torch.int32, device=edge.device)
    L.check(L.lib().pnerf_probe_hole_mask(_ptr(ray_mask), _ptr(max_opacity), _ptr(far_dist), _ptr(raycolor), _ptr(gt), _ptr(edge.view(torch.uint8)), bg3,
                                          H, W, float(opacity_thresh), float(far_thresh), _ptr(flags), _stream()), "pnerf_probe_hole_mask")
    return flags


RAY_GEOMETRY_KEYS = ("acc", "depth_sum", "depth", "median_depth", "median_slot")


def ray_geometry(cam, sample_loc, sample_nn, ray_hit, opacity, blend_w):
    _need_cuda(sample_nn, "sample_nn")
    if sample_nn.dim() != 2:
        raise ValueError("pointnerf_amd: sample_nn must be [R, SR], got %s" % (list(sample_nn.shape),))
    R, SR = int(sample_nn.shape[0]), int(sample_nn.shape[1])
    f32, i32 = torch.float32, torch.int32
    _dense_args("sample_nn", sample_nn, ("sample_loc", sample_loc, f32, R * SR * 3), ("sample_nn", sample_nn, i32, R * SR), ("ray_hit", ray_hit, i32, R),
                ("opacity", opacity, f32, R * SR), ("blend_w", blend_w, f32, R * SR))
    dev = sample_nn.device
    rows = torch.empty(4, R, dtype=f32, device=dev)
    out = {k: rows[i] for i, k in enumerate(RAY_GEOMETRY_KEYS[:4])}
    out["median_slot"] = torch.empty(R, dtype=i32, device=dev)
    L.check(L.lib().pnerf_ray_geometry(ctypes.byref(cam), _ptr(sample_loc), _ptr(sample_nn), _ptr(ray_hit), _ptr(opacity), _ptr(blend_w), R, SR,
                                       *[_ptr(out[k]) for k in RAY_GEOMETRY_KEYS], _stream()), "pnerf_ray_geometry")
    out["_rows"] = rows
    return out

# ... 132 lines not shown
```

Before: 2.158 million.

## Single-pass sample classification and atomic tile claiming for colour kernels

Replaces the per-class flag plus compaction plus gather loop (three launches per class) with a three-kernel count, offset-scan and scatter scheme that uses wave ballots to rank samples. It also switches the colour forward and backward persistent loops from a static grid stride to dynamic tile claiming through an atomic counter, with some tiles still assigned statically. The aim is to remove launch overhead in classification and load imbalance across workgroups in the colour MLP kernels. In exchange it adds atomics and extra LDS per workgroup, and it relies on the claim counters being zeroed beforehand.

After: 2.172 million (median of 6 runs). About the same (+0.6%).

```diff
diff --git a/include/pnerf.h b/include/pnerf.h
--- a/include/pnerf.h
+++ b/include/pnerf.h
@@ -145,6 +145,10 @@
 int pnerf_set_cross_terms_where(int mask);
 int pnerf_get_arithmetic(int32_t out[4]);
 int pnerf_debug_set_tile_grid(int max_workgroups);
+size_t pnerf_debug_classify_workspace_bytes(int64_t n);
+int pnerf_debug_classify_info_words(void);
+int pnerf_debug_classify(const int32_t *d_valid_list, const int32_t *d_counters, const int32_t *d_pidx, int K, int64_t n, int32_t *d_cls_list,
+                         int32_t *d_cls_info, void *d_ws, size_t ws_bytes, void *stream);
 
 int pnerf_render_backward(const pnerf_camera *cam, const pnerf_points *pts, const pnerf_step *step,
                           const float *d_decoded, const float *d_weight, const float *d_grad_ray_color,
diff --git a/pointnerf_amd/_lib.py b/pointnerf_amd/_lib.py
--- a/pointnerf_amd/_lib.py
+++ b/pointnerf_amd/_lib.py
@@ -8,7 +8,7 @@
 
 c_int, c_i64, c_f32, c_void_p, c_size_t = ctypes.c_int, ctypes.c_int64, ctypes.c_float, ctypes.c_void_p, ctypes.c_size_t
 
-ABI_VERSION = 1009
+ABI_VERSION = 1010
 PNERF_MAX_K = 16
 DF_PAIR_FLOATS = 32
 GI_N_IN_GRID, GI_N_OCC, GI_MAX_CNT, GI_CELL0, GI_FIRST_IDX, GI_LEN = 0, 1, 2, 3, 4, 8
@@ -127,6 +127,9 @@
     "pnerf_set_cross_terms_where": (c_int, [c_int]),
     "pnerf_get_arithmetic": (c_int, [ctypes.POINTER(ctypes.c_int32)]),
     "pnerf_debug_set_tile_grid": (c_int, [c_int]),
+    "pnerf_debug_classify_workspace_bytes": (c_size_t, [c_i64]),
+    "pnerf_debug_classify_info_words": (c_int, []),
+    "pnerf_debug_classify": (c_int, [c_void_p, c_void_p, c_void_p, c_int, c_i64, c_void_p, c_void_p, c_void_p, c_size_t, c_void_p]),
     "pnerf_compact_workspace_bytes": (c_size_t, [c_i64]),
     "pnerf_touched_flags": (c_int, [c_void_p, c_i64, c_int, c_void_p, c_void_p]),
     "pnerf_compact_valid": (c_int, [c_void_p, c_i64, c_void_p, c_void_p, c_void_p, c_size_t, c_void_p]),
diff --git a/pointnerf_amd/csrc/aggregate.hip b/pointnerf_amd/csrc/aggregate.hip
--- a/pointnerf_amd/csrc/aggregate.hip
+++ b/pointnerf_amd/csrc/aggregate.hip
@@ -339,10 +339,11 @@
     pn_cls_walk(cv, s);
     return cv.off;
 }
+static size_t pn_cls_tmp_ints(long long samples) { return (size_t)2 * samples + pn_scan_scratch_ints(samples) + 8; }
 void pn_cls_walk(PnCarver &cv, PnSaved &s) {
     s.cls_list = cv.take<int>((size_t)s.samples);
     s.cls_info = cv.take<int>(PN_CI_WORDS);
-    s.cls_tmp = cv.take<int>((size_t)2 * s.samples + pn_scan_scratch_ints(s.samples) + 8);
+    s.cls_tmp = cv.take<int>(pn_cls_tmp_ints(s.samples));
 }
 size_t pn_saved_bytes(long long n_valid, int K) { PnSaved s; return pn_saved_walk(nullptr, n_valid, K, s); }
 PnSaved pn_saved_carve(void *base, long long n_valid, int K) { PnSaved s; pn_saved_walk(base, n_valid, K, s); return s; }
@@ -376,33 +377,105 @@
 namespace {
 struct ClsArgs { const int *valid_list, *counters, *pidx; int K, n, ncls; int kc[PN_NCLS], ts[PN_NCLS]; };
 
-__global__ void k_cls_flags(ClsArgs c, int which, int *__restrict__ flags) {
-    const int vs = blockIdx.x * blockDim.x + threadIdx.x;
-    if (vs >= c.n) return;
+constexpr int CLS_TPB = 1024, CLS_NW = CLS_TPB / 64, CLS_NONE = PN_NCLS ;
+
+__device__ __forceinline__ int cls_wave_rank(int cl, int lane, int (&cnt)[PN_NCLS]) {
+    const unsigned long long below = (1ull << lane) - 1ull;
+    int rank = 0;
+#pragma unroll
+    for (int j = 0; j < PN_NCLS; ++j) {
+        const unsigned long long m = __ballot(cl == j);
+        cnt[j] = __popcll(m);
+        if (cl == j) rank = __popcll(m & below);
+    }
+    return rank;
+}
+
+__global__ __launch_bounds__(CLS_TPB) void k_cls_count(ClsArgs c, unsigned char *__restrict__ cls, int *__restrict__ bsum, int nb) {
+    __shared__ int wcnt[CLS_NW][PN_NCLS];
+    const int vs = blockIdx.x * CLS_TPB + threadIdx.x, lane = threadIdx.x & 63, wave = threadIdx.x >> 6;
     const int Ns = c.counters[0] < c.n ? c.counters[0] : c.n;
-    int f = 0;
+    int cl = CLS_NONE;
     if (vs < Ns) {
         const long long si = c.valid_list[vs];
         int hv = 0;
         for (int k = 0; k < c.K; ++k)
             if (c.pidx[si * c.K + k] >= 0) hv = k + 1;
-        int cl = 0;
+        cl = 0;
         for (int j = 1; j < c.ncls; ++j)
             if (hv <= c.kc[j]) cl = j;
-        f = cl == which;
-    }
-    flags[vs] = f;
-}
-
-__global__ void k_cls_gather(ClsArgs c, int which, const int *__restrict__ pos, const int *__restrict__ count, int *__restrict__ cls_list,
-                             int *__restrict__ info) {
-    const int n = *count, base = info[PN_CI_VBASE + which];
-    for (int i = blockIdx.x * blockDim.x + threadIdx.x; i < n; i += gridDim.x * blockDim.x) cls_list[base + i] = c.valid_list[pos[i]];
-    if (blockIdx.x == 0 && threadIdx.x == 0) {
-        const int tiles = (n + c.ts[which] - 1) / c.ts[which], tb = info[PN_CI_TBASE + which];
-        info[PN_CI_COUNT + which] = n;
-        if (which + 1 < PN_NCLS) { info[PN_CI_VBASE + which + 1] = base + n; info[PN_CI_TBASE + which + 1] = tb + tiles + 1; }
-        info[PN_CI_TILES] = tb + tiles + 1;
+    }
+    if (vs < c.n) cls[vs] = (unsigned char)cl;
+    int cnt[PN_NCLS];
+    cls_wave_rank(cl, lane, cnt);
+    if (lane == 0)
+        for (int j = 0; j < PN_NCLS; ++j) wcnt[wave][j] = cnt[j];
+    __syncthreads();
+    if (threadIdx.x < PN_NCLS) {
+        int t = 0;
+        for (int w = 0; w < CLS_NW; ++w) t += wcnt[w][threadIdx.x];
+        bsum[threadIdx.x * nb + blockIdx.x] = t;
+    }
+}
+
+__global__ __launch_bounds__(256) void k_cls_offsets(ClsArgs c, int *__restrict__ bsum, int nb, int *__restrict__ info) {
+    __shared__ int wtot[4][PN_NCLS];
+    const int lane = threadIdx.x & 63, wave = threadIdx.x >> 6;
+    int carry[PN_NCLS] = {0, 0, 0};
+    for (int base = 0; base < nb; base += 256) {
+        const int i = base + threadIdx.x;
+        int v[PN_NCLS], x[PN_NCLS];
+#pragma unroll
+        for (int j = 0; j < PN_NCLS; ++j) x[j] = v[j] = i < nb ? bsum[j * nb + i] : 0;
+#pragma unroll
+        for (int off = 1; off < 64; off <<= 1)
+#pragma unroll
+            for (int j = 0; j < PN_NCLS; ++j) {
+                const int y = __shfl_up(x[j], off, 64);
+                if (lane >= off) x[j] += y;
+            }
+        if (lane == 63)
+            for (int j = 0; j < PN_NCLS; ++j) wtot[wave][j] = x[j];
+        __syncthreads();
+#pragma unroll
+        for (int j = 0; j < PN_NCLS; ++j) {
+            int woff = 0, tot = 0;
+            for (int w = 0; w < 4; ++w) {
+                const int t = wtot[w][j];
+                if (w < wave) woff += t;
+                tot += t;
+            }
+            if (i < nb) bsum[j * nb + i] = carry[j] + woff + x[j] - v[j];
+            carry[j] += tot;
+        }
+        __syncthreads();
+    }
+    if (threadIdx.x == 0) {
+        int vb = 0, tb = 0;
+        for (int j = 0; j < c.ncls; ++j) {
+            const int n = carry[j], tiles = (n + c.ts[j] - 1) / c.ts[j];
+            info[PN_CI_COUNT + j] = n;
+            vb += n; tb += tiles + 1;
+            if (j + 1 < PN_NCLS) { info[PN_CI_VBASE + j + 1] = vb; info[PN_CI_TBASE + j + 1] = tb; }
+            info[PN_CI_TILES] = tb;
+        }
+    }
+}
+
+__global__ __launch_bounds__(CLS_TPB) void k_cls_scatter(ClsArgs c, const unsigned char *__restrict__ cls, const int *__restrict__ bsum, int nb,
+                                                         const int *__restrict__ info, int *__restrict__ cls_list) {
+    __shared__ int wcnt[CLS_NW][PN_NCLS];
+    const int vs = blockIdx.x * CLS_TPB + threadIdx.x, lane = threadIdx.x & 63, wave = threadIdx.x >> 6;
+    const int cl = vs < c.n ? cls[vs] : CLS_NONE;
+    int cnt[PN_NCLS];
+    const int rank = cls_wave_rank(cl, lane, cnt);
+    if (lane == 0)
+        for (int j = 0; j < PN_NCLS; ++j) wcnt[wave][j] = cnt[j];
+    __syncthreads();
+    if (cl < PN_NCLS) {
+        int pos = info[PN_CI_VBASE + cl] + bsum[cl * nb + blockIdx.x] + rank;
+        for (int w = 0; w < wave; ++w) pos += wcnt[w][cl];
+        cls_list[pos] = c.valid_list[vs];
     }
 }
 
@@ -440,17 +513,28 @@
     for (int j = 0; j < PN_NCLS; ++j) c.ts[j] = c.kc[j] > 0 ? pn_tile_samples(c.kc[j]) : 1;
     if (hipMemsetAsync(sv.cls_info, 0, PN_CI_WORDS * sizeof(int), s) != hipSuccess) return PNERF_E_LAUNCH;
     if (n_valid <= 0) return 0;
-    int *flags = sv.cls_tmp, *pos = flags + n_valid, *cnt = pos + n_valid, *scratch = cnt + 8;
+    unsigned char *cls = reinterpret_cast<unsigned char *>(sv.cls_tmp);
+    int *bsum = sv.cls_tmp + n_valid;
+    const int nb = pn_cdiv(n_valid, CLS_TPB);
     PnProfScope prof(PNK_COMPACT, s);
-    for (int j = 0; j < c.ncls; ++j) {
-        hipLaunchKernelGGL(k_cls_flags, dim3(pn_cdiv(n_valid, 256)), dim3(256), 0, s, c, j, flags);
-        int rc = pn_compact_gt0_i32(flags, n_valid, pos, cnt, scratch, s);
-        if (rc) return rc;
-        hipLaunchKernelGGL(k_cls_gather, dim3(256), dim3(256), 0, s, c, j, pos, cnt, sv.cls_list, sv.cls_info);
-    }
+    hipLaunchKernelGGL(k_cls_count, dim3(nb), dim3(CLS_TPB), 0, s, c, cls, bsum, nb);
+    hipLaunchKernelGGL(k_cls_offsets, dim3(1), dim3(256), 0, s, c, bsum, nb, sv.cls_info);
+    hipLaunchKernelGGL(k_cls_scatter, dim3(nb), dim3(CLS_TPB), 0, s, c, cls, bsum, nb, sv.cls_info, sv.cls_list);
     if (train) hipLaunchKernelGGL(k_cls_zero_gaps, dim3(9, c.ncls), dim3(256), 0, s, sv, c.ncls, save_x0 ? 1 : 0);
     PN_CHECK_LAUNCH();
     return 0;
+}
+
+extern "C" size_t pnerf_debug_classify_workspace_bytes(int64_t n) { return n < 0 ? 0 : pn_cls_tmp_ints(n) * sizeof(int); }
+extern "C" int pnerf_debug_classify_info_words(void) { return PN_CI_WORDS; }
+extern "C" int pnerf_debug_classify(const int32_t *d_valid_list, const int32_t *d_counters, const int32_t *d_pidx, int K, int64_t n, int32_t *d_cls_list,
+                                    int32_t *d_cls_info, void *d_ws, size_t ws_bytes, void *stream) {
+    if (K <= 0 || K > PNERF_MAX_K || n < 0 || n > 0x7fffffffLL || !d_counters || !d_cls_info) return PNERF_E_INVAL;
+    if (n > 0 && (!d_valid_list || !d_pidx || !d_cls_list || !d_ws)) return PNERF_E_INVAL;
+    if (ws_bytes < pnerf_debug_classify_workspace_bytes(n)) return PNERF_E_WS;
+    PnSaved sv{};
+    sv.cls_list = d_cls_list; sv.cls_info = d_cls_info; sv.cls_tmp = static_cast<int *>(d_ws); sv.samples = n;
+    return pn_classify(sv, d_valid_list, d_counters, d_pidx, K, n, false, false, (hipStream_t)stream);
 }
 
 
@@ -904,7 +988,7 @@
     }
 }
 
-constexpr int CL_W4 = PN_XBYTES, CL_BYTES = CL_W4 + 3 * PN_HC * 4;
+constexpr int CL_W4 = PN_XBYTES, CL_CLAIM = CL_W4 + 3 * PN_HC * 4 , CL_BYTES = CL_CLAIM + 16;
 static_assert(2 * CL_BYTES <= 160 * 1024, "two colour workgroups must fit the 160 KB LDS");
 
 __device__ __forceinline__ void c_load_bias(const float *__restrict__ bias, int wave, int lane, float4 (&b)[4]) {
@@ -939,6 +1023,9 @@
     return mw;
 }
 
+#ifdef PN_PHASE_TRACE
+PN_TR_SPAN_DECL(pn_span_cfwd);
+#endif
 template <bool TRAIN, int NP, bool WG2 = false, bool FRAMES = false>
 __global__ __launch_bounds__(256, 2) void k_color_forward(typename FwdArgsOf<FRAMES>::type a) {
     extern __shared__ __attribute__((aligned(16))) char smem_c[];
@@ -950,13 +1037,19 @@
     for (int i = threadIdx.x; i < 3 * PN_HC; i += 256) w4s[i] = P[PO_WC4 + i];
     const float b40 = P[PO_BC4], b41 = P[PO_BC4 + 1], b42 = P[PO_BC4 + 2];
 
+    int *claim_ctr = a.sv.cls_info + PN_CI_CLAIM_COLOR, *claim_w = reinterpret_cast<int *>(smem_c + CL_CLAIM);
     f32x16 acc[2][2];
-    for (long long tile = blockIdx.x; tile * PN_CTILE < Ns; tile += gridDim.x) {
+    PN_TR_ITER_DECL;
+    for (long long tile = blockIdx.x; tile * PN_CTILE < Ns;) {
+        PN_TR_ITER_NEXT;
         int tid = threadIdx.x;
         asm volatile("" : "+v"(tid));
+        PN_TR_SPAN(pn_span_cfwd, 0, 0);
         const int lane = tid & 63, wave = __builtin_amdgcn_readfirstlane(tid >> 6), row = tid >> 2, q = tid & 3;
         const long long grow0 = tile * PN_CTILE, vs = grow0 + row;
         const int si = vs < Ns ? a.valid_list[vs] : -1;
+        int claimed = 0;
+        if (tid == 0) claimed = atomicAdd(claim_ctr, 1);
         PnGemmW<18, 4, 1, 7, NP> WC1;
         WC1.prefetch(reinterpret_cast<const uint4 *>(img + PKH_FC1), wave, lane);
         PN_LDS_BARRIER();
@@ -997,7 +1090,9 @@
         pn_acc_zero(acc);
         pn_gemm_f16x3_run<18, 4, 1, 7, NP>(X, WC1, lane, acc);
         c_load_bias(P + PO_BC1, wave, lane, bias);
-        PN_LDS_BARRIER();
+        if (tid == 0) *claim_w = claimed;
+        PN_LDS_BARRIER();
+        const long long tile_next = pn_claim_tile(PN_CLAIM_STATIC_CFWD, gridDim.x, __builtin_amdgcn_readfirstlane(*claim_w), 0);
         unsigned mw = c_epilogue<TRAIN, false>(acc, bias, X, wave, lane, nullptr, grow0);
         if (TRAIN) a.sv.cmask[(tile * 2 + 0) * 256 + tid] = mw;
         PnGemmW<8, 4, 1, 7, NP> WC2;
@@ -1037,6 +1132,8 @@
                 o[3] = 1.0f / (1.0f + expf(-(o2 + b42))) * 1.002f - 0.001f;
             }
         }
+        PN_TR_SPAN(pn_span_cfwd, 0, 1);
+        tile = tile_next;
     }
 }
 }
@@ -1147,4 +1244,7 @@
 extern "C" int pnerf_debug_span_fwd(void *host, size_t bytes) {
     return hipMemcpyFromSymbol(host, HIP_SYMBOL(pn_span_fwd), bytes < sizeof(pn_span_fwd) ? bytes : sizeof(pn_span_fwd)) == hipSuccess ? 0 : -1;
 }
+extern "C" int pnerf_debug_span_cfwd(void *host, size_t bytes) {
+    return hipMemcpyFromSymbol(host, HIP_SYMBOL(pn_span_cfwd), bytes < sizeof(pn_span_cfwd) ? bytes : sizeof(pn_span_cfwd)) == hipSuccess ? 0 : -1;
+}
 #endif
diff --git a/pointnerf_amd/csrc/backward.hip b/pointnerf_amd/csrc/backward.hip
--- a/pointnerf_amd/csrc/backward.hip
+++ b/pointnerf_amd/csrc/backward.hip
@@ -106,7 +106,7 @@
 
 constexpr int CB_XRS = 2 * PN_HC + 16, CB_XPL = PN_CTILE * CB_XRS, CB_XBYTES = 2 * CB_XPL;
 constexpr int CB_GSUMS = 6 * PN_HC;
-constexpr int CB_DRAW = CB_XBYTES, CB_GACC = CB_DRAW + PN_CTILE * 4 * 4, CB_W4 = CB_GACC + 4 * CB_GSUMS * 4, CB_RSC = CB_W4 + 3 * PN_HC * 4, CB_BYTES = CB_RSC + PN_RSC_BYTES;
+constexpr int CB_DRAW = CB_XBYTES, CB_GACC = CB_DRAW + PN_CTILE * 4 * 4, CB_W4 = CB_GACC + 4 * CB_GSUMS * 4, CB_RSC = CB_W4 + 3 * PN_HC * 4, CB_CLAIM = CB_RSC + PN_RSC_BYTES , CB_BYTES = CB_CLAIM + 16;
 static_assert(3 * CB_BYTES <= 160 * 1024, "three colour workgroups must fit the 160 KB LDS");
 
 __device__ __forceinline__ void cb_epilogue(const f32x16 (&acc)[2][2], unsigned mw, char *X, int wave, int lane) {
@@ -142,6 +142,9 @@
     *p = make_float4(t.x + v[0], t.y + v[1], t.z + v[2], t.w + v[3]);
 }
 
+#ifdef PN_PHASE_TRACE
+PN_TR_SPAN_DECL(pn_span_cbwd);
+#endif
 template <bool WG2>
 __global__ __launch_bounds__(256, 3) void k_color_backward(BwdArgs a) {
     extern __shared__ __attribute__((aligned(16))) char smem_cb[];
@@ -174,10 +177,17 @@
     float *w4s = reinterpret_cast<float *>(smem_cb + CB_W4);
     for (int i = threadIdx.x; i < 3 * PN_HC; i += 256) w4s[i] = P[PO_WC4 + i] * pn_col_scale(a.packed, PN_CS_C3)[i & (PN_HC - 1)];
 
+    int *claim_ctr = reinterpret_cast<int *>(a.sv.gscale) + PN_GS_CLAIM_COLOR, *claim_w = reinterpret_cast<int *>(smem_cb + CB_CLAIM);
+    long long tile_next = (long long)blockIdx.x + gridDim.x;
     f32x16 acc[2][2];
-    for (long long tile = blockIdx.x; tile * PN_CTILE < Ns; tile += gridDim.x) {
+    PN_TR_ITER_DECL;
+    for (long long tile = blockIdx.x; tile * PN_CTILE < Ns;) {
+        PN_TR_ITER_NEXT;
         int tid = threadIdx.x;
         asm volatile("" : "+v"(tid));
+        PN_TR_SPAN(pn_span_cbwd, 0, 0);
+        int claimed = 0;
+        if (tid == 0) claimed = atomicAdd(claim_ctr, 1);
         const int lane = tid & 63, wave = __builtin_amdgcn_readfirstlane(tid >> 6);
         const long long grow0 = tile * PN_CTILE;
         float4 c3v[8];
@@ -196,7 +206,7 @@
             rs.set(tid, Si, invSi, S);
             gb4x += d0; gb4y += d1; gb4z += d2;
         }
-        const long long si_next = row_sample(tile + gridDim.x);
+        const long long si_next = row_sample(tile_next);
         PN_LDS_BARRIER();
         {
             const int c4 = tid & 31, rg = tid >> 5;
@@ -236,7 +246,9 @@
         }
         PnGemmW<8, 4, 1, 4, 3> WD3;
         WD3.prefetch(reinterpret_cast<const uint4 *>(img + PKH_DC3), wave, lane);
-        PN_LDS_BARRIER();
+        if (tid == 0) *claim_w = claimed;
+        PN_LDS_BARRIER();
+        const long long tile_after = pn_claim_tile(PN_CLAIM_STATIC_CBWD, gridDim.x, __builtin_amdgcn_readfirstlane(*claim_w), 0);
         pn_copy_out_kmajor_hs<PN_HC, CB_XRS>(X, rs, a.sv.dc3k, tile * 8, tid);
         if (WG2) pn_copy_out_kmajor_hs<PN_HC, CB_XRS>(X + CB_XPL, rs, a.sv.dc3m, tile * 8, tid);
         pn_acc_zero(acc);
@@ -274,6 +286,8 @@
                     PN_REG_STORE(t, reinterpret_cast<pn_f4 *>(a.sv.dfs + (grow0 + 32 * rb + (lane & 31)) * PN_H + pn_d_feat(2 * wave + fb, g, lane)));
                 }
             }
+        PN_TR_SPAN(pn_span_cbwd, 0, 1);
+        tile = tile_next; tile_next = tile_after;
     }
     PN_LDS_BARRIER();
     {
@@ -1315,4 +1329,7 @@
 extern "C" int pnerf_debug_span_bwd(void *host, size_t bytes) {
     return hipMemcpyFromSymbol(host, HIP_SYMBOL(pn_span_bwd), bytes < sizeof(pn_span_bwd) ? bytes : sizeof(pn_span_bwd)) == hipSuccess ? 0 : -1;
 }
+extern "C" int pnerf_debug_span_cbwd(void *host, size_t bytes) {
+    return hipMemcpyFromSymbol(host, HIP_SYMBOL(pn_span_cbwd), bytes < sizeof(pn_span_cbwd) ? bytes : sizeof(pn_span_cbwd)) == hipSuccess ? 0 : -1;
+}
 #endif
diff --git a/pointnerf_amd/csrc/grid.hip b/pointnerf_amd/csrc/grid.hip
--- a/pointnerf_amd/csrc/grid.hip
+++ b/pointnerf_amd/csrc/grid.hip
@@ -267,5 +267,5 @@
     return 0;
 }
 
-extern "C" int pnerf_version(void) { return 1009; }
+extern "C" int pnerf_version(void) { return 1010; }
 extern "C" const char *pnerf_arch(void) { return "gfx950"; }
diff --git a/pointnerf_amd/csrc/mlp_common.h b/pointnerf_amd/csrc/mlp_common.h
--- a/pointnerf_amd/csrc/mlp_common.h
+++ b/pointnerf_amd/csrc/mlp_common.h
@@ -92,11 +92,15 @@
     long long rows, samples;
 };
 enum : int { PN_NCLS = 3, PN_CI_COUNT = 0, PN_CI_VBASE = 4, PN_CI_TBASE = 8, PN_CI_TILES = 12, PN_CI_CTILES = 13 ,
-              PN_CI_CLAIM = 16 , PN_CI_WORDS = 20 };
+              PN_CI_CLAIM = 16 , PN_CI_CLAIM_COLOR = 19 ,
+              PN_CI_WORDS = 20 };
 #ifndef PN_CLAIM_TILES
 #define PN_CLAIM_TILES 1
 #endif
-enum : int { PN_CLAIM_STATIC_FWD = 4, PN_CLAIM_STATIC_BWD = 2, PN_GS_CLAIM = 4, PN_GS_WORDS = 8 };
+enum : int { PN_CLAIM_STATIC_FWD = 4, PN_CLAIM_STATIC_BWD = 2, PN_GS_CLAIM = 4, PN_GS_CLAIM_COLOR = 7, PN_GS_WORDS = 8 };
+enum : int { PN_CLAIM_STATIC_CFWD = 1, PN_CLAIM_STATIC_CBWD = 2 };
+static_assert(PN_CI_CLAIM + PN_NCLS <= PN_CI_CLAIM_COLOR && PN_CI_CLAIM_COLOR < PN_CI_WORDS && PN_GS_CLAIM + PN_NCLS <= PN_GS_CLAIM_COLOR && PN_GS_CLAIM_COLOR < PN_GS_WORDS,
+              "one counter word per launch");
 __device__ __forceinline__ int pn_claim_tile(int nstatic, int grid, int v, int m) { return nstatic * grid + v * PN_CLAIM_TILES + m % PN_CLAIM_TILES; }
 int pn_tile_grid(long long tiles, long long dflt);
 int pn_class_slots(int K, int kc[3]);
@@ -126,7 +130,7 @@
 
 
 #ifdef PN_PHASE_TRACE
-#define PN_TR_WGS   512
+#define PN_TR_WGS   768
 #define PN_TR_IT0   20
 #define PN_TR_ITERS 6
 #define PN_TR_SLOTS 24
diff --git a/pointnerf_amd/ops.py b/pointnerf_amd/ops.py
--- a/pointnerf_amd/ops.py
+++ b/pointnerf_amd/ops.py
@@ -629,6 +629,22 @@
     return old
 
 
+def classify_samples(valid_list, counters, pidx, K, n=None):
+    n = int(valid_list.numel() if n is None else n)
+    for t in (valid_list, counters, pidx):
+        _need_cuda(t, "classify_samples")
+        assert t.dtype == torch.int32 and t.is_contiguous()
+    assert 0 <= n <= valid_list.numel() and counters.numel() >= 1
+    dev = counters.device
+    cls_list = torch.full((max(n, 1),), -7, dtype=torch.int32, device=dev)
+    info = torch.full((L.lib().pnerf_debug_classify_info_words(),), -7, dtype=torch.int32, device=dev)
+    nbytes = L.lib().pnerf_debug_classify_workspace_bytes(n)
+    ws = torch.empty(max(nbytes, 4), dtype=torch.uint8, device=dev)
+    L.check(L.lib().pnerf_debug_classify(_ptr(valid_list), _ptr(counters), _ptr(pidx), int(K), n, _ptr(cls_list), _ptr(info), _ptr(ws), nbytes,
+                                         _stream()), "pnerf_debug_classify")
+    return cls_list[:n], info
+
+
 def arithmetic():
     out = (ctypes.c_int32 * 4)()
     L.check(L.lib().pnerf_get_arithmetic(out), "pnerf_get_arithmetic")
```
